# kspalaiologos/modern-rzip

Measured on AMD Instinct MI355X. Metric: rzip-stage GiB/s (mrzip -n), higher is better.
Workload: dtype u8; 1 GPU; tar-64G: rzip stage of mrzip -L7 on a 64 GiB synthetic tar (60 % text members, 25 % noise, 15 % exact duplicates, 512-byte aligned; BASELINE configs[2], the largest single-GPU configuration), one chunk per GPU, input resident in HBM; level=7, chunk_bytes_per_gpu=68719476736, streams=1, mode=streams

## Files before the change

### modern-rzip_amd/csrc/mrz_capi.hip

```cpp
#include <stdio.h>
#include <stdlib.h>
#include <string.h>

#include "../../include/mrzgpu.h"
#include "mrz_ctx.h"



static const unsigned k_levels[10][3] = { { 1, 4, 1 },  { 2, 4, 2 },  { 4, 4, 2 },   { 8, 4, 2 },   { 16, 4, 3 },
                                          { 32, 4, 4 }, { 32, 2, 6 }, { 64, 1, 16 }, { 64, 1, 32 }, { 64, 1, 128 } };

static void mrz_make_hash_index(int64_t H[256]) {
    int32_t r[31];
    int32_t word = 1;
    r[0] = 1;
    for (int i = 1; i < 31; i++) {
        const long hi = word / 127773, lo = word % 127773;
        long w = 16807 * lo - 2836 * hi;
        if (w < 0) w += 2147483647;
        r[i] = word = (int32_t)w;
    }
    int f = 3, b = 0;
    uint32_t draw[512];
    for (int k = -310; k < 512; k++) {
        const uint32_t s = (uint32_t)r[f] + (uint32_t)r[b];
        r[f] = (int32_t)s;
        if (++f == 31) f = 0;
        if (++b == 31) b = 0;
        if (k >= 0) draw[k] = s >> 1;
    }
    for (int i = 0; i < 256; i++) H[i] = ((int64_t)draw[2 * i] << 16) ^ (int64_t)draw[2 * i + 1];
}

extern "C" int mrz_abi_version(void) { return MRZ_ABI_VERSION; }

#define MRZ_EVENT_CAP (1ll << 28)
#define MRZ_EVENT_MIN 1024ll
#define MRZ_EVENT_MAX (1ll << 31)
static int64_t mrz_event_room(const mrz_ctx *ctx, int64_t n) {
    if (ctx->event_cap_set > 0) return ctx->event_cap_set;
    const int64_t worst = n / MRZ_MIN_MATCH + 2;
    return worst < MRZ_EVENT_CAP ? worst : MRZ_EVENT_CAP;
}

extern "C" const char *mrz_strerror(int code) {
    switch (code) {
        case MRZ_OK: return "ok";
        case MRZ_E_ARG: return "bad argument";
        case MRZ_E_NODEVICE: return "no usable HIP device (libmrzgpu has no CPU fallback)";
        case MRZ_E_NOMEM: return "out of memory";
        case MRZ_E_HIP: return "HIP runtime error";
        case MRZ_E_OVERFLOW: return "internal capacity exceeded";
        case MRZ_E_STATE: return "call order violated";
        case MRZ_E_CORRUPT: return "corrupt record stream or archive";
        case MRZ_E_UNSUPPORTED: return "block type not handled on this path (back-end codecs are host code)";
        default: return "unknown error";
    }
}

extern "C" int mrz_last_hip_error(const mrz_ctx *ctx, const char **text) {
    if (!ctx) return 0;
    if (text) *text = hipGetErrorString(ctx->last_err);
    return (int)ctx->last_err;
}

extern "C" int mrz_chunk_bytes(int64_t chunk_size) {
    int bits = 8;
    while (chunk_size >> bits > 0) bits++;
    return bits / 8 + (bits % 8 ? 1 : 0);
}

extern "C" void mrz_close(mrz_ctx *ctx) {
    if (!ctx) return;
    hipSetDevice(ctx->device);
    if (ctx->stream) hipStreamSynchronize(ctx->stream);
    hipFree(ctx->d_index);
    hipFree(ctx->d_tab);
    hipFree(ctx->d_state);
    if (ctx->h_ring) hipHostFree(ctx->h_ring);
    hipFree(ctx->d_fe_hdr);
    hipFree(ctx->d_bitmap);
    hipFree(ctx->d_tile_cnt);
    hipFree(ctx->d_tile_off);
    hipFree(ctx->d_grp_cnt);
    hipFree(ctx->d_cand);
    hipFree(ctx->d_events);
    hipFree(ctx->d_block_s0);
    hipFree(ctx->d_block_s1);
    hipFree(ctx->d_lit_off);
    hipFree(ctx->d_totals);
    hipFree(ctx->d_s0);
    hipFree(ctx->d_s1);
    hipFree(ctx->d_in);
    hipFree(ctx->d_crc_tables);
    hipFree(ctx->d_crc_parts);
    hipFree(ctx->d_crc_out);
    if (ctx->d_gmailbox) hipFree(ctx->d_gmailbox);
    if (ctx->d_seq_shared) hipFree(ctx->d_seq_shared);
    if (ctx->d_deep_shared) hipFree(ctx->d_deep_shared);
    if (ctx->d_wlog) hipFree(ctx->d_wlog);
    if (ctx->rz_scratch) hipFree(ctx->rz_scratch);
    if (ctx->d_rz_out) hipFree(ctx->d_rz_out);
    if (ctx->d_rz_done) hipFree(ctx->d_rz_done);
    if (ctx->d_rs_tables) hipFree(ctx->d_rs_tables);
    if (ctx->d_rs_out) hipFree(ctx->d_rs_out);
    if (ctx->lz4_scratch) hipFree(ctx->lz4_scratch);
    if (ctx->b2_scratch) hipFree(ctx->b2_scratch);
    if (ctx->side_stream) hipStreamDestroy(ctx->side_stream);
    if (ctx->copy_stream) hipStreamDestroy(ctx->copy_stream);
    if (ctx->stream) hipStreamDestroy(ctx->stream);
    free(ctx);
}

extern "C" int mrz_open(mrz_ctx **out, int device, int level, int64_t max_chunk) {
    if (!out || level < 1 || level > 9 || max_chunk < 0) return MRZ_E_ARG;
    *out = nullptr;
    int ndev = 0;
    hipError_t e0 = hipGetDeviceCount(&ndev);
    if (e0 != hipSuccess || ndev <= 0 || device < 0 || device >= ndev) {
        fprintf(stderr, "libmrzgpu: hipGetDeviceCount -> %d (%s), %d device(s), asked for %d\n", (int)e0,
                hipGetErrorString(e0), ndev, device);
        return MRZ_E_NODEVICE;
    }
    e0 = hipSetDevice(device);
    if (e0 != hipSuccess) {
        fprintf(stderr, "libmrzgpu: hipSetDevice(%d) -> %d (%s)\n", device, (int)e0, hipGetErrorString(e0));
        return MRZ_E_NODEVICE;
    }
    mrz_ctx *ctx = (mrz_ctx *)calloc(1, sizeof(mrz_ctx));
    if (!ctx) return MRZ_E_NOMEM;
    ctx->farm_helpers = -1;
    ctx->seg_positions = MRZ_SEG_POSITIONS;
    ctx->cand_cap = MRZ_CAND_CAP;
    {
        const char *e = getenv("MRZ_SEQ_ENGINE");
        if (e && !strcmp(e, "wide")) ctx->engine_pin = 1;
        if (e && !strcmp(e, "narrow")) ctx->engine_pin = 2;
        if (e && !strcmp(e, "deep")) ctx->engine_pin = 3;
        ctx->deep_min_bits = 6;
        if (const char *d = getenv("MRZ_DEEP_MIN_BITS")) ctx->deep_min_bits = atoi(d);
        ctx->narrow_max_bits = ctx->deep_min_bits;
        if (const char *d = getenv("MRZ_NARROW_MAX_BITS")) ctx->narrow_max_bits = atoi(d);
        e = getenv("MRZ_PRINT_PROF");
        if (e) ctx->print_prof = !strcmp(e, "narrow") ? 2 : 1;
        if (const char *c = getenv("MRZ_EVENT_CAPACITY")) {
            const long long v = atoll(c);
            if (v >= MRZ_EVENT_MIN && v <= MRZ_EVENT_MAX)
                ctx->event_cap_set = v;
            else if (v > 0)
                fprintf(stderr, "libmrzgpu: MRZ_EVENT_CAPACITY=%s ignored (%lld .. %lld entries)\n", c, MRZ_EVENT_MIN,
                        MRZ_EVENT_MAX);
        }
    }
    ctx->farm_default = mrz_sequencer_default_helpers(device);
    ctx->device = device;
    ctx->level = level;
    ctx->mb_used = k_levels[level][0];
    ctx->initial_freq = k_levels[level][1];
    ctx->max_chain = k_levels[level][2];
    const int64_t want = (int64_t)ctx->mb_used * (1048576 / 16);
    for (ctx->hash_bits = 0; (1ll << ctx->hash_bits) < want; ctx->hash_bits++) {
    }
    ctx->nslots = 1ll << ctx->hash_bits;
    mrz_make_hash_index(ctx->h_index);

    int rc = MRZ_OK;
    e0 = hipStreamCreate(&ctx->stream);
    if (e0 != hipSuccess) {
        fprintf(stderr, "libmrzgpu: hipStreamCreate -> %d (%s)\n", (int)e0, hipGetErrorString(e0));
        rc = MRZ_E_NODEVICE;
    }
    int64_t cap;
    if (!rc) { cap = 0; rc = mrz_grow(ctx, &ctx->d_index, &cap, 256); }
    if (!rc) { cap = 0; rc = mrz_grow(ctx, &ctx->d_tab, &cap, ctx->nslots); }
    if (!rc) { cap = 0; rc = mrz_grow(ctx, &ctx->d_state, &cap, 1); }
    if (!rc && hipHostMalloc((void **)&ctx->h_ring, MRZ_SEG_AHEAD * sizeof(mrz_seq_state)) != hipSuccess) rc = MRZ_E_NOMEM;
    if (!rc) { cap = 0; rc = mrz_grow(ctx, &ctx->d_fe_hdr, &cap, 1); }
    if (!rc) { cap = 0; rc = mrz_grow(ctx, &ctx->d_totals, &cap, 1); }
    if (!rc) { cap = 0; rc = mrz_grow(ctx, &ctx->d_crc_out, &cap, 4); }
    if (!rc) {
        void *p = nullptr;
        if (hipMalloc(&p, mrz_crc_tables_size()) != hipSuccess)
            rc = MRZ_E_NOMEM;
        else
            ctx->d_crc_tables = (mrz_crc_tables *)p;
    }
    if (!rc) {
        mrz_crc_tables *tb = (mrz_crc_tables *)malloc(mrz_crc_tables_size());
        if (!tb)
            rc = MRZ_E_NOMEM;
        else {
            mrz_crc_build_tables(tb);
            if (hipMemcpy(ctx->d_crc_tables, tb, mrz_crc_tables_size(), hipMemcpyHostToDevice) != hipSuccess)
                rc = MRZ_E_HIP;
            free(tb);
        }
    }
    if (!rc && hipMemcpy(ctx->d_index, ctx->h_index, sizeof(ctx->h_index), hipMemcpyHostToDevice) != hipSuccess)
        rc = MRZ_E_HIP;
    const size_t mbox = mrz_sequencer_mailbox_size() > mrz_seq_narrow_mailbox_size() ? mrz_sequencer_mailbox_size()
                                                                                     : mrz_seq_narrow_mailbox_size();
    if (!rc && mbox && !getenv("MRZ_NO_HELPER_WGS")) {
        void *p = nullptr;
        if (hipMalloc(&p, mbox) != hipSuccess)
            rc = MRZ_E_NOMEM;
        else
            ctx->d_gmailbox = p;
    }
    if (!rc) {
        if (hipMalloc(&ctx->d_seq_shared, mrz_sequencer_shared_size()) != hipSuccess ||
            hipMalloc((void **)&ctx->d_wlog, mrz_sequencer_wlog_size(ctx->nslots)) != hipSuccess)
            rc = MRZ_E_NOMEM;
        ctx->seq_wgs = 3;
        if (const char *e = getenv("MRZ_SEQ_WGS")) ctx->seq_wgs = atoi(e);
        if (hipMalloc(&ctx->d_deep_shared, mrz_seq_deep_shared_size()) != hipSuccess) rc = MRZ_E_NOMEM;
        ctx->deep_scanners = 63;
        if (const char *e = getenv("MRZ_DEEP_SCANNERS")) ctx->deep_scanners = atoi(e);
    }
    if (!rc && max_chunk > 0) {
        rc = mrz_grow(ctx, &ctx->d_events, &ctx->event_cap, mrz_event_room(ctx, max_chunk));
        if (!rc) rc = mrz_grow(ctx, &ctx->d_crc_parts, &ctx->crc_parts_cap, mrz_crc32_parts_needed(max_chunk));
        if (!rc) rc = mrz_fe_reserve(ctx, max_chunk / MRZ_TILE + 2, max_chunk);
    }
    if (rc) {
        mrz_close(ctx);
        return rc;
    }
    *out = ctx;
    return MRZ_OK;
}

extern "C" void *mrz_stream(const mrz_ctx *ctx) { return ctx ? (void *)ctx->stream : nullptr; }

extern "C" int mrz_synchronize(mrz_ctx *ctx) {
    if (!ctx) return MRZ_E_ARG;
    HIPCHK(ctx, hipSetDevice(ctx->device));
    HIPCHK(ctx, hipStreamSynchronize(ctx->stream));
    return MRZ_OK;
}

extern "C" int mrz_set_profiling(mrz_ctx *ctx, int enable) {
    if (!ctx) return MRZ_E_ARG;
    ctx->profiling = enable ? 1 : 0;
    return MRZ_OK;
}

extern "C" int mrz_set_progress(mrz_ctx *ctx, mrz_progress_fn fn, void *user) {
    if (!ctx) return MRZ_E_ARG;
    ctx->progress_fn = fn;
    ctx->progress_user = user;
    return MRZ_OK;
}

extern "C" int mrz_fetch_events(mrz_ctx *ctx, int64_t first, int64_t count, mrz_match *host_dst) {
    if (!ctx || first < 0 || count < 0 || (count > 0 && !host_dst)) return MRZ_E_ARG;
    if (first + count > ctx->events_final) return MRZ_E_STATE;
    if (first < ctx->ev_base) return MRZ_E_STATE;
    if (!count) return MRZ_OK;
    HIPCHK(ctx, hipSetDevice(ctx->device));
    if (!ctx->copy_stream) HIPCHK(ctx, hipStreamCreateWithFlags(&ctx->copy_stream, hipStreamNonBlocking));
    static_assert(sizeof(mrz_match) == sizeof(mrz_event), "mrz_match mirrors mrz_event");
    HIPCHK(ctx, hipMemcpyAsync(host_dst, ctx->d_events + (first - ctx->ev_base), (size_t)count * sizeof(mrz_event), hipMemcpyDeviceToHost,
                               ctx->copy_stream));
    HIPCHK(ctx, hipStreamSynchronize(ctx->copy_stream));
    return MRZ_OK;
}

extern "C" int mrz_set_cand_provider(mrz_ctx *ctx, mrz_cand_provider_fn fn, void *user) {
    if (!ctx) return MRZ_E_ARG;
    ctx->cand_fn = fn;
    ctx->cand_user = user;
    return MRZ_OK;
}

extern "C" int mrz_copy_to_device(mrz_ctx *ctx, void *dst_device, const void *src_host, int64_t n) {
    if (!ctx || n < 0 || (n > 0 && (!dst_device || !src_host))) return MRZ_E_ARG;
    if (!n) return MRZ_OK;
    HIPCHK(ctx, hipSetDevice(ctx->device));
    HIPCHK(ctx, hipMemcpyAsync(dst_device, src_host, (size_t)n, hipMemcpyHostToDevice, ctx->stream));
    HIPCHK(ctx, hipStreamSynchronize(ctx->stream));
    return MRZ_OK;
}

extern "C" int mrz_copy_device(mrz_ctx *ctx, void *dst_device, const void *src_device, int64_t n) {
    if (!ctx || n < 0 || (n > 0 && (!dst_device || !src_device))) return MRZ_E_ARG;
    if (!n) return MRZ_OK;
    HIPCHK(ctx, hipSetDevice(ctx->device));
    HIPCHK(ctx, hipMemcpyAsync(dst_device, src_device, (size_t)n, hipMemcpyDeviceToDevice, ctx->stream));
    HIPCHK(ctx, hipStreamSynchronize(ctx->stream));
    return MRZ_OK;
}

extern "C" int mrz_set_segment_positions(mrz_ctx *ctx, int64_t positions) {
    if (!ctx || positions < MRZ_TILE || positions > MRZ_SEG_POSITIONS || positions % MRZ_TILE) return MRZ_E_ARG;
    ctx->seg_positions = positions;
    return MRZ_OK;
}

extern "C" int mrz_set_candidate_capacity(mrz_ctx *ctx, int64_t entries) {
    if (!ctx || entries < MRZ_TILE || entries > (1ll << 30)) return MRZ_E_ARG;
    ctx->cand_cap = entries;
    return MRZ_OK;
}

extern "C" int mrz_set_event_capacity(mrz_ctx *ctx, int64_t entries) {
    if (!ctx || (entries > 0 && entries < MRZ_EVENT_MIN) || entries > MRZ_EVENT_MAX) return MRZ_E_ARG;
    ctx->event_cap_set = entries > 0 ? entries : 0;
    return MRZ_OK;
}

extern "C" int mrz_set_xcd(mrz_ctx *ctx, int xcd) {
    if (!ctx || xcd < 0 || xcd > 7) return MRZ_E_ARG;
    ctx->xcd = xcd;
    return MRZ_OK;
}

int mrz_fe_reserve(mrz_ctx *ctx, int64_t tiles, int64_t entries) {
    const int64_t max_tiles = ctx->seg_positions / MRZ_TILE;
    if (tiles > max_tiles) tiles = max_tiles;
    if (tiles < 1) tiles = 1;
    if (entries > ctx->cand_cap) entries = ctx->cand_cap;
    if (entries < MRZ_TILE) entries = MRZ_TILE;
    if (tiles > ctx->fe_tiles_cap) {
        int64_t c0 = 0, c1 = 0, c2 = 0, c3 = 0;
        if (ctx->d_bitmap) hipFree(ctx->d_bitmap), ctx->d_bitmap = nullptr;
        if (ctx->d_tile_cnt) hipFree(ctx->d_tile_cnt), ctx->d_tile_cnt = nullptr;
        if (ctx->d_tile_off) hipFree(ctx->d_tile_off), ctx->d_tile_off = nullptr;
        if (ctx->d_grp_cnt) hipFree(ctx->d_grp_cnt), ctx->d_grp_cnt = nullptr;
        ctx->fe_tiles_cap = 0;
        int rc = mrz_grow(ctx, &ctx->d_bitmap, &c0, tiles * (MRZ_TILE / 16) + 64);
        if (!rc) rc = mrz_grow(ctx, &ctx->d_tile_cnt, &c1, tiles + 1);
        if (!rc) rc = mrz_grow(ctx, &ctx->d_tile_off, &c2, tiles + 2);
        if (!rc) rc = mrz_grow(ctx, &ctx->d_grp_cnt, &c3, tiles / MRZ_FE_GROUP + 2);
        if (rc) return rc;
        ctx->fe_tiles_cap = tiles;
    }
    return mrz_grow(ctx, &ctx->d_cand, &ctx->cand_alloc, entries);
}

extern "C" int mrz_window_scan(mrz_ctx *ctx, const void *range_bytes, int64_t range_len, int where, int64_t range_start,
                               int64_t chunk_n, int64_t seg_start, int64_t max_span, int64_t min_mask, int64_t p_done,
                               int64_t cap, mrz_candidate *cand_out, int32_t *tile_off_out, void *bitmap_out, int out_where,
                               int64_t *scan_next, int64_t *n_cand) {
    if (!ctx || !range_bytes || !cand_out || !tile_off_out || !bitmap_out || !scan_next || !n_cand) return MRZ_E_ARG;
    if (range_len <= 0 || range_start < 0 || chunk_n <= 0 || cap < MRZ_TILE) return MRZ_E_ARG;
    if (max_span <= 0 || max_span > ctx->seg_positions || max_span % MRZ_TILE || seg_start % MRZ_TILE || seg_start < range_start)
        return MRZ_E_ARG;
    if (out_where != MRZ_MEM_HOST && out_where != MRZ_MEM_DEVICE) return MRZ_E_ARG;
    const int64_t end = chunk_n - MRZ_MIN_MATCH;
    int64_t last_pos = seg_start + max_span - 1;
    if (last_pos > end) last_pos = end;
    const int64_t need_end = last_pos + 48 < chunk_n ? last_pos + 48 : chunk_n;
    if (last_pos >= seg_start && need_end > range_start + range_len) return MRZ_E_ARG;
    HIPCHK(ctx, hipSetDevice(ctx->device));
    const uint8_t *d_range = nullptr;
    int rc = mrz_stage_input(ctx, range_bytes, range_len, where, &d_range);
    if (rc) return rc;
    const int64_t tiles = max_span / MRZ_TILE;
    const int64_t save_cap = ctx->cand_cap;
    if (cap > ctx->cand_cap) ctx->cand_cap = cap;
    rc = mrz_fe_reserve(ctx, tiles, cap);
    ctx->cand_cap = save_cap;
    if (rc) return rc;
    mrz_seq_state hs;
    memset(&hs, 0, sizeof(hs));
    hs.n = chunk_n;
    hs.end = end;
    hs.p = p_done + 1 < seg_start + MRZ_TILE ? p_done : seg_start - 1;
    hs.min_mask = min_mask;
    hs.scan_next = seg_start;
    hipStream_t s = ctx->stream;
    HIPCHK(ctx, hipMemcpyAsync(ctx->d_state, &hs, sizeof(hs), hipMemcpyHostToDevice, s));
    HIPCHK(ctx, mrz_launch_frontend(s, d_range - range_start, chunk_n, ctx->d_index, ctx->d_state, (int)tiles, cap,
                                    ctx->d_fe_hdr, ctx->d_bitmap, ctx->d_tile_cnt, ctx->d_tile_off, ctx->d_grp_cnt, ctx->d_cand));
    HIPCHK(ctx, hipMemcpyAsync(&hs, ctx->d_state, sizeof(hs), hipMemcpyDeviceToHost, s));
    HIPCHK(ctx, hipStreamSynchronize(s));
    int64_t T = (hs.scan_next - seg_start) / MRZ_TILE;
    if (hs.seg_start != seg_start || T < 0 || T > tiles) {
        T = 0;
        hs.n_cand = 0;
        hs.scan_next = hs.scan_next > seg_start ? hs.scan_next : seg_start;
    }
    const hipMemcpyKind k = out_where == MRZ_MEM_HOST ? hipMemcpyDeviceToHost : hipMemcpyDeviceToDevice;
    if (hs.n_cand > 0) HIPCHK(ctx, hipMemcpyAsync(cand_out, ctx->d_cand, (size_t)hs.n_cand * sizeof(mrz_cand), k, s));
    if (T > 0) {
        HIPCHK(ctx, hipMemcpyAsync(tile_off_out, ctx->d_tile_off, (size_t)(T + 1) * sizeof(int), k, s));
        HIPCHK(ctx, hipMemcpyAsync(bitmap_out, ctx->d_bitmap, (size_t)T * (MRZ_TILE / 8), k, s));
    }
    HIPCHK(ctx, hipStreamSynchronize(s));
    *scan_next = hs.scan_next;
    *n_cand = hs.n_cand;
    return MRZ_OK;
}

extern "C" int mrz_set_farm_helpers(mrz_ctx *ctx, int n) {
    if (!ctx) return MRZ_E_ARG;
    ctx->farm_helpers = n < 0 ? -1 : n;
    return MRZ_OK;
}

extern "C" int mrz_get_timings(const mrz_ctx *ctx, mrz_timings *out) {
    if (!ctx || !out) return MRZ_E_ARG;
    *out = ctx->timings;
    return MRZ_OK;
}

extern "C" int64_t mrz_table_slots(const mrz_ctx *ctx) { return ctx ? ctx->nslots : 0; }

extern "C" int mrz_fetch_table(mrz_ctx *ctx, void *host_dst) {
    if (!ctx || !host_dst) return MRZ_E_ARG;
    if (!ctx->have_chunk) return MRZ_E_STATE;
    HIPCHK(ctx, hipSetDevice(ctx->device));
    HIPCHK(ctx, hipMemcpy(host_dst, ctx->d_tab, (size_t)ctx->nslots * sizeof(mrz_slot), hipMemcpyDeviceToHost));
    return MRZ_OK;
}

int mrz_stage_input(mrz_ctx *ctx, const void *buf, int64_t n, int where, const uint8_t **dev) {
    if (where == MRZ_MEM_DEVICE) {
        *dev = (const uint8_t *)buf;
        return MRZ_OK;
    }
    if (where != MRZ_MEM_HOST) return MRZ_E_ARG;
    int rc = mrz_grow(ctx, &ctx->d_in, &ctx->in_cap, n + 64);
    if (rc) return rc;
    if (n > 0) HIPCHK(ctx, hipMemcpyAsync(ctx->d_in, buf, (size_t)n, hipMemcpyHostToDevice, ctx->stream));
    *dev = ctx->d_in;
    return MRZ_OK;
}

extern "C" int mrz_crc32(mrz_ctx *ctx, const void *buf, int64_t n, int where, uint32_t *crc_out) {
    if (!ctx || !crc_out || n < 0 || (n > 0 && !buf)) return MRZ_E_ARG;
    HIPCHK(ctx, hipSetDevice(ctx->device));
    const uint8_t *d = nullptr;
    int rc = mrz_stage_input(ctx, buf, n, where, &d);
    if (rc) return rc;
    rc = mrz_grow(ctx, &ctx->d_crc_parts, &ctx->crc_parts_cap, mrz_crc32_parts_needed(n));
    if (rc) return rc;
    HIPCHK(ctx, mrz_launch_crc32(ctx->stream, d, n, ctx->d_crc_tables, ctx->d_crc_parts, ctx->d_crc_out));
    HIPCHK(ctx, hipMemcpyAsync(crc_out, ctx->d_crc_out, 4, hipMemcpyDeviceToHost, ctx->stream));
    HIPCHK(ctx, hipStreamSynchronize(ctx->stream));
    return MRZ_OK;
}

struct mrz_evpair {
    hipEvent_t a, b;
    int kind;
};

static int64_t mrz_span_for_mask(const mrz_ctx *ctx, int64_t mask) {
    const int k = __builtin_popcountll((unsigned long long)mask);
    int64_t span = (ctx->cand_cap - ctx->cand_cap / 4) << (k < 24 ? k : 24);
    if (span > ctx->seg_positions) span = ctx->seg_positions;
    span = span / MRZ_TILE * MRZ_TILE;
    return span < MRZ_TILE ? MRZ_TILE : span;
}

extern "C" int mrz_rzip_chunk(mrz_ctx *ctx, const void *chunk, int64_t n, int where, int chunk_bytes,
                              int64_t *victim_round, mrz_chunk_result *res) {
    if (!ctx || !res || !victim_round || n < 0 || (n > 0 && !chunk) || chunk_bytes < 1 || chunk_bytes > 8)
        return MRZ_E_ARG;
    if (*victim_round < 0 || *victim_round >= (int64_t)ctx->max_chain) return MRZ_E_ARG;
    HIPCHK(ctx, hipSetDevice(ctx->device));
    memset(res, 0, sizeof(*res));
    memset(&ctx->timings, 0, sizeof(ctx->timings));
    ctx->have_chunk = 0;
    hipStream_t s = ctx->stream;

    const uint8_t *d_buf = nullptr;
    int rc = mrz_stage_input(ctx, chunk, n, where, &d_buf);
    if (rc) return rc;
    rc = mrz_grow(ctx, &ctx->d_events, &ctx->event_cap, mrz_event_room(ctx, n));
    if (rc) return rc;
    const int64_t ev_cap = ctx->event_cap_set > 0 ? ctx->event_cap_set : ctx->event_cap;
    const bool bounded = ev_cap < n / MRZ_MIN_MATCH + 2;
    rc = mrz_grow(ctx, &ctx->d_crc_parts, &ctx->crc_parts_cap, mrz_crc32_parts_needed(n));
    if (rc) return rc;
    const int64_t end = n - MRZ_MIN_MATCH;
    if (end > 0) {
        rc = mrz_fe_reserve(ctx, end / MRZ_TILE + 2, end + 1);
        if (rc) return rc;
    }

    mrz_evpair *evs = nullptr;
    int nev = 0, evcap = 0;
    hipEvent_t ev_begin = nullptr, ev_end = nullptr;
    if (ctx->profiling) {
        hipEventCreate(&ev_begin);
        hipEventCreate(&ev_end);
        hipEventRecord(ev_begin, s);
    }
#define PROF_BEGIN(k)                                                                       \
    do {                                                                                    \
        if (ctx->profiling) {                                                               \
            if (nev == evcap) {                                                             \
                const int ncap__ = evcap ? evcap * 2 : 64;                                  \
                mrz_evpair *ne__ = (mrz_evpair *)realloc(evs, (size_t)ncap__ * sizeof(mrz_evpair)); \
                if (ne__) evs = ne__, evcap = ncap__;                                       \
            }                                                                               \
            if (nev < evcap) {                                                              \
                evs[nev].kind = (k);                                                        \
                hipEventCreate(&evs[nev].a);                                                \
                hipEventCreate(&evs[nev].b);                                                \
                hipEventRecord(evs[nev].a, s);                                              \
            }                                                                               \
        }                                                                                   \
    } while (0)
#define PROF_END()                                     \
    do {                                               \
        if (ctx->profiling && nev < evcap) {           \
            hipEventRecord(evs[nev].b, s);             \
            nev++;                                     \
        }                                              \
    } while (0)

    mrz_seq_state hs;
    memset(&hs, 0, sizeof(hs));
    hs.n = n;
    hs.end = end;
    hs.min_mask = hs.tag_mask = (1ll << ctx->initial_freq) - 1;
    hs.limit = ctx->nslots / 3 * 2;
    hs.victim_round = *victim_round;
    hs.max_chain = ctx->max_chain;
    hs.slot_mask = ctx->nslots - 1;
    hs.event_cap = ev_cap;
    hs.finished = end > 0 ? 0 : 1;
    hipError_t herr = hipSuccess;
    int64_t E = 0;
    uint32_t crc = 0;
    mrz_enc_totals tot;
    memset(&tot, 0, sizeof(tot));

#define STEP(expr)                       \
    do {                                 \
        if (herr == hipSuccess) herr = (expr); \
    } while (0)

    STEP(hipMemsetAsync(ctx->d_tab, 0, (size_t)ctx->nslots * sizeof(mrz_slot), s));
    STEP(hipMemcpyAsync(ctx->d_state, &hs, sizeof(hs), hipMemcpyHostToDevice, s));
    STEP(hipMemsetAsync(ctx->d_totals, 0, sizeof(mrz_enc_totals), s));

    PROF_BEGIN(3);
    STEP(mrz_launch_crc32(s, d_buf, n, ctx->d_crc_tables, ctx->d_crc_parts, ctx->d_crc_out));
    PROF_END();

    ctx->events_final = 0;
    ctx->ev_base = 0;
    const size_t snap_bytes = offsetof(mrz_seq_state, prof);
    hipEvent_t seg_ev[MRZ_SEG_AHEAD];
    int n_seg_ev = 0;
    for (int k = 0; k < MRZ_SEG_AHEAD && herr == hipSuccess; k++) {
        STEP(hipEventCreateWithFlags(&seg_ev[k], hipEventDisableTiming));
        if (herr == hipSuccess) n_seg_ev++;
    }
    int64_t launched = 0, retired = 0, n_narrow = 0, n_deep = 0;
    int64_t span_of[MRZ_SEG_AHEAD];
    int64_t known_next = 0;
    int64_t known_mask = hs.min_mask, known_p = 0;
    int64_t hint_pos = 0, hint_matched = 0;
    int64_t known_events = 0, known_last = 0;
    bool finished = end <= 0;
    auto retire = [&]() {
        const mrz_seq_state *sn = &ctx->h_ring[retired % MRZ_SEG_AHEAD];
        retired++;
        known_p = sn->p;
        known_mask = sn->min_mask;
        known_events = sn->n_events;
        known_last = sn->last_match;
        if (!ctx->cand_fn)
            known_next = sn->scan_next;
        else if (sn->seg_end > sn->seg_start && sn->scan_next < sn->seg_end)
            known_next = sn->scan_next;
        hint_pos = sn->hint_positions;
        hint_matched = sn->hint_matched;
        if (ctx->progress_fn) {
            ctx->events_final = sn->n_events;
            if (ctx->progress_fn(ctx->progress_user, sn->n_events, sn->last_match, 0)) rc = MRZ_E_STATE;
        }
        if (sn->finished || sn->error) finished = true;
    };
    int64_t base0 = 0, base1 = 0, lit_from = 0, n_flushes = 0;
    auto encode_piece = [&](int64_t upto, int final_piece) {
        const int64_t Ep = upto - ctx->ev_base;
        const int64_t nblocks = (Ep + 1 + 255) / 256;
        int r = mrz_grow(ctx, &ctx->d_block_s0, &ctx->block_cap, nblocks);
        if (!r) r = mrz_grow(ctx, &ctx->d_block_s1, &ctx->block1_cap, nblocks);
        if (!r) r = mrz_grow(ctx, &ctx->d_lit_off, &ctx->lit_off_cap, Ep + 2);
        if (r) return r;
        PROF_BEGIN(2);
        STEP(mrz_launch_enc_size(s, ctx->d_events, Ep, final_piece, lit_from, n, chunk_bytes, ctx->d_block_s0,
                                 ctx->d_block_s1, base0, base1, ctx->d_totals));
        STEP(hipMemcpyAsync(&tot, ctx->d_totals, sizeof(tot), hipMemcpyDeviceToHost, s));
        STEP(hipStreamSynchronize(s));
        if (herr == hipSuccess) {
            if (!base0) r = mrz_grow(ctx, &ctx->d_s0, &ctx->s0_cap, tot.s0_len + 7 + 16);
            else r = mrz_grow_keep(ctx, &ctx->d_s0, &ctx->s0_cap, base0 + tot.s0_len + 7 + 16, base0);
            if (!r && !base1) r = mrz_grow(ctx, &ctx->d_s1, &ctx->s1_cap, tot.s1_len + 16);
            else if (!r) r = mrz_grow_keep(ctx, &ctx->d_s1, &ctx->s1_cap, base1 + tot.s1_len + 16, base1);
        }
        if (herr == hipSuccess && !r) {
            STEP(mrz_launch_enc_write(s, d_buf, ctx->d_events, Ep, final_piece, lit_from, n, chunk_bytes, ctx->d_block_s0,
                                      ctx->d_block_s1, ctx->d_s0, ctx->d_s1, base1, tot.s1_len, ctx->d_lit_off,
                                      ctx->d_totals, crc));
            STEP(hipMemcpyAsync(&tot, ctx->d_totals, sizeof(tot), hipMemcpyDeviceToHost, s));
        }
        PROF_END();
        return r;
    };
    auto drain = [&]() {
        const int r = encode_piece(known_events, 0);
        if (r || herr != hipSuccess) return r;
        ctx->ev_base = known_events;
        STEP(hipMemcpyAsync(&ctx->d_state->ev_base, &ctx->ev_base, sizeof(int64_t), hipMemcpyHostToDevice, s));
        STEP(hipStreamSynchronize(s));
        base0 += tot.s0_len;
        base1 += tot.s1_len;
        lit_from = known_last;
        n_flushes++;
        return 0;
    };
    int64_t pass_cap = MRZ_MIN_MATCH * (ev_cap / 2) / MRZ_TILE * MRZ_TILE;
    if (pass_cap < MRZ_TILE) pass_cap = MRZ_TILE;
    while (!finished && herr == hipSuccess && !rc) {
        while (retired < launched && !finished && !rc && hipEventQuery(seg_ev[retired % MRZ_SEG_AHEAD]) == hipSuccess) retire();
        if (finished || rc) break;
        int64_t est_next = known_next;
        for (int64_t k = retired; k < launched; k++) est_next += span_of[k % MRZ_SEG_AHEAD];
        const bool queue_full = launched - retired >= MRZ_SEG_AHEAD;
        const bool all_queued = est_next > end;
        if (queue_full || (all_queued && launched > retired)) {
            STEP(hipEventSynchronize(seg_ev[retired % MRZ_SEG_AHEAD]));
            if (herr != hipSuccess) break;
            retire();
            continue;
        }
        if (all_queued) {
            rc = MRZ_E_OVERFLOW;
            break;
        }
        int64_t span = mrz_span_for_mask(ctx, known_mask);
        if (bounded && span > pass_cap) span = pass_cap;
        int64_t max_tiles = span / MRZ_TILE;
        if (max_tiles > ctx->fe_tiles_cap) max_tiles = ctx->fe_tiles_cap;
        span = max_tiles * MRZ_TILE;
        if (bounded) {
            const int64_t pt = (known_p + 1) / MRZ_TILE * MRZ_TILE;
            int64_t from = known_next > pt ? known_next : pt;
            for (int64_t k = retired; k < launched; k++) from += span_of[k % MRZ_SEG_AHEAD];
            const int64_t fixed = known_events - ctx->ev_base + 2 + 1 + (launched - retired + 1);
            int64_t F = from + span - 1;
            if (F > end) F = end;
            if (fixed + (F - known_p) / MRZ_MIN_MATCH > ev_cap) {
                if (launched > retired) {
                    STEP(hipEventSynchronize(seg_ev[retired % MRZ_SEG_AHEAD]));
                    if (herr != hipSuccess) break;
                    retire();
                    continue;
                }
                if (known_events > ctx->ev_base) {
                    rc = drain();
                    continue;
                }
                const int64_t fit = (ev_cap - fixed) * MRZ_MIN_MATCH + MRZ_MIN_MATCH - 1 - (from - 1 - known_p);
                if (fit < MRZ_TILE) {
                    rc = MRZ_E_OVERFLOW;
                    break;
                }
                if (span > fit) span = fit / MRZ_TILE * MRZ_TILE;
                max_tiles = span / MRZ_TILE;
            }
        }
        PROF_BEGIN(0);
        if (ctx->cand_fn) {
            int64_t seg_start = known_next;
            const int64_t pt = (known_p + 1) / MRZ_TILE * MRZ_TILE;
            if (pt > seg_start) seg_start = pt;
            if (seg_start > end) {
                known_next = seg_start;
                span_of[launched % MRZ_SEG_AHEAD] = 0;
            } else {
                if (seg_start + span > end + 1) span = (end + 1 - seg_start + MRZ_TILE - 1) / MRZ_TILE * MRZ_TILE;
                int64_t geo[5] = { seg_start, 0, 0, 0, known_mask };
                int64_t nx = seg_start, nc = 0;
                if (herr == hipSuccess && ctx->cand_fn(ctx->cand_user, seg_start, span, known_mask, known_p, ctx->cand_cap,
                                                       (mrz_candidate *)ctx->d_cand, ctx->d_tile_off, ctx->d_bitmap, &nx, &nc,
                                                       (void *)s)) {
                    hipStreamSynchronize(s);
                    rc = MRZ_E_STATE;
                    break;
                }
                if (nx <= seg_start || nx > seg_start + span || nx % MRZ_TILE || nc < 0 || nc > ctx->cand_cap) {
                    hipStreamSynchronize(s);
                    rc = MRZ_E_STATE;
                    break;
                }
                geo[1] = nx < end + 1 ? nx : end + 1;
                geo[2] = nc;
                geo[3] = nx;
                STEP(hipMemcpyAsync(&ctx->d_state->seg_start, geo, sizeof(geo), hipMemcpyHostToDevice, s));
                STEP(hipStreamSynchronize(s));
                known_next = nx;
                span_of[launched % MRZ_SEG_AHEAD] = 0;
            }
        } else {
            STEP(mrz_launch_frontend(s, d_buf, n, ctx->d_index, ctx->d_state, (int)max_tiles, ctx->cand_cap, ctx->d_fe_hdr,
                                     ctx->d_bitmap, ctx->d_tile_cnt, ctx->d_tile_off, ctx->d_grp_cnt, ctx->d_cand));
            span_of[launched % MRZ_SEG_AHEAD] = span;
        }
        PROF_END();
        const int mask_bits = __builtin_popcountll((unsigned long long)known_mask);
        bool narrow = hint_pos > 0 && hint_matched * 10 >= hint_pos * 8 && mask_bits < ctx->narrow_max_bits;
        bool deep = !narrow && mask_bits >= ctx->deep_min_bits;
        if (ctx->engine_pin) narrow = ctx->engine_pin == 2, deep = ctx->engine_pin == 3;
        const int helpers = ctx->farm_helpers >= 0 && ctx->farm_helpers < ctx->farm_default ? ctx->farm_helpers : ctx->farm_default;
        PROF_BEGIN(1);
        if (narrow)
            STEP(mrz_launch_sequencer_narrow(s, d_buf, ctx->d_tab, ctx->d_cand, ctx->d_tile_off, (const mrz_u64 *)ctx->d_bitmap,
                                             ctx->d_events, ctx->d_state, ctx->d_gmailbox, helpers, ctx->xcd));
        else if (deep)
            STEP(mrz_launch_sequencer_deep(s, d_buf, ctx->d_tab, ctx->d_cand, ctx->d_tile_off, (const mrz_u64 *)ctx->d_bitmap,
                                           ctx->d_events, ctx->d_state, ctx->d_gmailbox, helpers, ctx->xcd, ctx->d_deep_shared,
                                           ctx->deep_scanners));
        else
            STEP(mrz_launch_sequencer(s, d_buf, ctx->d_tab, ctx->d_cand, ctx->d_tile_off, (const mrz_u64 *)ctx->d_bitmap,
                                      ctx->d_events, ctx->d_state, ctx->d_gmailbox, helpers, ctx->d_seq_shared, ctx->d_wlog,
                                      ctx->nslots, ctx->seq_wgs, ctx->xcd, ctx->engine_pin ? 0 : ctx->deep_min_bits));
        PROF_END();
        if (narrow) n_narrow++;
        if (deep) n_deep++;
        STEP(hipMemcpyAsync(&ctx->h_ring[launched % MRZ_SEG_AHEAD], ctx->d_state, snap_bytes, hipMemcpyDeviceToHost, s));
        STEP(hipEventRecord(seg_ev[launched % MRZ_SEG_AHEAD], s));
        launched++;
        if (launched <= 2 && !ctx->engine_pin && !ctx->cand_fn) STEP(hipStreamSynchronize(s));
    }
    hipStreamSynchronize(s);
    for (int k = 0; k < n_seg_ev; k++) hipEventDestroy(seg_ev[k]);
    STEP(hipMemcpyAsync(&hs, ctx->d_state, sizeof(hs), hipMemcpyDeviceToHost, s));
    STEP(hipMemcpyAsync(&crc, ctx->d_crc_out, 4, hipMemcpyDeviceToHost, s));
    STEP(hipStreamSynchronize(s));
    if (herr == hipSuccess) {
        if (!rc && (hs.error || !hs.finished)) {
            fprintf(stderr,
                    "libmrzgpu: sequencer stopped abnormally: error=%d finished=%d p=%lld end=%lld events=%lld/%lld "
                    "count=%lld min_mask=%lld scan_next=%lld launches=%lld\n",
                    hs.error, hs.finished, (long long)hs.p, (long long)hs.end, (long long)hs.n_events,
                    (long long)hs.event_cap, (long long)hs.count, (long long)hs.min_mask, (long long)hs.scan_next,
                    (long long)launched);
            rc = MRZ_E_OVERFLOW;
        }
        E = hs.n_events;
        if (!rc && ctx->progress_fn) {
            ctx->events_final = E;
            if (ctx->progress_fn(ctx->progress_user, E, hs.last_match, 1)) rc = MRZ_E_STATE;
        }
    }

    if (herr == hipSuccess && !rc) {
        rc = encode_piece(E, 1);
        if (ctx->profiling) hipEventRecord(ev_end, s);
        STEP(hipStreamSynchronize(s));
    }

    ctx->timings.n_segments = (int32_t)launched;
    ctx->timings.n_narrow = (int32_t)n_narrow;
    ctx->timings.n_deep = (int32_t)n_deep;
    ctx->timings.n_event_flushes = (int32_t)n_flushes;
    if (ctx->profiling) {
        hipStreamSynchronize(s);
        for (int i = 0; i < nev; i++) {
            float ms = 0;
            if (hipEventElapsedTime(&ms, evs[i].a, evs[i].b) == hipSuccess) {
                if (evs[i].kind == 0) ctx->timings.tagscan_ms += ms;
                if (evs[i].kind == 1) ctx->timings.sequencer_ms += ms;
                if (evs[i].kind == 2) ctx->timings.encode_ms += ms;
                if (evs[i].kind == 3) ctx->timings.crc_ms += ms;
            }
            hipEventDestroy(evs[i].a);
            hipEventDestroy(evs[i].b);
        }
        float ms = 0;
        if (hipEventElapsedTime(&ms, ev_begin, ev_end) == hipSuccess) ctx->timings.total_ms = ms;
        hipEventDestroy(ev_begin);
        hipEventDestroy(ev_end);
        free(evs);
    }
#undef PROF_BEGIN
#undef PROF_END
#undef STEP
    if (herr != hipSuccess) {
        ctx->last_err = herr;
        return MRZ_E_HIP;
    }
    if (rc) return rc;

    *victim_round = hs.victim_round;
    ctx->s0_len = base0 + tot.s0_len + 7;
    ctx->s1_len = base1 + tot.s1_len;
    ctx->have_chunk = 1;
    res->s0_len = ctx->s0_len;
    res->s1_len = ctx->s1_len;
    res->crc32 = crc;
    res->d_s0 = ctx->d_s0;
    res->d_s1 = ctx->d_s1;
    res->stats.inserts = hs.inserts;
    res->stats.tag_hits = hs.tag_hits;
    res->stats.tag_misses = hs.tag_misses;
    res->stats.literals = tot.literals + 1;
    res->stats.literal_bytes = tot.literal_bytes;
    res->stats.matches = tot.matches;
    res->stats.match_bytes = tot.match_bytes;
    res->min_mask = hs.min_mask;
    res->hash_count = hs.count;
    res->n_events = E;
    if (ctx->print_prof) {
        static const char *names[128] = { "batches", "formed", "committed", "segments", "emits", "backjump", "rewalk",
                                          "longres", "seq_cands", "cut_cplx", "cut_overflow", "skipout", "conf0", "pairs",
                                          "t_form", "t_walk", "t_conf", "t_pairs", "t_loop", "t_rewalk", "t_long", "t_seq",
                                          "farmed", "l_post", "l_stripe", "l_bwd", "l_wait", "l_rounds", "f_post", "f_wait",
                                          "f_fold", "s_tab", "s_pair", "s_ins", "ovl", "ovl_ok", "x_walk", "x_casc", "x_pool",
                                          "x_win", "x_same", "c_win", "c_evict", "c_deep", "c_many", "c_fail", "c_tie", "c_nw", "t_ovl",
                                          "h_pre", "h_cand", "h_post", "t_scan", "t_fold", "t_commit", "reprep", "w_stale", "w_drop", "reset",
                                          "t_turn", "t_prep", "t_precommit", "e_mask", "e_cull", "e_xw", "e_inwin", "e_window", "e_bulk",
                                          "e_more", "t_pc_cw", "t_pc_log", "t_pc_best", "t_pc_bulk", "t_turnwork", "t_snap", "rebulk",
                                          "batch_lanes", "cut_long", "cut_walk", "cut_conflict", "cut_cull", "batch_emits",
                                          "cut_cascade", "batch_formed", "t_walk2", "t_scans", "t_conflict", "t_window",
                                          "d_batches", "d_lanes", "d_rounds", "d_rescanned", "d_coop", "d_t_form", "d_t_scan",
                                          "d_t_commit", "d_t_rescan", "d_t_total", "d_launches", "d_t_coop", "d_coop_rec",
                                          "d_resolved", "d_s_coop", "d_s_conflict", "d_s_culled", "d_s_nocull", "d_s_stale", "d_c_over_alt", "d_c_over_noalt", "d_c_empty",
                                          "d_c_displace", "d_c_other" };
        for (int k = 0; k < 128; k++)
            if (names[k] && hs.prof[k]) fprintf(stderr, "seqstat %-12s %lld\n", names[k], (long long)hs.prof[k]);
    }
    return MRZ_OK;
}

extern "C" int mrz_fetch_streams(mrz_ctx *ctx, uint8_t *s0_host, uint8_t *s1_host) {
    if (!ctx) return MRZ_E_ARG;
    if (!ctx->have_chunk) return MRZ_E_STATE;
    HIPCHK(ctx, hipSetDevice(ctx->device));
    if (s0_host && ctx->s0_len > 0)
        HIPCHK(ctx, hipMemcpyAsync(s0_host, ctx->d_s0, (size_t)ctx->s0_len, hipMemcpyDeviceToHost, ctx->stream));
    if (s1_host && ctx->s1_len > 0)
        HIPCHK(ctx, hipMemcpyAsync(s1_host, ctx->d_s1, (size_t)ctx->s1_len, hipMemcpyDeviceToHost, ctx->stream));
    HIPCHK(ctx, hipStreamSynchronize(ctx->stream));
    return MRZ_OK;
}
```

### modern-rzip_amd/csrc/mrz_common.h

```cpp
#pragma once
#include <stdint.h>

#define MRZ_MIN_MATCH 31
#define MRZ_GREAT_MATCH 1024
#define MRZ_WAVE 64

struct __attribute__((aligned(16))) mrz_slot {
    int64_t off;
    int64_t t;
};

struct mrz_event {
    int64_t p;
    int64_t ofs;
    int64_t len;
};

struct mrz_seq_state {
    int64_t n;
    int64_t end;
    int64_t p;
    int64_t cur_p, cur_ofs, cur_len;
    int64_t last_match;
    int64_t min_mask;
    int64_t tag_mask;
    int64_t count;
    int64_t limit;
    int64_t clean_ptr;
    int64_t victim_round;
    int64_t max_chain;
    int64_t slot_mask;
    int64_t n_events;
    int64_t event_cap;
    int64_t ev_base;
    int64_t inserts, tag_hits, tag_misses;
    int32_t finished;
    int32_t error;
    int64_t hint_positions;
    int64_t hint_events;
    int64_t hint_matched;
    int64_t seg_start;
    int64_t seg_end;
    int64_t n_cand;
    int64_t scan_next;
    int64_t list_mask;
    int64_t prof[128];
};

typedef mrz_slot mrz_cand;

struct mrz_fe_hdr {
    int64_t base;
    int64_t mask;
    int64_t p_done;
    int32_t ntiles;
    int32_t T;
};

#define MRZ_TILE 4096
#define MRZ_TILE_SHIFT 12
#define MRZ_FE_GROUP 256

struct mrz_enc_totals {
    int64_t s0_len;
    int64_t s1_len;
    int64_t literals, literal_bytes, matches, match_bytes;
};
```

### modern-rzip_amd/csrc/mrz_ctx.h

```cpp
#pragma once
#include <stdint.h>
#include <stdlib.h>

#include "../../include/mrzgpu.h"
#include "mrz_kernels.h"

#define MRZ_SEG_POSITIONS (1ll << 30)
#define MRZ_CAND_CAP (8ll << 20)
#define MRZ_SEG_AHEAD 4

struct mrz_ctx {
    int device;
    int level;
    unsigned mb_used, initial_freq, max_chain;
    int hash_bits;
    int64_t nslots;
    hipStream_t stream;
    hipError_t last_err;
    int profiling;
    mrz_timings timings;

    int64_t h_index[256];
    int64_t *d_index;
    mrz_slot *d_tab;
    mrz_seq_state *d_state;
    mrz_seq_state *h_ring;
    mrz_fe_hdr *d_fe_hdr;
    uint16_t *d_bitmap;
    int *d_tile_cnt, *d_tile_off, *d_grp_cnt;
    int64_t fe_tiles_cap;
    mrz_cand *d_cand;
    int64_t cand_alloc;
    int64_t cand_cap;
    int engine_pin;
    int deep_min_bits;
    int narrow_max_bits;
    int print_prof;
    int xcd;
    mrz_event *d_events;
    int64_t event_cap;
    int64_t event_cap_set;
    int64_t ev_base;
    int64_t *d_block_s0, *d_block_s1;
    int64_t block_cap, block1_cap;
    int64_t *d_lit_off;
    int64_t lit_off_cap;
    mrz_enc_totals *d_totals;
    uint8_t *d_s0, *d_s1;
    int64_t s0_cap, s1_cap;
    int64_t s0_len, s1_len;
    uint8_t *d_in;
    int64_t in_cap;
    mrz_crc_tables *d_crc_tables;
    uint32_t *d_crc_parts;
    int64_t crc_parts_cap;
    uint32_t *d_crc_out;
    void *d_gmailbox;
    void *d_seq_shared;
    unsigned *d_wlog;
    int seq_wgs;
    void *d_deep_shared;
    int deep_scanners;
    int farm_helpers;
    int farm_default;
    void *d_rs_tables;
    uint8_t *d_rs_out;
    int64_t rs_out_cap;
    void *rz_scratch;
    int64_t rz_scratch_cap;
    uint8_t *d_rz_out;
    int64_t rz_out_cap;
    unsigned *d_rz_done;
    int64_t rz_done_cap;
    int have_chunk;

    void *lz4_scratch;
    int64_t lz4_scratch_cap;
    void *b2_scratch;
    int64_t b2_scratch_cap;
    hipStream_t side_stream;
    hipStream_t copy_stream;
    mrz_progress_fn progress_fn;
    void *progress_user;
    int64_t events_final;
    int64_t seg_positions;
    mrz_cand_provider_fn cand_fn;
    void *cand_user;
};

#define HIPCHK(ctx, expr)                     \
    do {                                      \
        hipError_t e__ = (expr);              \
        if (e__ != hipSuccess) {              \
            (ctx)->last_err = e__;            \
            return MRZ_E_HIP;                 \
        }                                     \
    } while (0)

template <typename T>
static inline int mrz_grow(mrz_ctx *ctx, T **ptr, int64_t *cap, int64_t want) {
    if (want <= *cap && *ptr) return MRZ_OK;
    if (*ptr) {
        hipFree(*ptr);
        *ptr = nullptr;
        *cap = 0;
    }
    int64_t ask = want < 16 ? 16 : want;
    void *p = nullptr;
    hipError_t e = hipMalloc(&p, (size_t)ask * sizeof(T));
    if (e != hipSuccess) {
        ctx->last_err = e;
        return MRZ_E_NOMEM;
    }
    *ptr = (T *)p;
    *cap = ask;
    return MRZ_OK;
}

template <typename T>
static inline int mrz_grow_keep(mrz_ctx *ctx, T **ptr, int64_t *cap, int64_t want, int64_t keep) {
    if (want <= *cap && *ptr) return MRZ_OK;
    int64_t ask = *cap + *cap / 2 > want ? *cap + *cap / 2 : want;
    if (ask < 16) ask = 16;
    void *p = nullptr;
    hipError_t e = hipMalloc(&p, (size_t)ask * sizeof(T));
    if (e != hipSuccess && ask > want) {
        ask = want;
        e = hipMalloc(&p, (size_t)ask * sizeof(T));
    }
    if (e != hipSuccess) {
        ctx->last_err = e;
        return MRZ_E_NOMEM;
    }
    if (*ptr) {
        if (keep > 0) e = hipMemcpyAsync(p, *ptr, (size_t)keep * sizeof(T), hipMemcpyDeviceToDevice, ctx->stream);
        if (e == hipSuccess) e = hipStreamSynchronize(ctx->stream);
        if (e != hipSuccess) {
            hipFree(p);
            ctx->last_err = e;
            return MRZ_E_HIP;
        }
        hipFree(*ptr);
    }
    *ptr = (T *)p;
    *cap = ask;
    return MRZ_OK;
}

int mrz_fe_reserve(mrz_ctx *ctx, int64_t tiles, int64_t entries);

int mrz_stage_input(mrz_ctx *ctx, const void *buf, int64_t n, int where, const uint8_t **dev);
```

### modern-rzip_amd/csrc/mrz_kernels.h

```cpp
#pragma once
#include <hip/hip_runtime.h>
#include <stdint.h>

#include "mrz_common.h"

typedef unsigned long long mrz_u64;
struct mrz_crc_tables;

extern "C" {
struct mrz_fe_bufs {
    mrz_fe_hdr *hdr;
    uint16_t *bitmap16;
    int *tile_cnt;
    int *tile_off;
    int *grp_cnt;
    mrz_cand *cand;
};
hipError_t mrz_launch_frontend(hipStream_t stream, const uint8_t *buf, int64_t n, const int64_t *hash_index,
                               mrz_seq_state *st, int max_tiles, int64_t cap, mrz_fe_hdr *hdr, uint16_t *bitmap16,
                               int *tile_cnt, int *tile_off, int *grp_cnt, mrz_cand *cand);
hipError_t mrz_launch_sequencer(hipStream_t stream, const uint8_t *buf, mrz_slot *tab, const mrz_cand *cand,
                                const int *tile_off, const mrz_u64 *bitmap, mrz_event *events, mrz_seq_state *st,
                                void *gmailbox, int n_helpers, void *wide_shared, unsigned *wlog,
                                int64_t nslots, int seq_wgs, int xcd, int deep_bits);
size_t mrz_sequencer_shared_size(void);
size_t mrz_sequencer_wlog_size(int64_t nslots);
hipError_t mrz_launch_sequencer_narrow(hipStream_t stream, const uint8_t *buf, mrz_slot *tab, const mrz_cand *cand,
                                       const int *tile_off, const mrz_u64 *bitmap, mrz_event *events, mrz_seq_state *st,
                                       void *gmailbox, int n_helpers, int xcd);
hipError_t mrz_launch_sequencer_deep(hipStream_t stream, const uint8_t *buf, mrz_slot *tab, const mrz_cand *cand,
                                     const int *tile_off, const mrz_u64 *bitmap, mrz_event *events, mrz_seq_state *st,
                                     void *gmailbox, int n_helpers, int xcd, void *deep_shared, int scanners);
size_t mrz_seq_deep_shared_size(void);
size_t mrz_sequencer_mailbox_size(void);
size_t mrz_seq_narrow_mailbox_size(void);
int mrz_sequencer_default_helpers(int device);
hipError_t mrz_launch_enc_size(hipStream_t stream, const mrz_event *ev, int64_t E, int final_piece, int64_t lit0,
                               int64_t n, int cb, int64_t *block_s0, int64_t *block_s1, int64_t base0, int64_t base1,
                               mrz_enc_totals *totals);
hipError_t mrz_launch_enc_write(hipStream_t stream, const uint8_t *buf, const mrz_event *ev, int64_t E, int final_piece,
                                int64_t lit0, int64_t n, int cb, const int64_t *block_s0, const int64_t *block_s1,
                                uint8_t *s0, uint8_t *s1, int64_t base1, int64_t s1_len, int64_t *lit_off,
                                mrz_enc_totals *totals, uint32_t crc);
void mrz_crc_build_tables(mrz_crc_tables *tb);
size_t mrz_crc_tables_size(void);
int64_t mrz_crc32_parts_needed(int64_t n);
hipError_t mrz_launch_crc32(hipStream_t stream, const uint8_t *buf, int64_t n, const mrz_crc_tables *tb, uint32_t *parts,
                            uint32_t *crc_out);
}
```

### modern-rzip_amd/csrc/mrz_seq_common.h

```cpp
#pragma once
#include "mrz_device.h"
#include <stdlib.h>

#ifdef __HIP_DEVICE_COMPILE__
#define MRZ_WAVE_SYNC() __builtin_amdgcn_wave_barrier()
#else
#define MRZ_WAVE_SYNC() (void)__ballot(1)
#endif

#ifndef MRZ_WIDE_WAVES
#define MRZ_WIDE_WAVES 8
#endif
#ifndef MRZ_SEQ_WAVES
#define MRZ_SEQ_WAVES MRZ_WIDE_WAVES
#endif
#define MRZ_SEQ_THREADS (64 * MRZ_SEQ_WAVES)
#ifdef MRZ_NARROW_ENGINE
#define MRZ_STRIPE_WAVES (MRZ_SEQ_WAVES > 2 ? MRZ_SEQ_WAVES - 1 : MRZ_SEQ_WAVES)
#else
#define MRZ_STRIPE_WAVES 1
#endif
#ifndef MRZ_HELPER_WAVES
#define MRZ_HELPER_WAVES 3
#endif
#define MRZ_CASCADE_MAX 64
#ifndef MRZ_SEQ_CREDIT
#define MRZ_SEQ_CREDIT 8
#endif
#ifndef MRZ_LOW_YIELD_RUNS
#define MRZ_LOW_YIELD_RUNS 2
#endif

#ifdef MRZ_SEQ_PROFILE
#define PROF_T0() int64_t prof_t0 = (int64_t)__builtin_amdgcn_s_memtime()
#define PROF_T0R() prof_t0 = (int64_t)__builtin_amdgcn_s_memtime()
#define PROF_ADD(k)                                                      \
    do {                                                                 \
        const int64_t now__ = (int64_t)__builtin_amdgcn_s_memtime();     \
        stat[k] += now__ - prof_t0;                                      \
        prof_t0 = now__;                                                 \
    } while (0)
#else
#define PROF_T0()
#define PROF_T0R()
#define PROF_ADD(k)
#endif

#if defined(MRZ_SEQ_PROFILE) && !defined(MRZ_SEQ_STATS)
#define MRZ_SEQ_STATS 1
#endif
#ifdef MRZ_SEQ_STATS
#define ST_ADD(k, v) (stat[k] += (v))
#else
#define ST_ADD(k, v) ((void)0)
#endif
#ifndef MRZ_WLOG_SHIFT
#define MRZ_WLOG_SHIFT 2
#endif
enum { MRZ_ST_BATCHES, MRZ_ST_FORMED, MRZ_ST_COMMITTED, MRZ_ST_SEGMENTS, MRZ_ST_EMITS, MRZ_ST_BACKJUMP, MRZ_ST_REWALK,
       MRZ_ST_LONGRES, MRZ_ST_SEQ, MRZ_ST_CUT_CPLX, MRZ_ST_CUT_OVERFLOW, MRZ_ST_SKIPOUT, MRZ_ST_CONF0, MRZ_ST_PAIRS,
       MRZ_ST_T_FORM, MRZ_ST_T_WALK, MRZ_ST_T_CONF, MRZ_ST_T_PAIRS, MRZ_ST_T_LOOP, MRZ_ST_T_REWALK, MRZ_ST_T_LONG,
       MRZ_ST_T_SEQ, MRZ_ST_FARMED, MRZ_ST_L_POST, MRZ_ST_L_STRIPE, MRZ_ST_L_BWD, MRZ_ST_L_WAIT, MRZ_ST_L_ROUNDS,
       MRZ_ST_F_POST, MRZ_ST_F_WAIT, MRZ_ST_F_FOLD, MRZ_ST_S_TAB, MRZ_ST_S_PAIR, MRZ_ST_S_INS, MRZ_ST_OVL, MRZ_ST_OVL_OK,
       MRZ_ST_X_WALK, MRZ_ST_X_CASC, MRZ_ST_X_POOL, MRZ_ST_X_WIN, MRZ_ST_X_SAME, MRZ_ST_C_WIN, MRZ_ST_C_EVICT, MRZ_ST_C_DEEP,
       MRZ_ST_C_MANY, MRZ_ST_C_FAIL, MRZ_ST_C_TIE, MRZ_ST_C_NW, MRZ_ST_T_OVL, MRZ_ST_H_PRE, MRZ_ST_H_CAND, MRZ_ST_H_POST,
       MRZ_ST_T_SCAN, MRZ_ST_T_FOLD, MRZ_ST_T_COMMIT, MRZ_ST_REPREP, MRZ_ST_W_STALE, MRZ_ST_W_DROP, MRZ_ST_RESET,
       MRZ_ST_T_TURN, MRZ_ST_T_PREP, MRZ_ST_T_PRECOMMIT, MRZ_ST_E_MASK, MRZ_ST_E_CULL, MRZ_ST_E_XW, MRZ_ST_E_INWIN,
       MRZ_ST_E_WINDOW, MRZ_ST_E_BULK, MRZ_ST_E_MORE, MRZ_ST_T_PC_CW, MRZ_ST_T_PC_LOG, MRZ_ST_T_PC_BEST, MRZ_ST_T_PC_BULK, MRZ_ST_T_TURNWORK, MRZ_ST_T_SNAP, MRZ_ST_REBULK,
       MRZ_ST_BATCH_LANES, MRZ_ST_CUT_LONG, MRZ_ST_CUT_WALK, MRZ_ST_CUT_CONFLICT, MRZ_ST_CUT_CULL, MRZ_ST_BATCH_EMITS,
       MRZ_ST_CUT_CASCADE, MRZ_ST_BATCH_FORMED, MRZ_ST_T_WALK2, MRZ_ST_T_SCANS, MRZ_ST_T_CONFLICT, MRZ_ST_T_WINDOW,
       MRZ_ST_D_BATCHES, MRZ_ST_D_LANES, MRZ_ST_D_ROUNDS, MRZ_ST_D_RESCANNED, MRZ_ST_D_COOP, MRZ_ST_D_T_FORM, MRZ_ST_D_T_SCAN,
       MRZ_ST_D_T_COMMIT, MRZ_ST_D_T_RESCAN, MRZ_ST_D_T_TOTAL, MRZ_ST_D_LAUNCHES, MRZ_ST_D_T_COOP, MRZ_ST_D_COOP_REC,
       MRZ_ST_D_RESOLVED, MRZ_ST_D_S_COOP, MRZ_ST_D_S_CONFLICT, MRZ_ST_D_S_CULLED, MRZ_ST_D_S_NOCULL, MRZ_ST_D_S_STALE, MRZ_ST_D_C_OVER_ALT, MRZ_ST_D_C_OVER_NOALT, MRZ_ST_D_C_EMPTY, MRZ_ST_D_C_DISPLACE, MRZ_ST_D_C_OTHER,
       MRZ_ST_N };
static_assert(MRZ_ST_N <= (int)(sizeof(((mrz_seq_state *)0)->prof) / sizeof(int64_t)), "mrz_seq_state.prof holds the counters");

struct mrz_seq_args {
    const uint8_t *buf;
    mrz_slot *tab;
    const mrz_cand *cand;
    const int *tile_off;
    const mrz_u64 *bitmap;
    mrz_event *events;
    mrz_seq_state *st;
    void *gmailbox;
    int n_helpers;
    int xcd;
    int deep_bits;
};

struct mrz_cands {
    const mrz_cand *cand;
    const int *tile_off;
    const mrz_u64 *bitmap;
    int64_t seg_start, seg_end, n;
};

__device__ static int64_t mrz_cand_lower_bound(const mrz_cands &K, int64_t pos, int lane) {
    if (pos <= K.seg_start) return 0;
    if (pos >= K.seg_end) return K.n;
    const int64_t rel = pos - K.seg_start;
    const int64_t tile = rel >> MRZ_TILE_SHIFT;
    const int r = (int)(rel & (MRZ_TILE - 1));
    const mrz_u64 w = K.bitmap[tile * (MRZ_TILE / 64) + lane];
    const int base = K.tile_off[tile];
    int c = 0;
    if (lane < (r >> 6))
        c = __popcll(w);
    else if (lane == (r >> 6))
        c = __popcll(w & mrz_low_mask(r & 63));
    const int sum = mrz_lane_read(mrz_wave_incl_sum(c, lane), 63);
    return (int64_t)mrz_uni(base) + sum;
}

__device__ __forceinline__ int mrz_mb_load(int *p) {
    return __hip_atomic_load(p, __ATOMIC_ACQUIRE, __HIP_MEMORY_SCOPE_WORKGROUP);
}
__device__ __forceinline__ void mrz_mb_store(int *p, int v) {
    __hip_atomic_store(p, v, __ATOMIC_RELEASE, __HIP_MEMORY_SCOPE_WORKGROUP);
}

__device__ __forceinline__ void mrz_mb_add(int *p, int v) {
    __hip_atomic_fetch_add(p, v, __ATOMIC_RELEASE, __HIP_MEMORY_SCOPE_WORKGROUP);
}

struct mrz_mailbox {
    int64_t p0, op, maxf, base;
    int64_t res[MRZ_SEQ_WAVES];
    int seq;
    int done;
    int quit;
    int scout_seq;
    int64_t scout_pos;
    int64_t scout_clean;
};

#ifndef MRZ_STRIPE_PIECES
#define MRZ_STRIPE_PIECES 4
#endif
#define MRZ_STRIPE (MRZ_STRIPE_PIECES * 1024)

template <int PIECES>
__device__ static int64_t mrz_wave_fwd_stripe_n(const uint8_t *__restrict__ buf, int64_t p0, int64_t op, int64_t maxf,
                                                int64_t base, int lane) {
    uint4 a[PIECES], b[PIECES];
#pragma unroll
    for (int j = 0; j < PIECES; j++) {
        const int64_t off = base + j * 1024 + lane * 16;
        if (off < maxf) {
            a[j] = mrz_ld16(buf + p0 + off);
            b[j] = mrz_ld16(buf + op + off);
        }
    }
    int64_t found = -1;
#pragma unroll
    for (int j = 0; j < PIECES; j++) {
        if (found >= 0) continue;
        const int64_t off = base + j * 1024 + lane * 16;
        int lane_len = 0;
        bool full = false;
        if (off < maxf) {
            const int64_t rem = maxf - off;
            const int lim = rem < 16 ? (int)rem : 16;
            const int d = mrz_first_diff16(a[j], b[j]);
            lane_len = d < lim ? d : lim;
            full = lane_len == 16;
        }
        const mrz_u64 stop = __ballot(!full);
        if (stop) {
            const int fl = __ffsll((long long)stop) - 1;
            found = base + j * 1024 + (int64_t)fl * 16 + mrz_lane_read(lane_len, fl);
        }
    }
    return found;
}

__device__ __forceinline__ int64_t mrz_wave_fwd_stripe(const uint8_t *__restrict__ buf, int64_t p0, int64_t op,
                                                       int64_t maxf, int64_t base, int lane) {
    return mrz_wave_fwd_stripe_n<MRZ_STRIPE_PIECES>(buf, p0, op, maxf, base, lane);
}

__device__ static int64_t mrz_wave_bwd(const uint8_t *__restrict__ buf, int64_t p0, int64_t op, int64_t maxb,
                                       int lane) {
    if (maxb <= 0) return 0;
    for (int64_t base = 0;; base += 1024) {
        const int64_t off = base + lane * 16;
        int lane_len = 0;
        bool full = false;
        if (off < maxb) {
            const int64_t rem = maxb - off;
            const int lim = rem < 16 ? (int)rem : 16;
            int cnt;
            if (op - off - 16 >= 0) {
                cnt = mrz_top_equal16(mrz_ld16(buf + p0 - off - 16), mrz_ld16(buf + op - off - 16));
            } else {
                cnt = 0;
                while (cnt < lim && buf[p0 - off - 1 - cnt] == buf[op - off - 1 - cnt]) cnt++;
            }
            lane_len = cnt < lim ? cnt : lim;
            full = lane_len == 16;
        }
        const mrz_u64 stop = __ballot(!full);
        if (stop) {
            const int fl = __ffsll((long long)stop) - 1;
            return base + (int64_t)fl * 16 + mrz_lane_read(lane_len, fl);
        }
    }
}

__device__ static int64_t mrz_long_match_len(const uint8_t *__restrict__ buf, mrz_mailbox *mb, int *mb_seq, int64_t p0,
                                             int64_t op, int64_t end, int64_t last_match, int64_t *rev_out, int lane,
                                             int64_t *stat = nullptr, int64_t *cont_base = nullptr) {
    *rev_out = 0;
#ifdef MRZ_SEQ_PROFILE
    int64_t lt0 = (int64_t)__builtin_amdgcn_s_memtime();
#define LPROF(k)                                                         \
    do {                                                                 \
        if (stat) {                                                      \
            const int64_t now__ = (int64_t)__builtin_amdgcn_s_memtime(); \
            stat[k] += now__ - lt0;                                      \
            lt0 = now__;                                                 \
        }                                                                \
    } while (0)
#else
#define LPROF(k)
#endif
    if (op >= p0) return 0;
    const int64_t maxf = end - p0;
    const int64_t floor_p = last_match > 0 ? last_match : 0;
    int64_t maxb = p0 - floor_p;
    if (op < maxb) maxb = op;
    int64_t fwd = 0, rev = 0;
    bool have_rev = false;
    const bool striped = MRZ_STRIPE_WAVES > 1 && mb != nullptr;
    const int64_t round_bytes = (int64_t)(striped ? MRZ_STRIPE_WAVES : 1) * MRZ_STRIPE;
    if (maxf > 0) {
        for (int64_t base = 0;; base += round_bytes) {
            if (striped) {
                if (lane == 0) {
                    mb->p0 = p0;
                    mb->op = op;
                    mb->maxf = maxf;
                    mb->base = base;
                    mb->done = 0;
                }
                *mb_seq += 1;
                if (lane == 0) mrz_mb_store(&mb->seq, *mb_seq);
            }
            LPROF(MRZ_ST_L_POST);
            int64_t best = mrz_wave_fwd_stripe(buf, p0, op, maxf, base, lane);
            LPROF(MRZ_ST_L_STRIPE);
            if (!have_rev) {
                rev = mrz_wave_bwd(buf, p0, op, maxb, lane);
                have_rev = true;
            }
            LPROF(MRZ_ST_L_BWD);
            if (striped) {
                while (mrz_uni(mrz_mb_load(&mb->done)) < MRZ_STRIPE_WAVES - 1) __builtin_amdgcn_s_sleep(1);
                for (int w = 1; w < MRZ_STRIPE_WAVES && best < 0; w++) best = mrz_uni64(mb->res[w]);
            }
            LPROF(MRZ_ST_L_WAIT);
#ifdef MRZ_SEQ_STATS
            if (stat) stat[MRZ_ST_L_ROUNDS] += 1;
#endif
            if (best >= 0) {
                fwd = best;
                break;
            }
            if (cont_base) {
                *cont_base = base + round_bytes;
                *rev_out = rev;
                return -1;
            }
        }
    }
    if (!have_rev) rev = mrz_wave_bwd(buf, p0, op, maxb, lane);
    *rev_out = rev;
    const int64_t len = fwd + rev;
    return len < MRZ_MIN_MATCH ? 0 : len;
}

__device__ __forceinline__ bool mrz_insert_step(const mrz_slot e, bool empty, int64_t t, int my_rank, int64_t slot0,
                                                int64_t slot_mask, int64_t better, int64_t max_chain,
                                                int64_t *round, int64_t *victim_h, int64_t *count,
                                                int64_t *victim_round, int64_t *stop_slot, int *kind, int64_t *occ_t,
                                                int64_t *occ_off) {
    const bool minbit = !empty && ((e.t & better) != better);
    const bool lesser = !empty && (mrz_ones_rank(e.t) < my_rank);
    const bool same = !empty && (e.t == t);
    const mrz_u64 m_stop = __ballot(empty || minbit || lesser);
    const int first_stop = m_stop ? __ffsll((long long)m_stop) - 1 : MRZ_WAVE;
    const mrz_u64 m_same = __ballot(same) & mrz_low_mask(first_stop);
    const int cnt = __popcll(m_same);
    const int64_t kv = *victim_round - *round;
    if (kv >= 0 && kv < cnt) *victim_h = (slot0 + mrz_nth_set(m_same, (int)kv)) & slot_mask;
    const int64_t k = max_chain - *round;
    if (k <= cnt) {
        *count -= 1;
        int64_t vr = *victim_round + 1;
        if (vr == max_chain) vr = 0;
        *victim_round = vr;
        *stop_slot = *victim_h;
        *kind = 1;
        return true;
    }
    if (first_stop < MRZ_WAVE) {
        *stop_slot = (slot0 + first_stop) & slot_mask;
        const int64_t et = mrz_bcast64(e.t, first_stop);
        const int64_t eo = mrz_bcast64(e.off, first_stop);
        if ((eo | et) == 0)
            *kind = 0;
        else if ((et & better) != better) {
            *count -= 1;
            *kind = 1;
        } else {
            *kind = 2;
            *occ_t = et;
            *occ_off = eo;
        }
        return true;
    }
    *round += cnt;
    return false;
}

#ifndef MRZ_HELPER_WGS
#define MRZ_HELPER_WGS 240
#endif
#ifndef MRZ_HELPERS_PER_CU
#define MRZ_HELPERS_PER_CU 1
#endif
#define MRZ_FARM_ENTRIES 16
#define MRZ_FARM_WATCH ((MRZ_HELPER_WGS + 63) / 64)
#ifndef MRZ_FARM_WAVE_BYTES
#define MRZ_FARM_WAVE_BYTES 2048
#endif
#ifndef MRZ_FARM_HELPER_SLEEP
#define MRZ_FARM_HELPER_SLEEP 2
#endif
#ifndef MRZ_FARM_LEADER_SLEEP
#define MRZ_FARM_LEADER_SLEEP 1
#endif
#ifndef MRZ_FARM_HINT_MIN
#define MRZ_FARM_HINT_MIN 8192
#endif
#define MRZ_FARM_SPW (MRZ_HELPER_WAVES * MRZ_FARM_WAVE_BYTES)
#define MRZ_FARM_GMAX 255
#ifndef MRZ_FARM_ROWS0
#define MRZ_FARM_ROWS0 14
#endif
#ifndef MRZ_FARM_BULK_MULT
#define MRZ_FARM_BULK_MULT 16
#endif
#define MRZ_FARM_SHIFT 40
#define MRZ_FARM_PAYLOAD ((1ull << MRZ_FARM_SHIFT) - 1)
#define MRZ_FARM_NONE MRZ_FARM_PAYLOAD
#define MRZ_SPIN_LIMIT (1 << 20)
#define MRZ_HELPER_SPIN_LIMIT (1ll << 34)

struct mrz_gmailbox {
    unsigned long long quit;
    unsigned long long ready;
    unsigned long long pad0[14];
    unsigned long long words[8 + MRZ_FARM_ENTRIES];
    unsigned long long pad1[8];
    unsigned long long rev[MRZ_FARM_ENTRIES];
    unsigned long long res[MRZ_HELPER_WGS > 0 ? MRZ_HELPER_WGS : 1];
    long long dbg[5][MRZ_FARM_ENTRIES];
};

__device__ __forceinline__ unsigned long long mrz_g_loadu(const unsigned long long *p) {
    return __hip_atomic_load(p, __ATOMIC_RELAXED, __HIP_MEMORY_SCOPE_AGENT);
}
__device__ __forceinline__ void mrz_g_storeu(unsigned long long *p, unsigned long long v) {
    __hip_atomic_store(p, v, __ATOMIC_RELAXED, __HIP_MEMORY_SCOPE_AGENT);
}

#if MRZ_HELPER_WGS > 0
__device__ static void mrz_helper_wg(const uint8_t *__restrict__ buf, mrz_gmailbox *g) {
    __shared__ unsigned long long s_job[2][26];
    __shared__ unsigned long long s_min;
    __shared__ unsigned s_cnt;
    const int lane = threadIdx.x & 63;
    const int wave = mrz_uni((int)(threadIdx.x >> 6));
    if (wave >= MRZ_HELPER_WAVES) return;
    if (threadIdx.x == 0) {
        s_job[0][25] = __hip_atomic_fetch_add(&g->ready, 1ull, __ATOMIC_RELAXED, __HIP_MEMORY_SCOPE_AGENT);
        s_min = MRZ_FARM_NONE;
        s_cnt = 0;
    }
    __syncthreads();
    const int me = (int)s_job[0][25];
    if (me >= MRZ_HELPER_WGS) return;
    unsigned long long seen = 0;
    int par = 0;
    while (true) {
        par ^= 1;
        if (wave == 0) {
            long long spins = 0;
            while (true) {
                unsigned long long w = 0;
                if (lane < 8 + MRZ_FARM_ENTRIES)
                    w = mrz_g_loadu(&g->words[lane]);
                else if (lane == 8 + MRZ_FARM_ENTRIES)
                    w = mrz_g_loadu(&g->quit);
                const unsigned long long tag = w >> MRZ_FARM_SHIFT;
                const unsigned long long tag0 = (unsigned long long)mrz_bcast64((int64_t)tag, 0);
                const bool quit = mrz_bcast64((int64_t)w, 8 + MRZ_FARM_ENTRIES) != 0;
                const bool fresh = tag0 != seen && __ballot(lane < 8 + MRZ_FARM_ENTRIES && tag != tag0) == 0;
                const bool giveup = quit || spins++ >= MRZ_HELPER_SPIN_LIMIT;
                if (fresh || giveup) {
                    if (lane < 8 + MRZ_FARM_ENTRIES) s_job[par][lane] = w & MRZ_FARM_PAYLOAD;
                    if (lane == 8 + MRZ_FARM_ENTRIES) s_job[par][lane] = giveup ? ~0ull : tag0;
                    break;
                }
                __builtin_amdgcn_s_sleep(MRZ_FARM_HELPER_SLEEP);
            }
        }
        __syncthreads();
        const unsigned long long tag = s_job[par][8 + MRZ_FARM_ENTRIES];
        if (tag == ~0ull) return;
        seen = tag;
        const int cfg = (int)s_job[par][4];
        const int lgc = cfg & 0xff, G = (cfg >> 8) & 0xff, mult = (cfg >> 24) & 0xff;
        const bool want_rev = (cfg >> 16) & 1;
        const int e = me & ((1 << lgc) - 1), s = me >> lgc;
        const bool bwd_job = want_rev && s == G;
        if (s >= G && !bwd_job) continue;
        const int64_t p0 = (int64_t)s_job[par][0], op = (int64_t)s_job[par][8 + e];
        if (op >= p0) continue;
        if (bwd_job) {
            if (wave == 0) {
                const int64_t floor_p = (int64_t)s_job[par][2];
                int64_t maxb = p0 - floor_p;
                if (op < maxb) maxb = op;
                const int64_t rev = mrz_wave_bwd(buf, p0, op, maxb, lane);
                if (lane == 0) mrz_g_storeu(&g->rev[e], (tag << MRZ_FARM_SHIFT) | (unsigned long long)rev);
            }
            continue;
        }
        const int64_t maxf = (int64_t)s_job[par][1], base = (int64_t)s_job[par][3];
        int64_t r = -1;
        {
            const int64_t off0 = base + (int64_t)s * mult * MRZ_FARM_SPW + (int64_t)wave * mult * MRZ_FARM_WAVE_BYTES;
            if (mult >= 4) {
                for (int k = 0; k < mult * MRZ_FARM_WAVE_BYTES && r < 0; k += 8192)
                    r = mrz_wave_fwd_stripe_n<8>(buf, p0, op, maxf, off0 + k, lane);
            } else
                for (int k = 0; k < mult && r < 0; k++)
                    r = mrz_wave_fwd_stripe_n<MRZ_FARM_WAVE_BYTES / 1024>(buf, p0, op, maxf,
                                                                          off0 + (int64_t)k * MRZ_FARM_WAVE_BYTES, lane);
        }
        if (lane == 0) {
            if (r >= 0) atomicMin(&s_min, (unsigned long long)r);
            if (atomicAdd(&s_cnt, 1u) == MRZ_HELPER_WAVES - 1) {
                const unsigned long long best = atomicExch(&s_min, MRZ_FARM_NONE);
                s_cnt = 0;
                mrz_g_storeu(&g->res[me], (tag << MRZ_FARM_SHIFT) | best);
            }
        }
    }
}
#endif

#define MRZ_SMAX 16
#ifndef MRZ_WALK_SLOTS
#define MRZ_WALK_SLOTS 8
#endif
#ifndef MRZ_WALK_STEPS
#define MRZ_WALK_STEPS 12
#endif
#ifndef MRZ_WALK_LANE_STEPS
#define MRZ_WALK_LANE_STEPS 2
#endif
#ifndef MRZ_WALK_COOP_MAX
#define MRZ_WALK_COOP_MAX 6
#endif
#define MRZ_WALK_COOP_STEPS 2

struct mrz_coop_lds {
    int64_t same_off[MRZ_SMAX];
    int pair_res[MRZ_SMAX];
    unsigned long long farm_min[16];
    int64_t pend_h[MRZ_CASCADE_MAX], pend_t[MRZ_CASCADE_MAX], pend_o[MRZ_CASCADE_MAX];
    int n_written;
    int64_t cull_slot;
};

__device__ __forceinline__ int mrz_first_diff16_bf(uint4 a, uint4 b) {
    const uint32_t d0 = a.x ^ b.x, d1 = a.y ^ b.y, d2 = a.z ^ b.z, d3 = a.w ^ b.w;
    int r = 16;
    r = d3 ? 12 + ((__ffs((int)d3) - 1) >> 3) : r;
    r = d2 ? 8 + ((__ffs((int)d2) - 1) >> 3) : r;
    r = d1 ? 4 + ((__ffs((int)d1) - 1) >> 3) : r;
    r = d0 ? ((__ffs((int)d0) - 1) >> 3) : r;
    return r;
}
__device__ __forceinline__ int mrz_top_equal16_bf(uint4 a, uint4 b) {
    const uint32_t d0 = a.x ^ b.x, d1 = a.y ^ b.y, d2 = a.z ^ b.z, d3 = a.w ^ b.w;
    int r = 16;
    r = d0 ? 12 + (__clz((int)d0) >> 3) : r;
    r = d1 ? 8 + (__clz((int)d1) >> 3) : r;
    r = d2 ? 4 + (__clz((int)d2) >> 3) : r;
    r = d3 ? (__clz((int)d3) >> 3) : r;
    return r;
}

__device__ static void mrz_lane_match_len(const uint8_t *__restrict__ buf, int64_t q, int64_t op, int64_t end,
                                          int64_t last_match, int64_t *len, int64_t *rev, bool *is_long) {
    *len = 0;
    *rev = 0;
    *is_long = false;
    if (op >= q) return;
    int64_t maxf = end - q;
    if (maxf < 0) maxf = 0;
    const int64_t floor_p = last_match > 0 ? last_match : 0;
    int64_t maxb = q - floor_p;
    if (op < maxb) maxb = op;
    if (maxb < 0) maxb = 0;
    const int64_t last_ok = end + (MRZ_MIN_MATCH - 16);
    uint4 fa[4], fb[4], ba[4], bb[4];
#pragma unroll
    for (int j = 0; j < 4; j++) {
        int64_t pa = q + j * 16, pb = op + j * 16;
        pa = pa < last_ok ? pa : last_ok;
        pb = pb < last_ok ? pb : last_ok;
        fa[j] = mrz_ld16(buf + pa);
        fb[j] = mrz_ld16(buf + pb);
        int64_t ra = q - (j + 1) * 16, rb = op - (j + 1) * 16;
        ra = ra > 0 ? ra : 0;
        rb = rb > 0 ? rb : 0;
        ba[j] = mrz_ld16(buf + ra);
        bb[j] = mrz_ld16(buf + rb);
    }
    int rawf;
    {
        const int d0 = mrz_first_diff16_bf(fa[0], fb[0]), d1 = mrz_first_diff16_bf(fa[1], fb[1]);
        const int d2 = mrz_first_diff16_bf(fa[2], fb[2]), d3 = mrz_first_diff16_bf(fa[3], fb[3]);
        rawf = d0 < 16 ? d0 : 16 + (d1 < 16 ? d1 : 16 + (d2 < 16 ? d2 : 16 + d3));
    }
    const int64_t fwd = rawf < maxf ? rawf : maxf;
    bool lng = rawf == 64 && maxf > 64;
    const int edge = op < 64 ? (int)(op >> 4) : 4;
    int rawb;
    {
        const int e0 = edge > 0 ? mrz_top_equal16_bf(ba[0], bb[0]) : 16, e1 = edge > 1 ? mrz_top_equal16_bf(ba[1], bb[1]) : 16;
        const int e2 = edge > 2 ? mrz_top_equal16_bf(ba[2], bb[2]) : 16, e3 = edge > 3 ? mrz_top_equal16_bf(ba[3], bb[3]) : 16;
        rawb = e0 < 16 ? e0 : 16 + (e1 < 16 ? e1 : 16 + (e2 < 16 ? e2 : 16 + e3));
    }
    const int64_t rv = rawb < maxb ? rawb : maxb;
    lng = lng || (rawb == 64 && maxb > 64) || (edge < 4 && rawb >= 16 * edge && maxb > 16 * edge);
    *is_long = lng;
    if (lng) return;
    *rev = rv;
    const int64_t l = fwd + rv;
    *len = l >= MRZ_MIN_MATCH ? l : 0;
}

struct mrz_lead {
    int64_t p, cur_p, cur_ofs, cur_len, last_match;
    int64_t min_mask, tag_mask, count, clean_ptr, victim_round;
    int64_t n_events, inserts, tag_hits, tag_misses;
    int64_t last_len;
    int64_t mbytes;
};

struct mrz_cfg {
    const uint8_t *buf;
    mrz_slot *tab;
    mrz_event *events;
    mrz_seq_state *st;
    int64_t end, limit, max_chain, slot_mask, nslots, event_cap;
    int64_t ev_base;
    mrz_gmailbox *gmb;
    unsigned long long *gseq;
    int *gnw;
    int n_helpers;
    int64_t *farm_hint;
    int *long_seen;
    mrz_mailbox *mb;
    int *mb_seq;
};

__device__ __forceinline__ bool mrz_select_emit(const mrz_cfg &C, mrz_lead &L, int64_t mlen, int64_t m_off,
                                                int64_t m_rev, int lane) {
    if (mlen > L.cur_len) {
        L.cur_p = L.p - m_rev;
        L.cur_len = mlen;
        L.cur_ofs = m_off;
    }
    if ((L.cur_len >= MRZ_GREAT_MATCH || L.p >= L.cur_p + MRZ_MIN_MATCH) && L.cur_len >= MRZ_MIN_MATCH) {
        if (L.n_events - C.ev_base >= C.event_cap) {
            if (lane == 0) C.st->error = 1;
            return false;
        }
        if (lane == 0) {
            mrz_event ev;
            ev.p = L.cur_p;
            ev.ofs = L.cur_ofs;
            ev.len = L.cur_len;
            C.events[L.n_events - C.ev_base] = ev;
        }
        L.n_events++;
        L.last_len = L.cur_len;
        L.mbytes += L.cur_len;
        L.last_match = L.cur_p + L.cur_len;
        L.cur_p = L.p = L.last_match;
        L.cur_len = 0;
    }
    return true;
}

__device__ static void mrz_cull_one(const mrz_cfg &C, mrz_lead &L, int lane) {
    mrz_slot *tab = C.tab;
    while (true) {
        const int64_t better2 = (L.min_mask << 1) | 1;
        bool culled = false;
        while (L.clean_ptr < C.nslots) {
            const int64_t s = L.clean_ptr + lane;
            mrz_slot e;
            e.off = 0;
            e.t = 0;
            if (s < C.nslots) e = tab[s];
            const bool hit = ((e.off | e.t) != 0) && ((e.t & better2) != better2);
            const mrz_u64 m = __ballot(hit);
            if (m) {
                const int fl = __ffsll((long long)m) - 1;
                L.clean_ptr += fl;
                if (lane == fl) {
                    mrz_slot z;
                    z.off = 0;
                    z.t = 0;
                    tab[s] = z;
                }
                L.count--;
                culled = true;
                break;
            }
            L.clean_ptr += MRZ_WAVE;
        }
        if (culled) {
            L.tag_mask = better2;
            return;
        }
        L.min_mask = better2;
        L.clean_ptr = 0;
    }
}

#if MRZ_HELPER_WGS > 0
__device__ static bool mrz_farm(const mrz_cfg &C, mrz_coop_lds *B, int64_t p0, int64_t maxf, int64_t floor_p,
                                int64_t base, int nsx, int64_t my_op, bool my_pending, bool want_rev, int lane,
                                int64_t *stat, int64_t *my_fwd, int64_t *my_rev) {
    mrz_gmailbox *g = C.gmb;
#ifdef MRZ_SEQ_PROFILE
    int64_t prof_t0 = (int64_t)__builtin_amdgcn_s_memtime();
#endif
    mrz_u64 pending = __ballot(my_pending && lane < nsx);
    int64_t fwd = 0, rev = 0;
    int rounds = 0;
    while (pending) {
        const int np = __popcll(pending);
        int lgc = 0;
        while ((1 << lgc) < np) lgc++;
        const int ncols = 1 << lgc;
        int G = (*C.gnw >> lgc) - (want_rev ? 1 : 0);
        if (G > MRZ_FARM_GMAX) G = MRZ_FARM_GMAX;
        if (rounds == 0 && G > MRZ_FARM_ROWS0) G = MRZ_FARM_ROWS0;
        const int mult = rounds == 0 ? 1 : (rounds == 1 ? 4 : MRZ_FARM_BULK_MULT);
        const int nass = G << lgc;
        const int my_col = __popcll(pending & mrz_low_mask(lane));
        const bool mine = lane < nsx && ((pending >> lane) & 1);
        *C.gseq += 1;
        const unsigned long long seq = *C.gseq;
        {
            const int col = lane - 8;
            if (mine) B->farm_min[my_col] = (unsigned long long)my_op;
            MRZ_WAVE_SYNC();
            const int64_t op_of = (col >= 0 && col < np) ? (int64_t)B->farm_min[col] : 0;
            MRZ_WAVE_SYNC();
            unsigned long long v = 0;
            if (lane == 0) v = (unsigned long long)p0;
            if (lane == 1) v = (unsigned long long)(maxf > 0 ? maxf : 0);
            if (lane == 2) v = (unsigned long long)floor_p;
            if (lane == 3) v = (unsigned long long)base;
            if (lane == 4) v = (unsigned long long)(lgc | (G << 8) | ((want_rev ? 1 : 0) << 16) | (mult << 24));
            if (lane >= 8) v = (unsigned long long)((col < np) ? op_of : p0);
            if (lane < 8 + MRZ_FARM_ENTRIES) mrz_g_storeu(&g->words[lane], (seq << MRZ_FARM_SHIFT) | v);
        }
        PROF_ADD(MRZ_ST_F_POST);
        int colw[MRZ_FARM_WATCH];
        bool watch[MRZ_FARM_WATCH];
#pragma unroll
        for (int j = 0; j < MRZ_FARM_WATCH; j++) {
            const int w = lane + 64 * j;
            colw[j] = w & (ncols - 1);
            watch[j] = w < nass && colw[j] < np;
        }
        const bool watch_rev = want_rev && mine;
        unsigned long long val[MRZ_FARM_WATCH], rv = 0, ready = 0;
#pragma unroll
        for (int j = 0; j < MRZ_FARM_WATCH; j++) val[j] = 0;
        int spins = 0;
        while (true) {
            bool ok = true;
#pragma unroll
            for (int j = 0; j < MRZ_FARM_WATCH; j++)
                if (watch[j]) val[j] = mrz_g_loadu(&g->res[lane + 64 * j]);
            if (watch_rev) rv = mrz_g_loadu(&g->rev[my_col]);
            if (lane == 63) ready = mrz_g_loadu(&g->ready);
#pragma unroll
            for (int j = 0; j < MRZ_FARM_WATCH; j++)
                if (watch[j]) ok = ok && (val[j] >> MRZ_FARM_SHIFT) == seq;
            if (watch_rev) ok = ok && (rv >> MRZ_FARM_SHIFT) == seq;
            if (__ballot(!ok) == 0) break;
            if (spins++ >= MRZ_SPIN_LIMIT) {
                *C.gnw = -1;
                return false;
            }
            __builtin_amdgcn_s_sleep(MRZ_FARM_LEADER_SLEEP);
        }
        {
            int seen = (int)mrz_bcast64((int64_t)ready, 63);
            if (seen > C.n_helpers) seen = C.n_helpers;
            if (seen > *C.gnw) *C.gnw = seen;
        }
        PROF_ADD(MRZ_ST_F_WAIT);
        ST_ADD(MRZ_ST_FARMED, 1);
        if (lane < MRZ_FARM_ENTRIES) B->farm_min[lane] = MRZ_FARM_NONE;
        MRZ_WAVE_SYNC();
#pragma unroll
        for (int j = 0; j < MRZ_FARM_WATCH; j++) {
            const unsigned long long off = val[j] & MRZ_FARM_PAYLOAD;
            if (watch[j] && off != MRZ_FARM_NONE) atomicMin(&B->farm_min[colw[j]], off);
        }
        MRZ_WAVE_SYNC();
        const unsigned long long m = mine ? B->farm_min[my_col] : MRZ_FARM_NONE;
        const bool resolved = mine && m != MRZ_FARM_NONE;
        if (resolved) fwd = (int64_t)m;
        if (watch_rev) rev = (int64_t)(rv & MRZ_FARM_PAYLOAD);
        pending &= ~__ballot(resolved);
        base += (int64_t)G * mult * MRZ_FARM_SPW;
        want_rev = false;
        rounds++;
        PROF_ADD(MRZ_ST_F_FOLD);
    }
    *my_fwd = fwd;
    *my_rev = rev;
    return true;
}

__device__ __forceinline__ void mrz_farm_census(const mrz_cfg &C) {
    if (C.gmb && *C.gnw >= 0 && *C.gnw < C.n_helpers) {
        int seen = (int)mrz_uni64((int64_t)mrz_g_loadu(&C.gmb->ready));
        if (seen > C.n_helpers) seen = C.n_helpers;
        *C.gnw = seen;
    }
}
#endif

__device__ static bool mrz_resolve_entries(const mrz_cfg &C, mrz_lead &L, mrz_coop_lds *B,
                                           int64_t qx, int nsx, int lane, int64_t *stat,
                                           int64_t *xb, int64_t *xoff, int64_t *xrev, int *xh, int *xm) {
    const uint8_t *__restrict__ buf = C.buf;
    int my_r = 0;
    int64_t my_op = 0, my_ml = 0, my_rv = 0;
    if (lane < nsx) {
        my_r = B->pair_res[lane];
        my_op = B->same_off[lane];
    }
    const mrz_u64 longmask = __ballot(lane < nsx && my_r < 0);
    const int nlong = __popcll(longmask);
    if (nlong) *C.long_seen = 1;
    const int64_t floor_p = L.last_match > 0 ? L.last_match : 0;
    bool farmed = false;
#if MRZ_HELPER_WGS > 0
    if (nlong && C.gmb && nsx <= MRZ_FARM_ENTRIES) {
        mrz_farm_census(C);
        if (*C.gnw >= 2 * MRZ_FARM_ENTRIES && (nlong >= 2 || *C.farm_hint >= MRZ_FARM_HINT_MIN)) {
            int64_t fw, rv;
            if (mrz_farm(C, B, qx, C.end - qx, floor_p, 0, nsx, my_op, my_r < 0 && my_op < qx, true, lane, stat, &fw,
                         &rv)) {
                if (my_r < 0) {
                    my_ml = my_op < qx ? fw + rv : 0;
                    my_rv = rv;
                    if (my_ml < MRZ_MIN_MATCH) my_ml = 0;
                }
                farmed = true;
            }
        }
    }
#endif
    if (!farmed) {
        for (int k = 0; k < nsx; k++) {
            if (!((longmask >> k) & 1)) continue;
            const int64_t op = mrz_bcast64(my_op, k);
            int64_t rv = 0, cont = 0;
            int64_t ml = mrz_long_match_len(buf, C.mb, C.mb_seq, qx, op, C.end, L.last_match, &rv, lane, stat,
#if MRZ_HELPER_WGS > 0
                                            (C.gmb && *C.gnw >= MRZ_FARM_ENTRIES) ? &cont : nullptr
#else
                                            nullptr
#endif
            );
#if MRZ_HELPER_WGS > 0
            if (ml < 0) {
                int64_t fw, dummy;
                if (mrz_farm(C, B, qx, C.end - qx, floor_p, cont, 1, op, true, false, lane, stat, &fw, &dummy)) {
                    fw = mrz_bcast64(fw, 0);
                    ml = fw + rv;
                    if (ml < MRZ_MIN_MATCH) ml = 0;
                } else
                    ml = mrz_long_match_len(buf, C.mb, C.mb_seq, qx, op, C.end, L.last_match, &rv, lane, stat, nullptr);
            }
#endif
            if (lane == k) {
                my_ml = ml;
                my_rv = rv;
            }
        }
    }
    if (lane < nsx && my_r >= 0) {
        my_ml = my_r >> 8;
        my_rv = my_r & 0xff;
    }
#if MRZ_HELPER_WGS > 0
    if (nlong) {
        int64_t far = 0;
        for (int k = 0; k < nsx; k++)
            if ((longmask >> k) & 1) {
                const int64_t v = mrz_bcast64(my_ml, k);
                if (v > far) far = v;
            }
        *C.farm_hint = far;
    }
#endif
    for (int k = 0; k < nsx; k++) {
        const int64_t ml = mrz_bcast64(my_ml, k);
        if (ml) {
            if (ml > *xb) {
                const int64_t rv = mrz_bcast64(my_rv, k);
                *xb = ml;
                *xoff = mrz_bcast64(my_op, k) - rv;
                *xrev = rv;
            }
            *xh += 1;
        } else
            *xm += 1;
    }
    return true;
}

__device__ static bool mrz_seq_candidate(const mrz_cfg &C, mrz_lead &L, mrz_coop_lds *B, int64_t t, int lane,
                                         int64_t *stat) {
    const uint8_t *__restrict__ buf = C.buf;
    mrz_slot *tab = C.tab;
    const int64_t p = L.p, end = C.end, slot_mask = C.slot_mask, max_chain = C.max_chain;
    PROF_T0();
    const bool do_insert = (t & L.tag_mask) == L.tag_mask;
    const int64_t better = (L.min_mask << 1) | 1;
    const int my_rank = mrz_ones_rank(t);
    if (lane == 0) {
        B->n_written = 0;
        B->cull_slot = -1;
    }
    int64_t mlen = 0, m_off = 0, m_rev = 0;
    bool ins_found = !do_insert;
    int64_t ins_slot = 0, occ_t = 0, occ_off = 0;
    int ins_kind = 0;
    if (do_insert) {
        L.inserts++;
        L.count++;
    }
    {
        const int64_t h0 = t & slot_mask;
        int64_t round = 0, victim_h = 0;
        for (int64_t b = 0;; b += MRZ_WAVE) {
            const int64_t s = (h0 + b + lane) & slot_mask;
            const mrz_slot e = tab[s];
            const bool empty = (e.off | e.t) == 0;
            const mrz_u64 m_empty = __ballot(empty);
            const int first_empty = m_empty ? __ffsll((long long)m_empty) - 1 : MRZ_WAVE;
            PROF_ADD(MRZ_ST_S_TAB);
            if (!ins_found)
                ins_found = mrz_insert_step(e, empty, t, my_rank, h0 + b, slot_mask, better, max_chain, &round,
                                            &victim_h, &L.count, &L.victim_round, &ins_slot, &ins_kind, &occ_t,
                                            &occ_off);
            const mrz_u64 m_same = __ballot(!empty && e.t == t) & mrz_low_mask(first_empty);
            mrz_u64 todo = m_same;
            while (todo) {
                const int my_idx = __popcll(todo & mrz_low_mask(lane));
                const bool is_mine = ((todo >> lane) & 1) && my_idx < MRZ_SMAX;
                if (is_mine) B->same_off[my_idx] = e.off;
                const int total = __popcll(todo);
                const int npass = total < MRZ_SMAX ? total : MRZ_SMAX;
                mrz_u64 rest = todo;
                for (int k = 0; k < npass; k++) rest &= rest - 1;
                MRZ_WAVE_SYNC();
                if (lane < npass) {
                    int64_t ml, rv;
                    bool lng;
                    mrz_lane_match_len(buf, p, B->same_off[lane], end, L.last_match, &ml, &rv, &lng);
                    B->pair_res[lane] = lng ? -1 : (int)((ml << 8) | rv);
                }
                MRZ_WAVE_SYNC();
                PROF_ADD(MRZ_ST_S_PAIR);
                int xh = 0, xm = 0;
                if (!mrz_resolve_entries(C, L, B, p, npass, lane, stat, &mlen, &m_off, &m_rev, &xh, &xm))
                    return false;
                L.tag_hits += xh;
                L.tag_misses += xm;
#ifdef MRZ_DBG_HITS_COOP
                if (lane == 0) MRZ_DBG_HITS_COOP(p, xh, xm);
#endif
                todo = rest;
                PROF_T0R();
            }
            if (first_empty < MRZ_WAVE) break;
        }
    }

    PROF_T0R();
    if (do_insert) {
        int np = 0;
        int64_t it = t, io = p;
        while (true) {
            if (np >= MRZ_CASCADE_MAX) {
                if (lane == 0) C.st->error = 2;
                return false;
            }
            if (lane == 0) {
                B->pend_h[np] = ins_slot;
                B->pend_t[np] = it;
                B->pend_o[np] = io;
            }
            np++;
            if (ins_kind != 2) break;
            it = occ_t;
            io = occ_off;
            const int64_t h0 = it & slot_mask;
            const int rank2 = mrz_ones_rank(it);
            int64_t round = 0, victim_h = 0;
            for (int64_t b = 0;; b += MRZ_WAVE) {
                const int64_t s = (h0 + b + lane) & slot_mask;
                const mrz_slot e = tab[s];
                const bool empty = (e.off | e.t) == 0;
                if (mrz_insert_step(e, empty, it, rank2, h0 + b, slot_mask, better, max_chain, &round, &victim_h,
                                    &L.count, &L.victim_round, &ins_slot, &ins_kind, &occ_t, &occ_off))
                    break;
            }
        }
        if (lane == 0) B->n_written = np;
        while (np-- > 0) {
            const int64_t hs = mrz_uni64(B->pend_h[np]);
            if (lane == 0) {
                mrz_slot w;
                w.off = B->pend_o[np];
                w.t = B->pend_t[np];
                tab[hs] = w;
            }
        }
        if (L.count > C.limit) {
            mrz_cull_one(C, L, lane);
            if (lane == 0) B->cull_slot = L.clean_ptr;
        }
    }
    const bool okk = mrz_select_emit(C, L, mlen, m_off, m_rev, lane);
    PROF_ADD(MRZ_ST_S_INS);
    return okk;
}
```

### modern-rzip_amd/csrc/mrz_seq_deep.hip

```cpp
#ifndef MRZ_DEEP_WAVES
#define MRZ_DEEP_WAVES 8
#endif
#define MRZ_SEQ_WAVES MRZ_DEEP_WAVES
#include "mrz_seq_common.h"
#include <cstddef>

#ifndef MRZ_DEEP_LANES
#define MRZ_DEEP_LANES 256
#endif
#ifndef MRZ_DEEP_GROUP
#define MRZ_DEEP_GROUP 8
#endif
#define MRZ_DEEP_THREADS (64 * MRZ_DEEP_WAVES)
#ifdef __HIP_DEVICE_COMPILE__
#define MRZ_DEEP_WAIT() asm volatile("s_waitcnt vmcnt(0)" ::: "memory")
#else
#define MRZ_DEEP_WAIT() ((void)0)
#endif
#define MRZ_DEEP_MAP 2048
#define MRZ_DEEP_CW_WORDS 32
#define MRZ_DEEP_XW 192

enum { MRZ_DK_NONE = 255, MRZ_DK_EMPTY = 0, MRZ_DK_OVER = 1, MRZ_DK_DISPLACE = 2, MRZ_DK_EVICT = 3 };
#define MRZ_DF_INS 1
#define MRZ_DF_CPLX 2
#define MRZ_DF_STALE 4
#define MRZ_DF_FE2 8
#define MRZ_DS_COOP 1
#define MRZ_DS_CONFLICT 2
#define MRZ_DS_CULLED 4
#define MRZ_DS_NOCULL 8

struct mrz_deep_recs {
    int64_t q[MRZ_DEEP_LANES], t[MRZ_DEEP_LANES];
    int64_t occ_t[MRZ_DEEP_LANES], occ_off[MRZ_DEEP_LANES];
    int64_t old_t[MRZ_DEEP_LANES], old_t2[MRZ_DEEP_LANES];
    int64_t cp_scan[MRZ_DEEP_LANES];
    int64_t alt_old_t[MRZ_DEEP_LANES];
    int alt_w[MRZ_DEEP_LANES];
    int h[MRZ_DEEP_LANES], fe[MRZ_DEEP_LANES], w[MRZ_DEEP_LANES], h2[MRZ_DEEP_LANES], w2[MRZ_DEEP_LANES];
    unsigned short xw_seen[MRZ_DEEP_LANES];
    unsigned char kind[MRZ_DEEP_LANES], kind2[MRZ_DEEP_LANES], nsame[MRZ_DEEP_LANES], flags[MRZ_DEEP_LANES];
    unsigned char alt_kind[MRZ_DEEP_LANES];
    int same_slot[MRZ_DEEP_LANES][MRZ_SMAX];
    int64_t same_off[MRZ_DEEP_LANES][MRZ_SMAX];
    unsigned short raw[MRZ_DEEP_LANES][MRZ_SMAX];
};

struct mrz_deep_lds {
    mrz_lead lead;
    int ctl[16];
    int wsum[MRZ_DEEP_WAVES], wsum2[MRZ_DEEP_WAVES], wmin[MRZ_DEEP_WAVES], wmin2[MRZ_DEEP_WAVES], wmin3[MRZ_DEEP_WAVES];
    int n_rescan;
    mrz_deep_recs R;
    int idx[MRZ_DEEP_LANES];
    int cmin[MRZ_DEEP_LANES];
    int cpos[MRZ_DEEP_LANES];
    int xw_n;
    int xw_slot[MRZ_DEEP_XW];
    unsigned short rescan_list[MRZ_DEEP_LANES];
    unsigned smap_key[MRZ_DEEP_MAP];
    int smap_lane[MRZ_DEEP_MAP];
    unsigned long long tmap_key[MRZ_DEEP_MAP];
    int tmap_lane[MRZ_DEEP_MAP];
    mrz_u64 cw[MRZ_DEEP_CW_WORDS];
    int cwcum[MRZ_DEEP_CW_WORDS + 1];
#ifdef MRZ_SEQ_STATS
    int64_t stat[MRZ_ST_N], stat_unused[MRZ_ST_N];
#endif
    mrz_coop_lds coop;
};

__device__ __forceinline__ bool mrz_deep_ranges_meet(int a, int la, int b, int lb, int smask) {
    return la > 0 && lb > 0 && ((((b - a) & smask) < la) || (((a - b) & smask) < lb));
}

__device__ static unsigned mrz_deep_probe_raw(const uint8_t *__restrict__ buf, int64_t q, int64_t op, int64_t end) {
    if (op >= q) return 0;
    int64_t maxf = end - q;
    if (maxf < 0) maxf = 0;
    const int64_t last_ok = end + (MRZ_MIN_MATCH - 16);
    uint4 fa[4], fb[4], ba[4], bb[4];
#pragma unroll
    for (int j = 0; j < 4; j++) {
        int64_t pa = q + j * 16, pb = op + j * 16;
        pa = pa < last_ok ? pa : last_ok;
        pb = pb < last_ok ? pb : last_ok;
        fa[j] = mrz_ld16(buf + pa);
        fb[j] = mrz_ld16(buf + pb);
        int64_t ra = q - (j + 1) * 16, rb = op - (j + 1) * 16;
        ra = ra > 0 ? ra : 0;
        rb = rb > 0 ? rb : 0;
        ba[j] = mrz_ld16(buf + ra);
        bb[j] = mrz_ld16(buf + rb);
    }
    int rawf;
    {
        const int d0 = mrz_first_diff16_bf(fa[0], fb[0]), d1 = mrz_first_diff16_bf(fa[1], fb[1]);
        const int d2 = mrz_first_diff16_bf(fa[2], fb[2]), d3 = mrz_first_diff16_bf(fa[3], fb[3]);
        rawf = d0 < 16 ? d0 : 16 + (d1 < 16 ? d1 : 16 + (d2 < 16 ? d2 : 16 + d3));
    }
    const int fwd = rawf < maxf ? rawf : (int)maxf;
    const unsigned lngf = (rawf == 64 && maxf > 64) ? 1u : 0u;
    const int edge = op < 64 ? (int)(op >> 4) : 4;
    int rawb;
    {
        const int e0 = edge > 0 ? mrz_top_equal16_bf(ba[0], bb[0]) : 16, e1 = edge > 1 ? mrz_top_equal16_bf(ba[1], bb[1]) : 16;
        const int e2 = edge > 2 ? mrz_top_equal16_bf(ba[2], bb[2]) : 16, e3 = edge > 3 ? mrz_top_equal16_bf(ba[3], bb[3]) : 16;
        rawb = e0 < 16 ? e0 : 16 + (e1 < 16 ? e1 : 16 + (e2 < 16 ? e2 : 16 + e3));
    }
    return (unsigned)fwd | (lngf << 7) | ((unsigned)rawb << 8);
}

__device__ __forceinline__ int mrz_deep_pair_eval(unsigned raw, int64_t q, int64_t op, int64_t floor_p) {
    if (op >= q) return 0;
    const int fwd = (int)(raw & 127u), rawb = (int)((raw >> 8) & 127u);
    int64_t maxb = q - floor_p;
    if (op < maxb) maxb = op;
    if (maxb < 0) maxb = 0;
    const int edge = op < 64 ? (int)(op >> 4) : 4;
    if (((raw >> 7) & 1u) || (rawb == 64 && maxb > 64) || (edge < 4 && rawb >= 16 * edge && maxb > 16 * edge)) return 1;
    const int rv = rawb < maxb ? rawb : (int)maxb;
    return fwd + rv >= MRZ_MIN_MATCH ? 1 : 0;
}

__device__ __forceinline__ unsigned mrz_deep_hs(unsigned x) { return (x * 2654435761u) >> (32 - 11); }
static_assert(MRZ_DEEP_MAP == 2048, "mrz_deep_hs gives 11 bits");
static_assert(MRZ_DEEP_LANES * 4 <= MRZ_DEEP_MAP * 3 / 4 || MRZ_DEEP_LANES <= 256, "the maps hold a batch's writes");

__device__ static void mrz_deep_smap_put(mrz_deep_lds *S, int slot, int lane_no) {
    const unsigned key = (unsigned)slot + 1u;
    unsigned i = mrz_deep_hs(key);
    for (int n = 0; n < MRZ_DEEP_MAP; n++) {
        const unsigned k = atomicCAS(&S->smap_key[i], 0u, key);
        if (k == 0u || k == key) {
            atomicMin(&S->smap_lane[i], lane_no);
            return;
        }
        i = (i + 1) & (MRZ_DEEP_MAP - 1);
    }
}
__device__ static int mrz_deep_smap_get(const mrz_deep_lds *S, int slot) {
    if (slot < 0) return 0x7fffffff;
    const unsigned key = (unsigned)slot + 1u;
    unsigned i = mrz_deep_hs(key);
    for (int n = 0; n < MRZ_DEEP_MAP; n++) {
        const unsigned k = S->smap_key[i];
        if (k == 0u) return 0x7fffffff;
        if (k == key) return S->smap_lane[i];
        i = (i + 1) & (MRZ_DEEP_MAP - 1);
    }
    return 0;
}
__device__ static void mrz_deep_tmap_put(mrz_deep_lds *S, int64_t tag, int lane_no) {
    if (tag == 0) return;
    const unsigned long long key = (unsigned long long)tag;
    unsigned i = mrz_deep_hs((unsigned)(key ^ (key >> 23)));
    for (int n = 0; n < MRZ_DEEP_MAP; n++) {
        const unsigned long long k = atomicCAS(&S->tmap_key[i], 0ull, key);
        if (k == 0ull || k == key) {
            atomicMin(&S->tmap_lane[i], lane_no);
            return;
        }
        i = (i + 1) & (MRZ_DEEP_MAP - 1);
    }
}
__device__ static int mrz_deep_tmap_get(const mrz_deep_lds *S, int64_t tag) {
    if (tag == 0) return 0x7fffffff;
    const unsigned long long key = (unsigned long long)tag;
    unsigned i = mrz_deep_hs((unsigned)(key ^ (key >> 23)));
    for (int n = 0; n < MRZ_DEEP_MAP; n++) {
        const unsigned long long k = S->tmap_key[i];
        if (k == 0ull) return 0x7fffffff;
        if (k == key) return S->tmap_lane[i];
        i = (i + 1) & (MRZ_DEEP_MAP - 1);
    }
    return 0;
}

__device__ __forceinline__ int mrz_deep_cw_slot(const mrz_deep_lds *S, int64_t cw_base, int r) {
    int lo = 0, hi = MRZ_DEEP_CW_WORDS - 1;
#pragma unroll
    for (int it = 0; it < 5; it++) {
        const int mid = (lo + hi + 1) >> 1;
        if (S->cwcum[mid] <= r)
            lo = mid;
        else
            hi = mid - 1;
    }
    return (int)(cw_base + lo * 64 + mrz_select64(S->cw[lo], r - S->cwcum[lo]));
}
static_assert(MRZ_DEEP_CW_WORDS == 32, "mrz_deep_cw_slot searches 32 words in 5 steps");

__device__ static void mrz_deep_scan(const mrz_cfg &C, mrz_deep_lds *S, int i, int64_t better, int64_t tag_mask,
                                     int64_t clean_ptr, int xw_n, int lane, int from = 0) {
    const mrz_slot *tab = C.tab;
    const uint8_t *__restrict__ buf = C.buf;
    const int smask = (int)C.slot_mask;
    const int max_chain = (int)C.max_chain;
    const int64_t q = mrz_uni64(S->R.q[i]), t = mrz_uni64(S->R.t[i]);
    const bool ins = (t & tag_mask) == tag_mask;
    const int my_rank = mrz_ones_rank(t);
    const int h = (int)(t & C.slot_mask);
    int fe = -1, w = -1, kind = ins ? -1 : MRZ_DK_NONE;
    int nsame = 0, round = 0;
    bool cplx = false;
    int64_t occ_t = 0, occ_off = 0, old_t = 0;
    bool cont = false, insert_kept = false, fe2 = false;
    int nsame0 = 0;
    int alt_w = -1, alt_kind = MRZ_DK_NONE, alt_st = 0, alt_round = 0;
    int64_t alt_old_t = 0;
    if (from > 0) {
        const int f0 = mrz_uni((int)S->R.flags[i]), k0 = mrz_uni((int)S->R.kind[i]);
        const int ns0 = mrz_uni((int)S->R.nsame[i]);
        if (!(f0 & MRZ_DF_CPLX) && k0 != MRZ_DK_EVICT && k0 != MRZ_DK_DISPLACE && from <= ((mrz_uni(S->R.fe[i]) - h) & smask)) {
            cont = true;
            const bool before = lane < ns0 && ((S->R.same_slot[i][lane < MRZ_SMAX ? lane : 0] - h) & smask) < from;
            nsame0 = nsame = __popcll(__ballot(before));
            if (ins && (k0 == MRZ_DK_EMPTY || k0 == MRZ_DK_OVER) && ((mrz_uni(S->R.w[i]) - h) & smask) < from) {
                insert_kept = true;
                kind = k0;
                w = mrz_uni(S->R.w[i]);
                old_t = mrz_uni64(S->R.old_t[i]);
            } else
                round = nsame;
        }
    }
    const int start = cont ? from : 0;
    const int max_groups = (int)((C.nslots + 64 * MRZ_DEEP_GROUP - 1) / (64 * MRZ_DEEP_GROUP)) + 1;
    for (int grp = 0; fe < 0; grp++) {
        if (grp >= max_groups) {
            cplx = true;
            fe = h;
            break;
        }
        mrz_slot e[MRZ_DEEP_GROUP];
        const int s0 = h + start + grp * (64 * MRZ_DEEP_GROUP) + lane;
#pragma unroll
        for (int g = 0; g < MRZ_DEEP_GROUP; g++) e[g] = tab[(s0 + g * 64) & smask];
#pragma unroll
        for (int g = 0; g < MRZ_DEEP_GROUP; g++) {
            if (fe >= 0) continue;
            const int sb = s0 - lane + g * 64;
            const bool empty = (e[g].off | e[g].t) == 0;
            const mrz_u64 m_empty = __ballot(empty);
            const int fe_idx = m_empty ? __ffsll((long long)m_empty) - 1 : 64;
            const mrz_u64 valid = mrz_low_mask(fe_idx);
            const mrz_u64 m_same = __ballot(!empty && e[g].t == t) & valid;
            mrz_u64 m_due = 0, m_low = 0;
            if (kind == -1 || alt_st == 1) {
                m_due = __ballot(!empty && (e[g].t & better) != better) & valid;
                m_low = __ballot(!empty && mrz_ones_rank(e[g].t) < my_rank) & valid & ~m_due;
            }
            int alt_from = 0;
            if (kind == -1) {
                const mrz_u64 m_stop = m_due | m_low;
                const int ks = m_stop ? __ffsll((long long)m_stop) - 1 : 64;
                const int nq = __popcll(m_same & mrz_low_mask(ks));
                if (round + nq >= max_chain) {
                    kind = MRZ_DK_EVICT;
                } else {
                    round += nq;
                    if (ks < 64) {
                        w = (sb + ks) & smask;
                        if ((m_due >> ks) & 1) {
                            kind = MRZ_DK_OVER;
                            old_t = mrz_bcast64(e[g].t, ks);
                            alt_st = 1;
                            alt_from = ks + 1;
                            alt_round = round;
                        } else {
                            kind = MRZ_DK_DISPLACE;
                            occ_t = mrz_bcast64(e[g].t, ks);
                            occ_off = mrz_bcast64(e[g].off, ks);
                        }
                    } else if (fe_idx < 64) {
                        w = (sb + fe_idx) & smask;
                        kind = MRZ_DK_EMPTY;
                        if (fe_idx < 63 && ((m_empty >> (fe_idx + 1)) & 1)) {
                            alt_w = (sb + fe_idx + 1) & smask;
                            alt_kind = MRZ_DK_EMPTY;
                        }
                        alt_st = 2;
                    }
                }
            }
            if (alt_st == 1 && alt_from < 64) {
                const mrz_u64 beyond = ~mrz_low_mask(alt_from);
                const mrz_u64 m_stop2 = (m_due | m_low) & beyond;
                const int ks2 = m_stop2 ? __ffsll((long long)m_stop2) - 1 : 64;
                const int nq2 = __popcll(m_same & beyond & mrz_low_mask(ks2));
                if (alt_round + nq2 >= max_chain)
                    alt_st = 2;
                else {
                    alt_round += nq2;
                    if (ks2 < 64) {
                        if ((m_due >> ks2) & 1) {
                            alt_w = (sb + ks2) & smask;
                            alt_kind = MRZ_DK_OVER;
                            alt_old_t = mrz_bcast64(e[g].t, ks2);
                        }
                        alt_st = 2;
                    } else if (fe_idx < 64) {
                        alt_w = (sb + fe_idx) & smask;
                        alt_kind = MRZ_DK_EMPTY;
                        alt_st = 2;
                    }
                }
            }
            if (m_same) {
                if ((m_same >> lane) & 1) {
                    const int k = nsame + __popcll(m_same & mrz_low_mask(lane));
                    if (k < MRZ_SMAX) {
                        S->R.same_slot[i][k] = (sb + lane) & smask;
                        S->R.same_off[i][k] = e[g].off;
                    }
                }
                nsame += __popcll(m_same);
            }
            if (fe_idx < 64) {
                fe = (sb + fe_idx) & smask;
                fe2 = fe_idx < 63 && ((m_empty >> (fe_idx + 1)) & 1);
            }
        }
    }
    if (nsame > MRZ_SMAX) cplx = true;
    if (kind == MRZ_DK_EVICT && max_chain > MRZ_SMAX) cplx = true;
    int h2 = 0, w2 = -1, kind2 = MRZ_DK_NONE;
    int64_t old_t2 = 0;
    if (kind == MRZ_DK_DISPLACE && !cplx) {
        const int rank2 = mrz_ones_rank(occ_t);
        h2 = (int)(occ_t & C.slot_mask);
        int round2 = 0;
        bool done = false;
        for (int grp = 0; !done; grp++) {
            if (grp >= max_groups) {
                cplx = true;
                break;
            }
            mrz_slot e[MRZ_DEEP_GROUP];
            const int s0 = h2 + grp * (64 * MRZ_DEEP_GROUP) + lane;
#pragma unroll
            for (int g = 0; g < MRZ_DEEP_GROUP; g++) e[g] = tab[(s0 + g * 64) & smask];
#pragma unroll
            for (int g = 0; g < MRZ_DEEP_GROUP; g++) {
                if (done) continue;
                const int sb = s0 - lane + g * 64;
                const bool empty = (e[g].off | e[g].t) == 0;
                const bool due = !empty && (e[g].t & better) != better;
                const bool low = !empty && !due && mrz_ones_rank(e[g].t) < rank2;
                const mrz_u64 m_empty = __ballot(empty), m_due = __ballot(due), m_low = __ballot(low);
                const mrz_u64 m_stop = m_empty | m_due | m_low;
                const int ks = m_stop ? __ffsll((long long)m_stop) - 1 : 64;
                const int nq = __popcll(__ballot(!empty && !due && !low && e[g].t == occ_t) & mrz_low_mask(ks));
                if (round2 + nq >= max_chain) {
                    cplx = true;
                    done = true;
                } else if (ks < 64) {
                    if ((m_low >> ks) & 1)
                        cplx = true;
                    else {
                        w2 = (sb + ks) & smask;
                        kind2 = ((m_empty >> ks) & 1) ? MRZ_DK_EMPTY : MRZ_DK_OVER;
                        if (kind2 == MRZ_DK_OVER) old_t2 = mrz_bcast64(e[g].t, ks);
                    }
                    done = true;
                } else
                    round2 += nq;
            }
        }
    }
    const int ns = nsame < MRZ_SMAX ? nsame : MRZ_SMAX;
    if (ns > nsame0) {
        MRZ_WAVE_SYNC();
        if (lane >= nsame0 && lane < ns) S->R.raw[i][lane] = (unsigned short)mrz_deep_probe_raw(buf, q, S->R.same_off[i][lane], C.end);
    }
    if (lane == 0) {
        S->R.h[i] = h;
        S->R.fe[i] = fe;
        S->R.w[i] = w;
        S->R.kind[i] = (unsigned char)(kind < 0 ? MRZ_DK_NONE : kind);
        S->R.h2[i] = h2;
        S->R.w2[i] = w2;
        S->R.kind2[i] = (unsigned char)kind2;
        S->R.occ_t[i] = occ_t;
        S->R.occ_off[i] = occ_off;
        S->R.old_t[i] = old_t;
        S->R.old_t2[i] = old_t2;
        S->R.alt_w[i] = (cplx || kind == MRZ_DK_DISPLACE || kind == MRZ_DK_EVICT || insert_kept) ? -1 : alt_w;
        S->R.alt_kind[i] = (unsigned char)alt_kind;
        S->R.alt_old_t[i] = alt_old_t;
        S->R.nsame[i] = (unsigned char)ns;
        S->R.flags[i] = (unsigned char)((ins ? MRZ_DF_INS : 0) | (cplx ? MRZ_DF_CPLX : 0) | (fe2 ? MRZ_DF_FE2 : 0));
        if (!cont) {
            S->R.cp_scan[i] = clean_ptr;
            S->R.xw_seen[i] = (unsigned short)xw_n;
        }
    }
}

#ifndef MRZ_DEEP_SCANNERS
#define MRZ_DEEP_SCANNERS 63
#endif
#ifndef MRZ_DEEP_HELP_MIN
#define MRZ_DEEP_HELP_MIN 48
#endif

struct mrz_deep_shared {
    unsigned long long seq;
    unsigned long long quit;
    unsigned long long n_ok;
    unsigned long long xcc_plus1;
    unsigned long long pad0[12];
    long long nb, nscan, better, tag_mask, clean_ptr, xw_n;
    long long pad1[10];
    unsigned long long done;
    unsigned long long pad2[15];
    mrz_deep_recs R;
};

#ifdef __HIP_DEVICE_COMPILE__
#define MRZ_DEEP_ACQUIRE() __builtin_amdgcn_fence(__ATOMIC_ACQUIRE, "agent")
#define MRZ_DEEP_RELEASE() __builtin_amdgcn_fence(__ATOMIC_RELEASE, "agent")
#define MRZ_DEEP_XCC_ID() (__builtin_amdgcn_s_getreg(20 | (0 << 6) | (3 << 11)) & 15)
#else
#define MRZ_DEEP_ACQUIRE() ((void)0)
#define MRZ_DEEP_RELEASE() ((void)0)
#define MRZ_DEEP_XCC_ID() 0
#endif

__device__ __forceinline__ void mrz_deep_rec_copy(mrz_deep_recs *dst, const mrz_deep_recs *src, int i) {
    dst->occ_t[i] = src->occ_t[i];
    dst->occ_off[i] = src->occ_off[i];
    dst->old_t[i] = src->old_t[i];
    dst->old_t2[i] = src->old_t2[i];
    dst->cp_scan[i] = src->cp_scan[i];
    dst->alt_old_t[i] = src->alt_old_t[i];
    dst->alt_w[i] = src->alt_w[i];
    dst->alt_kind[i] = src->alt_kind[i];
    dst->h[i] = src->h[i];
    dst->fe[i] = src->fe[i];
    dst->w[i] = src->w[i];
    dst->h2[i] = src->h2[i];
    dst->w2[i] = src->w2[i];
    dst->xw_seen[i] = src->xw_seen[i];
    dst->kind[i] = src->kind[i];
    dst->kind2[i] = src->kind2[i];
    dst->flags[i] = src->flags[i];
    const int ns = src->nsame[i];
    dst->nsame[i] = (unsigned char)ns;
    for (int k = 0; k < ns; k++) {
        dst->same_slot[i][k] = src->same_slot[i][k];
        dst->same_off[i][k] = src->same_off[i][k];
        dst->raw[i][k] = src->raw[i][k];
    }
}


__device__ static void mrz_deep_scan_helper(const mrz_cfg &C, mrz_deep_lds *S, mrz_deep_shared *G, int tid, int lane, int wave) {
    if (tid == 0) {
        long long spins = 0;
        unsigned long long x = 0;
        while ((x = __hip_atomic_load(&G->xcc_plus1, __ATOMIC_RELAXED, __HIP_MEMORY_SCOPE_AGENT)) == 0 &&
               !__hip_atomic_load(&G->quit, __ATOMIC_RELAXED, __HIP_MEMORY_SCOPE_AGENT) && spins++ < (1ll << 24))
            __builtin_amdgcn_s_sleep(8);
        int ticket = -1;
        if (x != 0)
            ticket = (int)__hip_atomic_fetch_add(&G->n_ok, 1ull, __ATOMIC_RELAXED, __HIP_MEMORY_SCOPE_AGENT);
        S->ctl[0] = ticket;
    }
    __syncthreads();
    const int ticket = mrz_uni(S->ctl[0]);
    if (ticket < 0 || ticket >= MRZ_DEEP_SCANNERS) return;
    const int me = ticket + 1;
    unsigned long long seen = 0;
    while (true) {
        if (tid == 0) {
            long long spins = 0;
            unsigned long long sq = 0;
            int v = 1;
            while (true) {
                sq = __hip_atomic_load(&G->seq, __ATOMIC_RELAXED, __HIP_MEMORY_SCOPE_AGENT);
                if (sq != seen) break;
                if (__hip_atomic_load(&G->quit, __ATOMIC_RELAXED, __HIP_MEMORY_SCOPE_AGENT) || spins++ > MRZ_HELPER_SPIN_LIMIT) {
                    v = 0;
                    break;
                }
                __builtin_amdgcn_s_sleep(2);
            }
            MRZ_DEEP_ACQUIRE();
            S->ctl[1] = v;
            S->lead.p = (int64_t)sq;
        }
        __syncthreads();
        if (!mrz_uni(S->ctl[1])) return;
        seen = (unsigned long long)mrz_uni64(S->lead.p);
        const int nb = (int)G->nb, nscan = (int)G->nscan, xw_n = (int)G->xw_n;
        const int64_t better = G->better, tag_mask = G->tag_mask, clean_ptr = G->clean_ptr;
        int mine_n = 0;
        if (me < nscan) {
            for (int i = me + tid * nscan; i < nb; i += nscan * MRZ_DEEP_THREADS) {
                S->R.q[i] = G->R.q[i];
                S->R.t[i] = G->R.t[i];
            }
            __syncthreads();
            int k = 0;
            for (int i = me; i < nb; i += nscan, k++)
                if (k % MRZ_DEEP_WAVES == wave) mrz_deep_scan(C, S, i, better, tag_mask, clean_ptr, xw_n, lane);
            mine_n = k;
            __syncthreads();
            for (int i = me + tid * nscan; i < nb; i += nscan * MRZ_DEEP_THREADS) mrz_deep_rec_copy(&G->R, &S->R, i);
            MRZ_DEEP_WAIT();
        }
        __syncthreads();
        if (tid == 0 && mine_n) {
            MRZ_DEEP_RELEASE();
            __hip_atomic_fetch_add(&G->done, (unsigned long long)mine_n, __ATOMIC_RELEASE, __HIP_MEMORY_SCOPE_AGENT);
        }
    }
}

__device__ static __attribute__((noinline)) bool mrz_deep_coop(const mrz_cfg &C, mrz_lead &L, mrz_coop_lds *B, int64_t t,
                                                               int lane, int64_t *stat) {
    return mrz_seq_candidate(C, L, B, t, lane, stat);
}

__device__ static __attribute__((noinline)) bool mrz_deep_candidate_rec(const mrz_cfg &C, mrz_lead &L, mrz_deep_lds *S, int i, int *xw_n, int lane,
                                              int64_t *stat) {
    mrz_coop_lds *B = &S->coop;
    const int64_t q = mrz_uni64(S->R.q[i]), t = mrz_uni64(S->R.t[i]);
    const int ns = mrz_uni((int)S->R.nsame[i]);
    const int f = mrz_uni((int)S->R.flags[i]);
    int64_t mlen = 0, m_off = 0, m_rev = 0;
    L.p = q;
    if (ns) {
        if (lane < ns) {
            const int64_t op = S->R.same_off[i][lane];
            B->same_off[lane] = op;
            int64_t ml, rv;
            bool lng;
            mrz_lane_match_len(C.buf, q, op, C.end, L.last_match, &ml, &rv, &lng);
            B->pair_res[lane] = lng ? -1 : (int)((ml << 8) | rv);
        }
        MRZ_WAVE_SYNC();
        int xh = 0, xm = 0;
        if (!mrz_resolve_entries(C, L, B, q, ns, lane, stat, &mlen, &m_off, &m_rev, &xh, &xm)) return false;
        L.tag_hits += xh;
        L.tag_misses += xm;
    }
    int nx = *xw_n;
    if (f & MRZ_DF_INS) {
        const int kind = mrz_uni((int)S->R.kind[i]);
        L.inserts++;
        L.count++;
        int ws = mrz_uni(S->R.w[i]);
        if (kind == MRZ_DK_OVER)
            L.count--;
        else if (kind == MRZ_DK_EVICT) {
            L.count--;
            ws = mrz_uni(S->R.same_slot[i][(int)L.victim_round]);
            L.victim_round = L.victim_round + 1 == C.max_chain ? 0 : L.victim_round + 1;
        } else if (kind == MRZ_DK_DISPLACE) {
            const int w2 = mrz_uni(S->R.w2[i]);
            if (mrz_uni((int)S->R.kind2[i]) == MRZ_DK_OVER) L.count--;
            if (lane == 0) {
                mrz_slot oc;
                oc.off = S->R.occ_off[i];
                oc.t = S->R.occ_t[i];
                C.tab[w2] = oc;
                S->xw_slot[nx] = w2;
            }
            nx++;
        }
        if (lane == 0) {
            mrz_slot nw;
            nw.off = q;
            nw.t = t;
            C.tab[ws] = nw;
            S->xw_slot[nx] = ws;
        }
        nx++;
        if (L.count > C.limit) {
            MRZ_DEEP_WAIT();
            mrz_cull_one(C, L, lane);
            if (lane == 0) S->xw_slot[nx] = (int)L.clean_ptr;
            nx++;
        }
    }
    *xw_n = nx;
    return mrz_select_emit(C, L, mlen, m_off, m_rev, lane);
}

__device__ __forceinline__ int mrz_deep_incl(int v, int *ws, int lane, int wave, int *total) {
    const int incl = mrz_wave_incl_sum(v, lane);
    if (lane == 63) ws[wave] = incl;
    __syncthreads();
    int add = 0, tot = 0;
#pragma unroll
    for (int w = 0; w < MRZ_DEEP_WAVES; w++) {
        const int x = ws[w];
        tot += x;
        if (w < wave) add += x;
    }
    *total = tot;
    return incl + add;
}

__device__ __forceinline__ int mrz_deep_first(bool flag, int *wm, int lane, int wave, int tid, int none) {
    const mrz_u64 m = __ballot(flag);
    if (lane == 0) wm[wave] = m ? wave * 64 + (__ffsll((long long)m) - 1) : none;
    __syncthreads();
    int r = none;
#pragma unroll
    for (int w = 0; w < MRZ_DEEP_WAVES; w++) r = wm[w] < r ? wm[w] : r;
    return r;
}

__global__ __launch_bounds__(MRZ_DEEP_THREADS) void mrz_seq_deep_kernel(mrz_seq_args a, mrz_deep_shared *G, int scanners) {
#ifdef MRZ_EMU_LDS_PER_BLOCK
    static mrz_deep_lds deep_all[1 + 15];
    mrz_deep_lds *S = &deep_all[(blockIdx.x / 8) % (1 + 15)];
#else
    __shared__ mrz_deep_lds deep;
    mrz_deep_lds *S = &deep;
#endif
    const int tid = (int)threadIdx.x;
    const int lane = tid & 63;
    const int wave = mrz_uni(tid >> 6);
    mrz_seq_state *st = a.st;
    if (st->finished || st->error) return;
    const int xcd = a.xcd & 7;
    const int bx = (int)blockIdx.x;
    const bool is_seq = bx == xcd;
#ifdef MRZ_EMU_LDS_PER_BLOCK
    const bool is_scanner = G != nullptr && !is_seq && bx % 8 == xcd && bx / 8 >= 1 && bx / 8 <= scanners && bx / 8 <= MRZ_DEEP_SCANNERS;
#else
    const bool is_scanner = G != nullptr && !is_seq && (bx < xcd ? bx : bx - 1) < scanners && scanners <= MRZ_DEEP_SCANNERS;
#endif
#if MRZ_HELPER_WGS > 0
    if (!is_seq && !is_scanner) {
        if (a.gmailbox) mrz_helper_wg(a.buf, (mrz_gmailbox *)a.gmailbox);
        return;
    }
#else
    if (!is_seq && !is_scanner) return;
#endif
    mrz_cfg C;
    C.buf = a.buf;
    C.tab = a.tab;
    C.events = a.events;
    C.st = st;
    C.end = st->end;
    C.limit = st->limit;
    C.max_chain = st->max_chain;
    C.slot_mask = st->slot_mask;
    C.nslots = st->slot_mask + 1;
    C.event_cap = st->event_cap;
    C.ev_base = st->ev_base;
    C.gmb = (mrz_gmailbox *)a.gmailbox;
    unsigned long long gseq = 0;
    C.gseq = &gseq;
    int gnw = 0;
    C.gnw = &gnw;
    C.n_helpers = a.n_helpers;
    int64_t farm_hint = 0;
    C.farm_hint = &farm_hint;
    int long_seen = 0;
    C.long_seen = &long_seen;
    C.mb = nullptr;
    C.mb_seq = nullptr;
    mrz_cands K;
    K.cand = a.cand;
    K.tile_off = a.tile_off;
    K.bitmap = a.bitmap;
    K.seg_start = st->seg_start;
    K.seg_end = st->seg_end;
    K.n = st->n_cand;
    if (is_scanner) {
        mrz_deep_scan_helper(C, S, G, tid, lane, wave);
        return;
    }
    if (K.seg_end <= K.seg_start) {
        if (tid == 0 && G) __hip_atomic_store(&G->quit, 1ull, __ATOMIC_RELAXED, __HIP_MEMORY_SCOPE_AGENT);
#if MRZ_HELPER_WGS > 0
        if (tid == 0 && C.gmb) mrz_g_storeu(&C.gmb->quit, 1ull);
#endif
        return;
    }
    if (tid == 0 && G) __hip_atomic_store(&G->xcc_plus1, (unsigned long long)MRZ_DEEP_XCC_ID() + 1ull, __ATOMIC_RELAXED, __HIP_MEMORY_SCOPE_AGENT);
    unsigned long long batch_seq = 0;
    const int64_t lim = (C.end < K.seg_end - 1) ? C.end : K.seg_end - 1;
    const int smask = (int)C.slot_mask;
    const int max_chain = (int)C.max_chain;
#ifdef MRZ_SEQ_STATS
    for (int k = tid; k < MRZ_ST_N; k += MRZ_DEEP_THREADS) S->stat[k] = 0;
    __syncthreads();
    int64_t *stat = tid == 0 ? S->stat : S->stat_unused;
#else
    int64_t *stat = nullptr;
#endif

    mrz_lead L;
    L.p = st->p;
    L.cur_p = st->cur_p;
    L.cur_ofs = st->cur_ofs;
    L.cur_len = st->cur_len;
    L.last_match = st->last_match;
    L.min_mask = st->min_mask;
    L.tag_mask = st->tag_mask;
    L.count = st->count;
    L.clean_ptr = st->clean_ptr;
    L.victim_round = st->victim_round;
    L.n_events = st->n_events;
    L.inserts = st->inserts;
    L.tag_hits = st->tag_hits;
    L.tag_misses = st->tag_misses;
    L.last_len = 0;
    L.mbytes = 0;
    const int64_t hint_p0 = L.p, hint_ev0 = L.n_events;

    int64_t ci;
    {
        int64_t pos = L.p + 1;
        if (pos < K.seg_start) pos = K.seg_start;
        ci = mrz_cand_lower_bound(K, pos, lane);
    }
    bool ok = true;
    PROF_T0();
#ifdef MRZ_SEQ_PROFILE
    const int64_t launch_t0 = (int64_t)__builtin_amdgcn_s_memtime();
#endif
    ST_ADD(MRZ_ST_D_LAUNCHES, 1);
    while (ok && ci < K.n && L.p < lim) {
        PROF_T0R();
        const int64_t better = (L.min_mask << 1) | 1;
        const bool loose = L.tag_mask != better;
        int64_t my_q = 0, my_t = 0;
        bool live = false;
        if (ci + tid < K.n) {
            const mrz_cand c = K.cand[ci + tid];
            my_q = c.off;
            my_t = c.t;
            live = c.off > L.p && c.off <= lim && (c.t & L.min_mask) == L.min_mask;
        }
        int total;
        const int incl = mrz_deep_incl(live ? 1 : 0, S->wsum, lane, wave, &total);
        const int at = incl - 1;
        if (live && at < MRZ_DEEP_LANES) {
            S->R.q[at] = my_q;
            S->R.t[at] = my_t;
            S->idx[at] = (int)(ci + tid);
        }
        const int nb = total < MRZ_DEEP_LANES ? total : MRZ_DEEP_LANES;
        int64_t n_examined = K.n - ci < MRZ_DEEP_THREADS ? K.n - ci : MRZ_DEEP_THREADS;
        __syncthreads();
        if (total > MRZ_DEEP_LANES) n_examined = (int64_t)S->idx[MRZ_DEEP_LANES - 1] + 1 - ci;
        if (nb == 0) {
            ci += n_examined;
            __syncthreads();
            continue;
        }
        ST_ADD(MRZ_ST_D_BATCHES, 1);
        ST_ADD(MRZ_ST_D_LANES, nb);
        PROF_ADD(MRZ_ST_D_T_FORM);
        if (!loose) {
            int nscan = 1;
            if (G && nb >= MRZ_DEEP_HELP_MIN) {
                int nh = (int)mrz_uni64((int64_t)__hip_atomic_load(&G->n_ok, __ATOMIC_RELAXED, __HIP_MEMORY_SCOPE_AGENT));
                if (nh > MRZ_DEEP_SCANNERS) nh = MRZ_DEEP_SCANNERS;
                if (nh > scanners) nh = scanners;
                nscan = 1 + nh;
            }
            int helper_lanes = 0;
            if (nscan > 1) {
                if (tid < nb) {
                    G->R.q[tid] = S->R.q[tid];
                    G->R.t[tid] = S->R.t[tid];
                }
                if (tid == 0) {
                    G->nb = nb;
                    G->nscan = nscan;
                    G->better = better;
                    G->tag_mask = L.tag_mask;
                    G->clean_ptr = L.clean_ptr;
                    G->xw_n = 0;
                    __hip_atomic_store(&G->done, 0ull, __ATOMIC_RELAXED, __HIP_MEMORY_SCOPE_AGENT);
                }
                MRZ_DEEP_WAIT();
                __syncthreads();
                batch_seq++;
                if (tid == 0) {
                    MRZ_DEEP_RELEASE();
                    __hip_atomic_store(&G->seq, batch_seq, __ATOMIC_RELEASE, __HIP_MEMORY_SCOPE_AGENT);
                }
                helper_lanes = nb - (nb + nscan - 1) / nscan;
            }
            {
                int k = 0;
                for (int i = 0; i < nb; i += nscan, k++)
                    if (k % MRZ_DEEP_WAVES == wave) mrz_deep_scan(C, S, i, better, L.tag_mask, L.clean_ptr, 0, lane);
            }
            if (nscan > 1) {
                if (tid == 0) {
                    long long spins = 0;
                    while (__hip_atomic_load(&G->done, __ATOMIC_ACQUIRE, __HIP_MEMORY_SCOPE_AGENT) < (unsigned long long)helper_lanes &&
                           spins++ < (1ll << 26))
                        __builtin_amdgcn_s_sleep(1);
                    S->ctl[6] = spins < (1ll << 26) ? 1 : 0;
                    MRZ_DEEP_ACQUIRE();
                }
                __syncthreads();
                if (!mrz_uni(S->ctl[6])) {
                    if (tid == 0) C.st->error = 7;
                    ok = false;
                } else if (tid < nb && tid % nscan != 0)
                    mrz_deep_rec_copy(&S->R, &G->R, tid);
            }
        }
        __syncthreads();
        PROF_ADD(MRZ_ST_D_T_SCAN);
        for (int k = tid; k < MRZ_DEEP_MAP; k += MRZ_DEEP_THREADS) {
            S->smap_key[k] = 0u;
            S->smap_lane[k] = 0x7fffffff;
            S->tmap_key[k] = 0ull;
            S->tmap_lane[k] = 0x7fffffff;
        }
        __syncthreads();
        int next = 0;
        bool cut = false;
        int xw_n = 0;
        while (next < nb && !cut && ok) {
            const int i = tid;
            const bool mine = i >= next && i < nb;
            const int round_start = next;
            int coop_lane = -1;
            bool use_record = false;
            if (loose || L.cur_len > 0) {
                coop_lane = next;
            } else {
                const int64_t cw_base = L.clean_ptr;
                const bool load_cw = L.count + (nb - next) > C.limit;
                constexpr int CW_PER_WAVE = (MRZ_DEEP_CW_WORDS + MRZ_DEEP_WAVES - 1) / MRZ_DEEP_WAVES;
                mrz_slot cwe[CW_PER_WAVE];
#pragma unroll
                for (int b = 0; b < CW_PER_WAVE; b++) {
                    cwe[b].off = 0;
                    cwe[b].t = 0;
                    const int wi = b * MRZ_DEEP_WAVES + wave;
                    const int64_t slot = cw_base + (int64_t)wi * 64 + lane;
                    if (load_cw && wi < MRZ_DEEP_CW_WORDS && slot < C.nslots) cwe[b] = C.tab[slot];
                }
                const int f = mine ? S->R.flags[i] : 0;
                const bool ins = mine && (f & MRZ_DF_INS), cplx = mine && (f & MRZ_DF_CPLX);
                const int kind = mine ? S->R.kind[i] : MRZ_DK_NONE, kind2 = mine ? S->R.kind2[i] : MRZ_DK_NONE;
                const int64_t q = mine ? S->R.q[i] : 0, t = mine ? S->R.t[i] : 0;
                const int w = mine ? S->R.w[i] : -1, w2 = mine ? S->R.w2[i] : -1, fe = mine ? S->R.fe[i] : -1;
                const int h = mine ? S->R.h[i] : 0, h2 = mine ? S->R.h2[i] : 0;
                const int64_t occ_t = mine ? S->R.occ_t[i] : 0;
                const bool wr_w = ins && !cplx && (kind == MRZ_DK_EMPTY || kind == MRZ_DK_OVER || kind == MRZ_DK_DISPLACE);
                const bool wr_w2 = ins && !cplx && kind == MRZ_DK_DISPLACE;
                if (ins && !cplx) {
                    if (wr_w) mrz_deep_smap_put(S, w, i);
                    if (wr_w2) mrz_deep_smap_put(S, w2, i);
                    mrz_deep_tmap_put(S, t, i);
                    if (kind == MRZ_DK_OVER) mrz_deep_tmap_put(S, S->R.old_t[i], i);
                    if (kind == MRZ_DK_DISPLACE) {
                        mrz_deep_tmap_put(S, occ_t, i);
                        if (kind2 == MRZ_DK_OVER) mrz_deep_tmap_put(S, S->R.old_t2[i], i);
                    }
                }
                __syncthreads();
                int res = 0, res_x = -1;
                int w_e = w, kind_e = kind, fe_e = fe;
                if (mine && !cplx && !(f & MRZ_DF_STALE) && kind != MRZ_DK_DISPLACE) {
                    const int m_t = mrz_deep_tmap_get(S, t);
                    const int m_fe = mrz_deep_smap_get(S, fe);
                    const int m_w = wr_w ? mrz_deep_smap_get(S, w) : 0x7fffffff;
                    const bool c_w = wr_w && m_w < i, c_fe = m_fe < i;
                    if (m_t >= i && (c_w || c_fe)) {
                        bool can = true;
                        const int aw = S->R.alt_w[i], ak = S->R.alt_kind[i];
                        if (c_w) {
                            const int x = m_w;
                            res_x = x;
                            const int kx = S->R.kind[x];
                            can = aw >= 0 && S->R.w[x] == w && (kx == MRZ_DK_EMPTY || kx == MRZ_DK_OVER) &&
                                  mrz_ones_rank(S->R.t[x]) >= mrz_ones_rank(t);
                            res |= 1;
                            if (kind == MRZ_DK_EMPTY) res |= 2;
                        }
                        if (c_fe && !(res & 2)) {
                            can = can && (f & MRZ_DF_FE2) && !((res & 1) && ak == MRZ_DK_EMPTY);
                            res |= 2;
                        }
                        if (!can) res = 0;
                    }
                    if (res & 1) {
                        w_e = S->R.alt_w[i];
                        kind_e = S->R.alt_kind[i];
                        mrz_deep_smap_put(S, w_e, i);
                        if (kind_e == MRZ_DK_OVER) mrz_deep_tmap_put(S, S->R.alt_old_t[i], i);
                    }
                    if (res & 2) fe_e = (fe + 1) & smask;
                }
                __syncthreads();
                int cmin = 0x7fffffff;
                int cfrom = 0x7fffffff;
                int stop = 0;
                const int cw_len = MRZ_DEEP_CW_WORDS * 64;
                if (mine) {
                    if (cplx)
                        stop |= MRZ_DS_COOP;
                    else {
                        int m;
                        bool hard = false;
                        m = mrz_deep_smap_get(S, fe);
                        cmin = m < cmin ? m : cmin;
                        if (m < i) {
                            cfrom = (fe - h) & smask;
                            if (!(res & 2)) hard = true;
                        }
                        m = mrz_deep_tmap_get(S, t);
                        if (m != i) cmin = m < cmin ? m : cmin;
                        if (m < i) {
                            cfrom = 0;
                            hard = true;
                        }
                        if (wr_w) {
                            m = mrz_deep_smap_get(S, w);
                            if (m != i) cmin = m < cmin ? m : cmin;
                            if (m < i) {
                                const int pw_ = (w - h) & smask;
                                cfrom = pw_ < cfrom ? pw_ : cfrom;
                                if (!(res & 1) || m != res_x) hard = true;
                            }
                        }
                        if (wr_w2) {
                            m = mrz_deep_smap_get(S, w2);
                            if (m != i) cmin = m < cmin ? m : cmin;
                            if (m < i) {
                                cfrom = 0;
                                hard = true;
                            }
                            m = mrz_deep_tmap_get(S, occ_t);
                            if (m != i) cmin = m < cmin ? m : cmin;
                            if (m < i) {
                                cfrom = 0;
                                hard = true;
                            }
                        }
                        if ((res & 1) && mrz_deep_smap_get(S, w_e) < i) hard = true;
                        if ((res & 2) && mrz_deep_smap_get(S, fe_e) < i) hard = true;
                        if (hard || (f & MRZ_DF_STALE)) stop |= MRZ_DS_CONFLICT;
                        const int ns = S->R.nsame[i];
                        const int64_t floor_p = L.last_match > 0 ? L.last_match : 0;
                        for (int k = 0; k < ns; k++)
                            if (mrz_deep_pair_eval(S->R.raw[i][k], q, S->R.same_off[i][k], floor_p)) stop |= MRZ_DS_COOP;
                        if (wr_w && kind_e == MRZ_DK_OVER && w_e >= cw_base && w_e < cw_base + cw_len) stop |= MRZ_DS_COOP;
                        if (wr_w2 && kind2 == MRZ_DK_OVER && w2 >= cw_base && w2 < cw_base + cw_len) stop |= MRZ_DS_COOP;
                        for (int k = S->R.xw_seen[i]; k < xw_n; k++) {
                            const int xs = S->xw_slot[k];
                            if ((((xs - h) & smask) <= ((fe_e - h) & smask)) || (wr_w2 && (((xs - h2) & smask) <= ((w2 - h2) & smask))))
                                stop |= MRZ_DS_CULLED;
                        }
                        const int64_t cp0 = S->R.cp_scan[i];
                        if (L.clean_ptr != cp0) {
                            const int lc = (int)(L.clean_ptr - cp0) + 1;
                            if (mrz_deep_ranges_meet(h, ((fe_e - h) & smask) + 1, (int)cp0, lc, smask)) stop |= MRZ_DS_CULLED;
                            if (wr_w2 && mrz_deep_ranges_meet(h2, ((w2 - h2) & smask) + 1, (int)cp0, lc, smask)) stop |= MRZ_DS_CULLED;
                        }
                    }
                    S->cmin[i] = cmin;
                }
                int e1 = mrz_deep_first(mine && stop != 0, S->wmin, lane, wave, tid, nb);
                for (int k = tid; k < MRZ_DEEP_MAP; k += MRZ_DEEP_THREADS) {
                    S->smap_key[k] = 0u;
                    S->smap_lane[k] = 0x7fffffff;
                    S->tmap_key[k] = 0ull;
                    S->tmap_lane[k] = 0x7fffffff;
                }
#pragma unroll
                for (int b = 0; b < CW_PER_WAVE; b++) {
                    const int wi = b * MRZ_DEEP_WAVES + wave;
                    const mrz_u64 m = __ballot(((cwe[b].off | cwe[b].t) != 0) && ((cwe[b].t & better) != better));
                    if (lane == 0 && wi < MRZ_DEEP_CW_WORDS) S->cw[wi] = m;
                }
                __syncthreads();
                if (wave == 0) {
                    const int c = lane < MRZ_DEEP_CW_WORDS ? __popcll(S->cw[lane]) : 0;
                    const int cinc = mrz_wave_incl_sum(c, lane);
                    if (lane < MRZ_DEEP_CW_WORDS) S->cwcum[lane + 1] = cinc;
                    if (lane == 0) S->cwcum[0] = 0;
                }
                __syncthreads();
                const int cw_total = S->cwcum[MRZ_DEEP_CW_WORDS];
                const bool inb = mine && i < e1;
                const bool a_ins = inb && ins;
                const bool a_ev = a_ins && kind == MRZ_DK_EVICT;
                const int d = a_ins ? (kind_e == MRZ_DK_EMPTY ? 1 : (kind == MRZ_DK_DISPLACE ? (kind2 == MRZ_DK_EMPTY ? 1 : 0) : 0)) : 0;
                int dummy;
                const int i1 = mrz_deep_incl(d | (a_ev ? 1 << 10 : 0) | (a_ins ? 1 << 20 : 0), S->wsum, lane, wave, &dummy);
                int64_t c_before = L.count + ((i1 & 1023) - d);
                if (c_before > C.limit) c_before = C.limit;
                const bool cull = a_ins && (c_before + d > C.limit);
                const int i2 = mrz_deep_incl((cull ? 1 : 0) | ((inb ? (int)S->R.nsame[i] : 0) << 10), S->wsum2, lane, wave, &dummy);
                int cslot = -1;
                const int r_before = (i2 & 1023) - (cull ? 1 : 0);
                if (cull) {
                    if (r_before >= cw_total)
                        stop |= MRZ_DS_NOCULL;
                    else
                        cslot = mrz_deep_cw_slot(S, cw_base, r_before);
                }
                if (inb && !cplx && r_before > 0) {
                    const int rr = r_before - 1 < cw_total ? r_before - 1 : cw_total - 1;
                    if (rr >= 0) {
                        const int lc = (int)(mrz_deep_cw_slot(S, cw_base, rr) - cw_base) + 1;
                        if (mrz_deep_ranges_meet(h, ((fe_e - h) & smask) + 1, (int)cw_base, lc, smask) ||
                            (wr_w2 && mrz_deep_ranges_meet(h2, ((w2 - h2) & smask) + 1, (int)cw_base, lc, smask)))
                            stop |= MRZ_DS_CULLED;
                    }
                }
                const int e2 = mrz_deep_first(inb && stop != 0, S->wmin2, lane, wave, tid, e1);
                if (mine && i == e2) S->ctl[4] = stop;
                if (mine && i >= e2 && cmin < e2) {
                    const int old = (f & MRZ_DF_STALE) ? S->cpos[i] : 0x7fffffff;
                    S->cpos[i] = cfrom < old ? cfrom : old;
                    S->R.flags[i] = (unsigned char)(f | MRZ_DF_STALE);
                }
                if (mine && i < e2) {
                    if (a_ins) {
                        int ws = w_e;
                        if (a_ev) {
                            const int er = ((i1 >> 10) & 1023) - 1;
                            const int vr = (int)(((unsigned)L.victim_round + (unsigned)er) % (unsigned)max_chain);
                            ws = S->R.same_slot[i][vr];
                        }
                        if (kind == MRZ_DK_DISPLACE) {
                            mrz_slot oc;
                            oc.off = S->R.occ_off[i];
                            oc.t = occ_t;
                            C.tab[w2] = oc;
                        }
                        mrz_slot nw;
                        nw.off = q;
                        nw.t = t;
                        C.tab[ws] = nw;
                        if (cslot >= 0) {
                            mrz_slot z;
                            z.off = 0;
                            z.t = 0;
                            C.tab[cslot] = z;
                        }
                    }
                }
                if (e2 > next && tid == e2 - 1) {
                    mrz_lead N = L;
                    int64_t c_after = c_before + d;
                    if (c_after > C.limit) c_after = C.limit;
                    N.count = c_after;
                    N.inserts = L.inserts + ((i1 >> 20) & 1023);
                    N.victim_round = (int64_t)(((unsigned)L.victim_round + (unsigned)((i1 >> 10) & 1023)) % (unsigned)max_chain);
                    N.tag_misses = L.tag_misses + (i2 >> 10);
                    N.p = q;
                    S->lead = N;
                }
                {
                    const bool is_c = mine && i < e2 && cslot >= 0;
                    const mrz_u64 mc = __ballot(is_c);
                    int wl = -1;
                    if (mc) wl = mrz_lane_read(cslot, 63 - __clzll((long long)mc));
                    if (lane == 0) S->wsum2[wave] = wl;
                }
                MRZ_DEEP_WAIT();
                __syncthreads();
                if (e2 > next) {
                    L = S->lead;
                    int lastc = -1;
#pragma unroll
                    for (int wv = 0; wv < MRZ_DEEP_WAVES; wv++) lastc = S->wsum2[wv] > lastc ? S->wsum2[wv] : lastc;
                    if (lastc >= 0) L.clean_ptr = lastc;
                }
                ST_ADD(MRZ_ST_COMMITTED, e2 - next);
                next = e2;
                PROF_ADD(MRZ_ST_D_T_COMMIT);
                if (next < nb) {
                    const int sf = mrz_uni(S->ctl[4]);
                    ST_ADD(MRZ_ST_D_S_COOP, (sf & MRZ_DS_COOP) ? 1 : 0);
                    ST_ADD(MRZ_ST_D_S_CONFLICT, (sf & MRZ_DS_CONFLICT) ? 1 : 0);
                    ST_ADD(MRZ_ST_D_S_CULLED, (sf & MRZ_DS_CULLED) ? 1 : 0);
                    ST_ADD(MRZ_ST_D_S_NOCULL, (sf & MRZ_DS_NOCULL) ? 1 : 0);
                    ST_ADD(MRZ_ST_D_S_STALE, (S->R.flags[next] & MRZ_DF_STALE) ? 1 : 0);
                    if ((sf & MRZ_DS_CONFLICT) && !(sf & MRZ_DS_COOP)) {
                        const int kk = S->R.kind[next];
                        (void)kk;
                        ST_ADD(MRZ_ST_D_C_OVER_ALT, (kk == MRZ_DK_OVER && S->R.alt_w[next] >= 0) ? 1 : 0);
                        ST_ADD(MRZ_ST_D_C_OVER_NOALT, (kk == MRZ_DK_OVER && S->R.alt_w[next] < 0) ? 1 : 0);
                        ST_ADD(MRZ_ST_D_C_EMPTY, kk == MRZ_DK_EMPTY ? 1 : 0);
                        ST_ADD(MRZ_ST_D_C_DISPLACE, kk == MRZ_DK_DISPLACE ? 1 : 0);
                        ST_ADD(MRZ_ST_D_C_OTHER, (kk == MRZ_DK_NONE || kk == MRZ_DK_EVICT) ? 1 : 0);
                    }
                    bool stop_stale = (sf & (MRZ_DS_CONFLICT | MRZ_DS_CULLED)) != 0 || (S->R.flags[next] & MRZ_DF_STALE);
                    if (!stop_stale && !(S->R.flags[next] & MRZ_DF_CPLX)) {
                        const int64_t cp0 = S->R.cp_scan[next];
                        if (L.clean_ptr != cp0) {
                            const int lc = (int)(L.clean_ptr - cp0) + 1;
                            const int hh = S->R.h[next], ff = S->R.fe[next];
                            stop_stale = mrz_deep_ranges_meet(hh, ((ff - hh) & smask) + 1, (int)cp0, lc, smask);
                            if (!stop_stale && (S->R.flags[next] & MRZ_DF_INS) && S->R.kind[next] == MRZ_DK_DISPLACE) {
                                const int hh2 = S->R.h2[next], ww2 = S->R.w2[next];
                                stop_stale = mrz_deep_ranges_meet(hh2, ((ww2 - hh2) & smask) + 1, (int)cp0, lc, smask);
                            }
                        }
                    }
                    if ((sf & MRZ_DS_COOP) && !stop_stale) {
                        coop_lane = next;
                        use_record = !(S->R.flags[next] & MRZ_DF_CPLX);
                    } else if ((sf & MRZ_DS_NOCULL) && next == round_start && !stop_stale) {
                        coop_lane = next;
                        use_record = !(S->R.flags[next] & MRZ_DF_CPLX);
                    } else {
                        bool again = false, by_flag = false;
                        if (i >= next && i < nb && !(S->R.flags[i] & MRZ_DF_CPLX)) {
                            again = (S->R.flags[i] & MRZ_DF_STALE) != 0;
                            by_flag = again;
                            {
                                const int hh = S->R.h[i], ff = S->R.fe[i], hh2 = S->R.h2[i], ww2 = S->R.w2[i];
                                const bool dsp = (S->R.flags[i] & MRZ_DF_INS) && S->R.kind[i] == MRZ_DK_DISPLACE;
                                for (int k = S->R.xw_seen[i]; k < xw_n && !again; k++) {
                                    const int xs = S->xw_slot[k];
                                    again = (((xs - hh) & smask) <= ((ff - hh) & smask)) || (dsp && (((xs - hh2) & smask) <= ((ww2 - hh2) & smask)));
                                }
                            }
                            if (!again) {
                                const int64_t cp0 = S->R.cp_scan[i];
                                if (L.clean_ptr != cp0) {
                                    const int lc = (int)(L.clean_ptr - cp0) + 1;
                                    const int hh = S->R.h[i], ff = S->R.fe[i];
                                    again = mrz_deep_ranges_meet(hh, ((ff - hh) & smask) + 1, (int)cp0, lc, smask);
                                    if (!again && (S->R.flags[i] & MRZ_DF_INS) && S->R.kind[i] == MRZ_DK_DISPLACE) {
                                        const int hh2 = S->R.h2[i], ww2 = S->R.w2[i];
                                        again = mrz_deep_ranges_meet(hh2, ((ww2 - hh2) & smask) + 1, (int)cp0, lc, smask);
                                    }
                                }
                            }
                        }
                        if (again && i >= next && i < nb) {
                            bool other = false;
                            {
                                const int hh = S->R.h[i], ff = S->R.fe[i], hh2 = S->R.h2[i], ww2 = S->R.w2[i];
                                const bool dsp = (S->R.flags[i] & MRZ_DF_INS) && S->R.kind[i] == MRZ_DK_DISPLACE;
                                for (int k = S->R.xw_seen[i]; k < xw_n && !other; k++) {
                                    const int xs = S->xw_slot[k];
                                    other = (((xs - hh) & smask) <= ((ff - hh) & smask)) || (dsp && (((xs - hh2) & smask) <= ((ww2 - hh2) & smask)));
                                }
                                const int64_t cp0 = S->R.cp_scan[i];
                                if (!other && L.clean_ptr != cp0) {
                                    const int lc = (int)(L.clean_ptr - cp0) + 1;
                                    other = mrz_deep_ranges_meet(hh, ((ff - hh) & smask) + 1, (int)cp0, lc, smask) ||
                                            (dsp && mrz_deep_ranges_meet(hh2, ((ww2 - hh2) & smask) + 1, (int)cp0, lc, smask));
                                }
                            }
                            if (!by_flag || other) S->cpos[i] = 0;
                        }
                        if (tid == 0) S->n_rescan = 0;
                        __syncthreads();
                        if (again) S->rescan_list[atomicAdd(&S->n_rescan, 1)] = (unsigned short)i;
                        __syncthreads();
                        const int nr = S->n_rescan;
                        ST_ADD(MRZ_ST_D_ROUNDS, 1);
                        ST_ADD(MRZ_ST_D_RESCANNED, nr);
                        for (int k = wave; k < nr; k += MRZ_DEEP_WAVES) {
                            const int li = (int)S->rescan_list[k];
                            const int cf = mrz_uni(S->cpos[li]);
                            mrz_deep_scan(C, S, li, better, L.tag_mask, L.clean_ptr, xw_n, lane, cf == 0x7fffffff ? 0 : cf);
                        }
                        __syncthreads();
                        PROF_ADD(MRZ_ST_D_T_RESCAN);
                    }
                }
            }
            if (coop_lane >= 0) {
                if (wave == 0) {
                    int cl = coop_lane;
                    int verdict = 1, nx = xw_n;
                    while (true) {
                        const int64_t q = mrz_uni64(S->R.q[cl]), t = mrz_uni64(S->R.t[cl]);
                        const int64_t mm0 = L.min_mask, tm0 = L.tag_mask;
                        L.p = q;
                        int nx_rec = nx;
                        const bool rec = use_record && nx + 4 <= MRZ_DEEP_XW;
                        const bool okc = rec ? mrz_deep_candidate_rec(C, L, S, cl, &nx_rec, lane, stat)
                                             : mrz_deep_coop(C, L, &S->coop, t, lane, stat);
                        ST_ADD(MRZ_ST_D_COOP, 1);
                        ST_ADD(MRZ_ST_D_COOP_REC, rec ? 1 : 0);
                        const bool same_masks = L.min_mask == mm0 && L.tag_mask == tm0;
                        const int nwr = rec ? 0 : mrz_uni(S->coop.n_written);
                        const int64_t cs = rec ? -1 : mrz_uni64(S->coop.cull_slot);
                        const bool room = nx + nwr + 1 <= MRZ_DEEP_XW;
                        if (rec)
                            nx = nx_rec;
                        else if (okc && same_masks && room && !loose) {
                            if (lane < nwr) S->xw_slot[nx + lane] = (int)S->coop.pend_h[lane];
                            nx += nwr;
                            if (cs >= 0) {
                                if (lane == 0) S->xw_slot[nx] = (int)cs;
                                nx++;
                            }
                        }
                        verdict = !okc ? 3 : ((same_masks && (room || loose) && L.p >= q) ? 1 : 2);
                        if (!(loose && verdict == 1)) break;
                        int j = cl + 1;
                        while (j < nb && mrz_uni64(S->R.q[j]) <= L.p) j++;
                        if (j >= nb) break;
                        cl = j;
                    }
                    if (lane == 0) {
                        S->lead = L;
                        S->ctl[0] = verdict;
                        S->ctl[5] = nx;
                    }
                    MRZ_DEEP_WAIT();
                }
                __syncthreads();
                L = S->lead;
                xw_n = mrz_uni(S->ctl[5]);
                const int v = mrz_uni(S->ctl[0]);
                if (v == 3) ok = false;
                if (v == 2) cut = true;
                {
                    const int i = tid;
                    const int nf = mrz_deep_first(i > coop_lane && i < nb && S->R.q[i] > L.p, S->wmin3, lane, wave, tid, nb);
                    next = nf;
                }
                PROF_ADD(MRZ_ST_D_T_COOP);
            }
        }
        if (ok) {
            if (cut || L.p > mrz_uni64(S->R.q[nb - 1])) {
                int64_t pos = L.p + 1;
                if (pos < K.seg_start) pos = K.seg_start;
                ci = mrz_cand_lower_bound(K, pos, lane);
            } else
                ci += n_examined;
        }
        __syncthreads();
    }
    if (ok && ci >= K.n && L.p < lim) L.p = lim;
#ifdef MRZ_SEQ_PROFILE
    stat[MRZ_ST_D_T_TOTAL] += (int64_t)__builtin_amdgcn_s_memtime() - launch_t0;
#endif
    if (tid == 0) {
        if (G) __hip_atomic_store(&G->quit, 1ull, __ATOMIC_RELAXED, __HIP_MEMORY_SCOPE_AGENT);
#if MRZ_HELPER_WGS > 0
        if (C.gmb) mrz_g_storeu(&C.gmb->quit, 1ull);
#endif
        st->p = L.p;
        st->cur_p = L.cur_p;
        st->cur_ofs = L.cur_ofs;
        st->cur_len = L.cur_len;
        st->last_match = L.last_match;
        st->min_mask = L.min_mask;
        st->tag_mask = L.tag_mask;
        st->count = L.count;
        st->clean_ptr = L.clean_ptr;
        st->victim_round = L.victim_round;
        st->n_events = L.n_events;
        st->inserts = L.inserts;
        st->tag_hits = L.tag_hits;
        st->tag_misses = L.tag_misses;
        st->finished = L.p >= C.end ? 1 : 0;
        st->hint_positions = L.p - hint_p0;
        st->hint_events = L.n_events - hint_ev0;
        st->hint_matched = L.mbytes;
#ifdef MRZ_SEQ_STATS
        for (int k = 0; k < MRZ_ST_N; k++) st->prof[k] += stat[k];
#endif
    }
}

extern "C" hipError_t mrz_launch_sequencer_deep(hipStream_t stream, const uint8_t *buf, mrz_slot *tab, const mrz_cand *cand,
                                                const int *tile_off, const mrz_u64 *bitmap, mrz_event *events,
                                                mrz_seq_state *st, void *gmailbox, int n_helpers, int xcd, void *deep_shared,
                                                int scanners) {
    mrz_seq_args a;
    a.buf = buf;
    a.tab = tab;
    a.cand = cand;
    a.tile_off = tile_off;
    a.bitmap = bitmap;
    a.events = events;
    a.st = st;
    a.gmailbox = gmailbox;
    a.xcd = xcd & 7;
    a.deep_bits = 0;
#if MRZ_HELPER_WGS == 0
    n_helpers = 0;
#endif
    if (n_helpers > MRZ_HELPER_WGS) n_helpers = MRZ_HELPER_WGS;
    if (n_helpers < 0 || !gmailbox) n_helpers = 0;
    a.n_helpers = n_helpers;
    if (gmailbox) {
        hipError_t e = hipMemsetAsync(gmailbox, 0, sizeof(mrz_gmailbox), stream);
        if (e != hipSuccess) return e;
    }
    if (scanners < 0 || !deep_shared) scanners = 0;
    if (scanners > MRZ_DEEP_SCANNERS) scanners = MRZ_DEEP_SCANNERS;
    unsigned grid = (unsigned)(1 + a.n_helpers);
    if (grid < (unsigned)(a.xcd + 1)) grid = (unsigned)(a.xcd + 1);
#ifdef MRZ_EMU_LDS_PER_BLOCK
    if (scanners > 0) {
        grid = (unsigned)(8 * scanners + a.xcd + 1);
        emu::request_coresident();
    }
#else
    if (scanners > a.n_helpers / 2) scanners = a.n_helpers / 2;
    while (scanners > 0 && grid < (unsigned)(scanners + 2)) scanners--;
#endif
    if (deep_shared) {
        hipError_t e = hipMemsetAsync(deep_shared, 0, offsetof(mrz_deep_shared, R), stream);
        if (e != hipSuccess) return e;
    }
    hipLaunchKernelGGL(mrz_seq_deep_kernel, dim3(grid), dim3(MRZ_DEEP_THREADS), 0, stream, a, (mrz_deep_shared *)deep_shared,
                       scanners);
    return hipGetLastError();
}

extern "C" size_t mrz_seq_deep_shared_size(void) { return sizeof(mrz_deep_shared); }
```

Before: 6.372 GiB/s.

## Double deep sequencer batch to 512 lanes with pooled same-slot storage

Raises the deep sequencer's batch from 256 to 512 lanes, with each thread forming two candidates, and caps the batch at half size when the min mask is wide. Per-lane fixed same-slot arrays in LDS are replaced by a shared pool with per-lane offsets and per-wave staging, so LDS stays bounded as the lane count grows. Helper handshakes now carry a sequence stamp in the done counter and job parameters are snapshotted into LDS. The aim is fewer batch rounds and less per-batch overhead. The cost is more conflict rescans, and lanes whose pool allocation overflows fall back to the complex path.

```diff
diff --git a/modern-rzip_amd/csrc/mrz_capi.hip b/modern-rzip_amd/csrc/mrz_capi.hip
--- a/modern-rzip_amd/csrc/mrz_capi.hip
+++ b/modern-rzip_amd/csrc/mrz_capi.hip
@@ -216,6 +216,8 @@
         if (hipMalloc(&ctx->d_deep_shared, mrz_seq_deep_shared_size()) != hipSuccess) rc = MRZ_E_NOMEM;
         ctx->deep_scanners = 63;
         if (const char *e = getenv("MRZ_DEEP_SCANNERS")) ctx->deep_scanners = atoi(e);
+        if (const char *e = getenv("MRZ_DEEP_BATCH")) ctx->deep_batch = atoi(e);
+        if (const char *e = getenv("MRZ_DEEP_NARROW_BITS")) ctx->deep_narrow_bits = atoi(e);
     }
     if (!rc && max_chunk > 0) {
         rc = mrz_grow(ctx, &ctx->d_events, &ctx->event_cap, mrz_event_room(ctx, max_chunk));
@@ -719,7 +721,7 @@
         else if (deep)
             STEP(mrz_launch_sequencer_deep(s, d_buf, ctx->d_tab, ctx->d_cand, ctx->d_tile_off, (const mrz_u64 *)ctx->d_bitmap,
                                            ctx->d_events, ctx->d_state, ctx->d_gmailbox, helpers, ctx->xcd, ctx->d_deep_shared,
-                                           ctx->deep_scanners));
+                                           ctx->deep_scanners, ctx->deep_batch, ctx->deep_narrow_bits));
         else
             STEP(mrz_launch_sequencer(s, d_buf, ctx->d_tab, ctx->d_cand, ctx->d_tile_off, (const mrz_u64 *)ctx->d_bitmap,
                                       ctx->d_events, ctx->d_state, ctx->d_gmailbox, helpers, ctx->d_seq_shared, ctx->d_wlog,
@@ -811,6 +813,7 @@
     res->min_mask = hs.min_mask;
     res->hash_count = hs.count;
     res->n_events = E;
+    res->reserved = (uint32_t)hs.deep_max_batch;
     if (ctx->print_prof) {
         static const char *names[128] = { "batches", "formed", "committed", "segments", "emits", "backjump", "rewalk",
                                           "longres", "seq_cands", "cut_cplx", "cut_overflow", "skipout", "conf0", "pairs",
diff --git a/modern-rzip_amd/csrc/mrz_common.h b/modern-rzip_amd/csrc/mrz_common.h
--- a/modern-rzip_amd/csrc/mrz_common.h
+++ b/modern-rzip_amd/csrc/mrz_common.h
@@ -44,6 +44,7 @@
     int64_t n_cand;
     int64_t scan_next;
     int64_t list_mask;
+    int64_t deep_max_batch;
     int64_t prof[128];
 };
 
diff --git a/modern-rzip_amd/csrc/mrz_ctx.h b/modern-rzip_amd/csrc/mrz_ctx.h
--- a/modern-rzip_amd/csrc/mrz_ctx.h
+++ b/modern-rzip_amd/csrc/mrz_ctx.h
@@ -61,6 +61,8 @@
     int seq_wgs;
     void *d_deep_shared;
     int deep_scanners;
+    int deep_batch;
+    int deep_narrow_bits;
     int farm_helpers;
     int farm_default;
     void *d_rs_tables;
diff --git a/modern-rzip_amd/csrc/mrz_kernels.h b/modern-rzip_amd/csrc/mrz_kernels.h
--- a/modern-rzip_amd/csrc/mrz_kernels.h
+++ b/modern-rzip_amd/csrc/mrz_kernels.h
@@ -30,7 +30,8 @@
                                        void *gmailbox, int n_helpers, int xcd);
 hipError_t mrz_launch_sequencer_deep(hipStream_t stream, const uint8_t *buf, mrz_slot *tab, const mrz_cand *cand,
                                      const int *tile_off, const mrz_u64 *bitmap, mrz_event *events, mrz_seq_state *st,
-                                     void *gmailbox, int n_helpers, int xcd, void *deep_shared, int scanners);
+                                     void *gmailbox, int n_helpers, int xcd, void *deep_shared, int scanners,
+                                     int batch, int narrow_bits);
 size_t mrz_seq_deep_shared_size(void);
 size_t mrz_sequencer_mailbox_size(void);
 size_t mrz_seq_narrow_mailbox_size(void);
diff --git a/modern-rzip_amd/csrc/mrz_seq_common.h b/modern-rzip_amd/csrc/mrz_seq_common.h
--- a/modern-rzip_amd/csrc/mrz_seq_common.h
+++ b/modern-rzip_amd/csrc/mrz_seq_common.h
@@ -87,6 +87,8 @@
     int n_helpers;
     int xcd;
     int deep_bits;
+    int deep_batch;
+    int deep_narrow_bits;
 };
 
 struct mrz_cands {
diff --git a/modern-rzip_amd/csrc/mrz_seq_deep.hip b/modern-rzip_amd/csrc/mrz_seq_deep.hip
--- a/modern-rzip_amd/csrc/mrz_seq_deep.hip
+++ b/modern-rzip_amd/csrc/mrz_seq_deep.hip
@@ -6,7 +6,13 @@
 #include <cstddef>
 
 #ifndef MRZ_DEEP_LANES
-#define MRZ_DEEP_LANES 256
+#define MRZ_DEEP_LANES 512
+#endif
+#ifndef MRZ_DEEP_POOL
+#define MRZ_DEEP_POOL 1024
+#endif
+#ifndef MRZ_DEEP_NARROW_BITS
+#define MRZ_DEEP_NARROW_BITS 14
 #endif
 #ifndef MRZ_DEEP_GROUP
 #define MRZ_DEEP_GROUP 8
@@ -17,7 +23,8 @@
 #else
 #define MRZ_DEEP_WAIT() ((void)0)
 #endif
-#define MRZ_DEEP_MAP 2048
+#define MRZ_DEEP_MAP_BITS (MRZ_DEEP_LANES > 256 ? 12 : 11)
+#define MRZ_DEEP_MAP (1 << MRZ_DEEP_MAP_BITS)
 #define MRZ_DEEP_CW_WORDS 32
 #define MRZ_DEEP_XW 192
 
@@ -31,7 +38,8 @@
 #define MRZ_DS_CULLED 4
 #define MRZ_DS_NOCULL 8
 
-struct mrz_deep_recs {
+template <int NPOOL>
+struct mrz_deep_recs_t {
     int64_t q[MRZ_DEEP_LANES], t[MRZ_DEEP_LANES];
     int64_t occ_t[MRZ_DEEP_LANES], occ_off[MRZ_DEEP_LANES];
     int64_t old_t[MRZ_DEEP_LANES], old_t2[MRZ_DEEP_LANES];
@@ -42,10 +50,15 @@
     unsigned short xw_seen[MRZ_DEEP_LANES];
     unsigned char kind[MRZ_DEEP_LANES], kind2[MRZ_DEEP_LANES], nsame[MRZ_DEEP_LANES], flags[MRZ_DEEP_LANES];
     unsigned char alt_kind[MRZ_DEEP_LANES];
-    int same_slot[MRZ_DEEP_LANES][MRZ_SMAX];
-    int64_t same_off[MRZ_DEEP_LANES][MRZ_SMAX];
-    unsigned short raw[MRZ_DEEP_LANES][MRZ_SMAX];
+    unsigned short first[MRZ_DEEP_LANES];
+    int pool_n;
+    int64_t pool_off[NPOOL];
+    int pool_slot[NPOOL];
+    unsigned short pool_raw[NPOOL];
 };
+typedef mrz_deep_recs_t<MRZ_DEEP_POOL> mrz_deep_recs;
+typedef mrz_deep_recs_t<MRZ_DEEP_LANES * MRZ_SMAX> mrz_deep_recs_dev;
+static_assert(MRZ_DEEP_LANES * MRZ_SMAX <= 65536 && MRZ_DEEP_POOL <= 65536, "mrz_deep_recs_t::first is 16 bits wide");
 
 struct mrz_deep_lds {
     mrz_lead lead;
@@ -59,6 +72,10 @@
     int xw_n;
     int xw_slot[MRZ_DEEP_XW];
     unsigned short rescan_list[MRZ_DEEP_LANES];
+    int64_t st_off[MRZ_DEEP_WAVES][MRZ_SMAX];
+    int st_slot[MRZ_DEEP_WAVES][MRZ_SMAX];
+    unsigned short st_raw[MRZ_DEEP_WAVES][MRZ_SMAX];
+    long long job[8];
     unsigned smap_key[MRZ_DEEP_MAP];
     int smap_lane[MRZ_DEEP_MAP];
     unsigned long long tmap_key[MRZ_DEEP_MAP];
@@ -124,9 +141,10 @@
     return fwd + rv >= MRZ_MIN_MATCH ? 1 : 0;
 }
 
-__device__ __forceinline__ unsigned mrz_deep_hs(unsigned x) { return (x * 2654435761u) >> (32 - 11); }
-static_assert(MRZ_DEEP_MAP == 2048, "mrz_deep_hs gives 11 bits");
-static_assert(MRZ_DEEP_LANES * 4 <= MRZ_DEEP_MAP * 3 / 4 || MRZ_DEEP_LANES <= 256, "the maps hold a batch's writes");
+__device__ __forceinline__ unsigned mrz_deep_hs(unsigned x) { return (x * 2654435761u) >> (32 - MRZ_DEEP_MAP_BITS); }
+static_assert(MRZ_DEEP_LANES * 3 <= MRZ_DEEP_MAP * 3 / 4, "the maps hold a batch's writes");
+static_assert(MRZ_DEEP_LANES <= MRZ_DEEP_THREADS, "one lane per thread of the committer");
+static_assert(MRZ_DEEP_LANES <= 1023, "the packed prefix sums of a round count lanes in 10-bit fields");
 
 __device__ static void mrz_deep_smap_put(mrz_deep_lds *S, int slot, int lane_no) {
     const unsigned key = (unsigned)slot + 1u;
@@ -193,7 +211,7 @@
 static_assert(MRZ_DEEP_CW_WORDS == 32, "mrz_deep_cw_slot searches 32 words in 5 steps");
 
 __device__ static void mrz_deep_scan(const mrz_cfg &C, mrz_deep_lds *S, int i, int64_t better, int64_t tag_mask,
-                                     int64_t clean_ptr, int xw_n, int lane, int from = 0) {
+                                     int64_t clean_ptr, int xw_n, int lane, int wave, bool again = false, int from = 0) {
     const mrz_slot *tab = C.tab;
     const uint8_t *__restrict__ buf = C.buf;
     const int smask = (int)C.slot_mask;
@@ -208,6 +226,11 @@
     int64_t occ_t = 0, occ_off = 0, old_t = 0;
     bool cont = false, insert_kept = false, fe2 = false;
     int nsame0 = 0;
+    int first0 = 0, room0 = 0;
+    if (again && !(mrz_uni((int)S->R.flags[i]) & MRZ_DF_CPLX)) {
+        first0 = mrz_uni((int)S->R.first[i]);
+        room0 = mrz_uni((int)S->R.nsame[i]);
+    }
     int alt_w = -1, alt_kind = MRZ_DK_NONE, alt_st = 0, alt_round = 0;
     int64_t alt_old_t = 0;
     if (from > 0) {
@@ -215,8 +238,13 @@
         const int ns0 = mrz_uni((int)S->R.nsame[i]);
         if (!(f0 & MRZ_DF_CPLX) && k0 != MRZ_DK_EVICT && k0 != MRZ_DK_DISPLACE && from <= ((mrz_uni(S->R.fe[i]) - h) & smask)) {
             cont = true;
-            const bool before = lane < ns0 && ((S->R.same_slot[i][lane < MRZ_SMAX ? lane : 0] - h) & smask) < from;
+            const bool before = lane < ns0 && ((S->R.pool_slot[first0 + (lane < ns0 ? lane : 0)] - h) & smask) < from;
             nsame0 = nsame = __popcll(__ballot(before));
+            if (lane < nsame0) {
+                S->st_slot[wave][lane] = S->R.pool_slot[first0 + lane];
+                S->st_off[wave][lane] = S->R.pool_off[first0 + lane];
+                S->st_raw[wave][lane] = S->R.pool_raw[first0 + lane];
+            }
             if (ins && (k0 == MRZ_DK_EMPTY || k0 == MRZ_DK_OVER) && ((mrz_uni(S->R.w[i]) - h) & smask) < from) {
                 insert_kept = true;
                 kind = k0;
@@ -312,8 +340,8 @@
                 if ((m_same >> lane) & 1) {
                     const int k = nsame + __popcll(m_same & mrz_low_mask(lane));
                     if (k < MRZ_SMAX) {
-                        S->R.same_slot[i][k] = (sb + lane) & smask;
-                        S->R.same_off[i][k] = e[g].off;
+                        S->st_slot[wave][k] = (sb + lane) & smask;
+                        S->st_off[wave][k] = e[g].off;
                     }
                 }
                 nsame += __popcll(m_same);
@@ -370,10 +398,27 @@
             }
         }
     }
-    const int ns = nsame < MRZ_SMAX ? nsame : MRZ_SMAX;
-    if (ns > nsame0) {
+    int ns = cplx ? 0 : (nsame < MRZ_SMAX ? nsame : MRZ_SMAX);
+    int first = first0;
+    if (ns > room0) {
+        int a = 0;
+        if (lane == 0) a = atomicAdd(&S->R.pool_n, ns);
+        a = mrz_lane_read(a, 0);
+        if (a + ns > MRZ_DEEP_POOL) {
+            cplx = true;
+            ns = 0;
+        } else
+            first = a;
+    }
+    if (ns > 0) {
         MRZ_WAVE_SYNC();
-        if (lane >= nsame0 && lane < ns) S->R.raw[i][lane] = (unsigned short)mrz_deep_probe_raw(buf, q, S->R.same_off[i][lane], C.end);
+        if (lane < ns) {
+            const int64_t op = S->st_off[wave][lane];
+            S->R.pool_slot[first + lane] = S->st_slot[wave][lane];
+            S->R.pool_off[first + lane] = op;
+            S->R.pool_raw[first + lane] = lane < nsame0 ? S->st_raw[wave][lane] : (unsigned short)mrz_deep_probe_raw(buf, q, op, C.end);
+        }
+        MRZ_WAVE_SYNC();
     }
     if (lane == 0) {
         S->R.h[i] = h;
@@ -391,6 +436,7 @@
         S->R.alt_kind[i] = (unsigned char)alt_kind;
         S->R.alt_old_t[i] = alt_old_t;
         S->R.nsame[i] = (unsigned char)ns;
+        S->R.first[i] = (unsigned short)first;
         S->R.flags[i] = (unsigned char)((ins ? MRZ_DF_INS : 0) | (cplx ? MRZ_DF_CPLX : 0) | (fe2 ? MRZ_DF_FE2 : 0));
         if (!cont) {
             S->R.cp_scan[i] = clean_ptr;
@@ -412,11 +458,11 @@
     unsigned long long n_ok;
     unsigned long long xcc_plus1;
     unsigned long long pad0[12];
-    long long nb, nscan, better, tag_mask, clean_ptr, xw_n;
-    long long pad1[10];
+    long long nb, nscan, better, tag_mask, clean_ptr, xw_n, stamp;
+    long long pad1[9];
     unsigned long long done;
     unsigned long long pad2[15];
-    mrz_deep_recs R;
+    mrz_deep_recs_dev R;
 };
 
 #ifdef __HIP_DEVICE_COMPILE__
@@ -429,7 +475,8 @@
 #define MRZ_DEEP_XCC_ID() 0
 #endif
 
-__device__ __forceinline__ void mrz_deep_rec_copy(mrz_deep_recs *dst, const mrz_deep_recs *src, int i) {
+template <int NA, int NB>
+__device__ __forceinline__ void mrz_deep_rec_copy(mrz_deep_recs_t<NA> *dst, const mrz_deep_recs_t<NB> *src, int i, bool take) {
     dst->occ_t[i] = src->occ_t[i];
     dst->occ_off[i] = src->occ_off[i];
     dst->old_t[i] = src->old_t[i];
@@ -446,13 +493,24 @@
     dst->xw_seen[i] = src->xw_seen[i];
     dst->kind[i] = src->kind[i];
     dst->kind2[i] = src->kind2[i];
-    dst->flags[i] = src->flags[i];
-    const int ns = src->nsame[i];
+    int ns = src->nsame[i], f = src->flags[i];
+    int first = i * MRZ_SMAX;
+    if (take && ns > 0) {
+        first = atomicAdd(&dst->pool_n, ns);
+        if (first + ns > NA) {
+            f |= MRZ_DF_CPLX;
+            ns = 0;
+            first = 0;
+        }
+    }
+    dst->flags[i] = (unsigned char)f;
     dst->nsame[i] = (unsigned char)ns;
+    dst->first[i] = (unsigned short)first;
+    const int sf = src->first[i];
     for (int k = 0; k < ns; k++) {
-        dst->same_slot[i][k] = src->same_slot[i][k];
-        dst->same_off[i][k] = src->same_off[i][k];
-        dst->raw[i][k] = src->raw[i][k];
+        dst->pool_slot[first + k] = src->pool_slot[sf + k];
+        dst->pool_off[first + k] = src->pool_off[sf + k];
+        dst->pool_raw[first + k] = src->pool_raw[sf + k];
     }
 }
 
@@ -481,24 +539,35 @@
             int v = 1;
             while (true) {
                 sq = __hip_atomic_load(&G->seq, __ATOMIC_RELAXED, __HIP_MEMORY_SCOPE_AGENT);
-                if (sq != seen) break;
+                if (sq != seen) {
+                    MRZ_DEEP_ACQUIRE();
+                    S->job[0] = __hip_atomic_load(&G->nb, __ATOMIC_RELAXED, __HIP_MEMORY_SCOPE_AGENT);
+                    S->job[1] = __hip_atomic_load(&G->nscan, __ATOMIC_RELAXED, __HIP_MEMORY_SCOPE_AGENT);
+                    S->job[2] = __hip_atomic_load(&G->better, __ATOMIC_RELAXED, __HIP_MEMORY_SCOPE_AGENT);
+                    S->job[3] = __hip_atomic_load(&G->tag_mask, __ATOMIC_RELAXED, __HIP_MEMORY_SCOPE_AGENT);
+                    S->job[4] = __hip_atomic_load(&G->clean_ptr, __ATOMIC_RELAXED, __HIP_MEMORY_SCOPE_AGENT);
+                    S->job[5] = __hip_atomic_load(&G->xw_n, __ATOMIC_RELAXED, __HIP_MEMORY_SCOPE_AGENT);
+                    asm volatile("" ::: "memory");
+                    const long long stamp = __hip_atomic_load(&G->stamp, __ATOMIC_RELAXED, __HIP_MEMORY_SCOPE_AGENT);
+                    if (stamp == (long long)sq) break;
+                }
                 if (__hip_atomic_load(&G->quit, __ATOMIC_RELAXED, __HIP_MEMORY_SCOPE_AGENT) || spins++ > MRZ_HELPER_SPIN_LIMIT) {
                     v = 0;
                     break;
                 }
                 __builtin_amdgcn_s_sleep(2);
             }
-            MRZ_DEEP_ACQUIRE();
             S->ctl[1] = v;
             S->lead.p = (int64_t)sq;
+            S->R.pool_n = 0;
         }
         __syncthreads();
         if (!mrz_uni(S->ctl[1])) return;
         seen = (unsigned long long)mrz_uni64(S->lead.p);
-        const int nb = (int)G->nb, nscan = (int)G->nscan, xw_n = (int)G->xw_n;
-        const int64_t better = G->better, tag_mask = G->tag_mask, clean_ptr = G->clean_ptr;
+        const int nb = (int)mrz_uni64(S->job[0]), nscan = (int)mrz_uni64(S->job[1]), xw_n = (int)mrz_uni64(S->job[5]);
+        const int64_t better = mrz_uni64(S->job[2]), tag_mask = mrz_uni64(S->job[3]), clean_ptr = mrz_uni64(S->job[4]);
         int mine_n = 0;
-        if (me < nscan) {
+        if (me < nscan && nb <= MRZ_DEEP_LANES) {
             for (int i = me + tid * nscan; i < nb; i += nscan * MRZ_DEEP_THREADS) {
                 S->R.q[i] = G->R.q[i];
                 S->R.t[i] = G->R.t[i];
@@ -506,16 +575,18 @@
             __syncthreads();
             int k = 0;
             for (int i = me; i < nb; i += nscan, k++)
-                if (k % MRZ_DEEP_WAVES == wave) mrz_deep_scan(C, S, i, better, tag_mask, clean_ptr, xw_n, lane);
+                if (k % MRZ_DEEP_WAVES == wave) mrz_deep_scan(C, S, i, better, tag_mask, clean_ptr, xw_n, lane, wave);
             mine_n = k;
             __syncthreads();
-            for (int i = me + tid * nscan; i < nb; i += nscan * MRZ_DEEP_THREADS) mrz_deep_rec_copy(&G->R, &S->R, i);
+            for (int i = me + tid * nscan; i < nb; i += nscan * MRZ_DEEP_THREADS) mrz_deep_rec_copy(&G->R, &S->R, i, false);
             MRZ_DEEP_WAIT();
         }
         __syncthreads();
         if (tid == 0 && mine_n) {
             MRZ_DEEP_RELEASE();
-            __hip_atomic_fetch_add(&G->done, (unsigned long long)mine_n, __ATOMIC_RELEASE, __HIP_MEMORY_SCOPE_AGENT);
+            const unsigned long long was =
+                __hip_atomic_fetch_add(&G->done, (unsigned long long)mine_n, __ATOMIC_RELEASE, __HIP_MEMORY_SCOPE_AGENT);
+            if ((was >> 32) != (seen & 0xffffffffull)) __hip_atomic_store(&C.st->error, 8, __ATOMIC_RELAXED, __HIP_MEMORY_SCOPE_AGENT);
         }
     }
 }
@@ -529,13 +600,13 @@
                                               int64_t *stat) {
     mrz_coop_lds *B = &S->coop;
     const int64_t q = mrz_uni64(S->R.q[i]), t = mrz_uni64(S->R.t[i]);
-    const int ns = mrz_uni((int)S->R.nsame[i]);
+    const int ns = mrz_uni((int)S->R.nsame[i]), pf = mrz_uni((int)S->R.first[i]);
     const int f = mrz_uni((int)S->R.flags[i]);
     int64_t mlen = 0, m_off = 0, m_rev = 0;
     L.p = q;
     if (ns) {
         if (lane < ns) {
-            const int64_t op = S->R.same_off[i][lane];
+            const int64_t op = S->R.pool_off[pf + lane];
             B->same_off[lane] = op;
             int64_t ml, rv;
             bool lng;
@@ -558,7 +629,7 @@
             L.count--;
         else if (kind == MRZ_DK_EVICT) {
             L.count--;
-            ws = mrz_uni(S->R.same_slot[i][(int)L.victim_round]);
+            ws = mrz_uni(S->R.pool_slot[pf + (int)L.victim_round]);
             L.victim_round = L.victim_round + 1 == C.max_chain ? 0 : L.victim_round + 1;
         } else if (kind == MRZ_DK_DISPLACE) {
             const int w2 = mrz_uni(S->R.w2[i]);
@@ -589,6 +660,12 @@
     }
     *xw_n = nx;
     return mrz_select_emit(C, L, mlen, m_off, m_rev, lane);
+}
+
+__device__ __forceinline__ int mrz_deep_cap(int64_t min_mask, int pinned, int narrow_bits) {
+    int cap = __popcll((unsigned long long)min_mask) >= narrow_bits ? MRZ_DEEP_LANES / 2 : MRZ_DEEP_LANES;
+    if (pinned > 0) cap = pinned < MRZ_DEEP_LANES ? pinned : MRZ_DEEP_LANES;
+    return cap;
 }
 
 __device__ __forceinline__ int mrz_deep_incl(int v, int *ws, int lane, int wave, int *total) {
@@ -689,6 +766,7 @@
     }
     if (tid == 0 && G) __hip_atomic_store(&G->xcc_plus1, (unsigned long long)MRZ_DEEP_XCC_ID() + 1ull, __ATOMIC_RELAXED, __HIP_MEMORY_SCOPE_AGENT);
     unsigned long long batch_seq = 0;
+    int max_nb = 0;
     const int64_t lim = (C.end < K.seg_end - 1) ? C.end : K.seg_end - 1;
     const int smask = (int)C.slot_mask;
     const int max_chain = (int)C.max_chain;
@@ -735,26 +813,39 @@
         PROF_T0R();
         const int64_t better = (L.min_mask << 1) | 1;
         const bool loose = L.tag_mask != better;
-        int64_t my_q = 0, my_t = 0;
-        bool live = false;
-        if (ci + tid < K.n) {
-            const mrz_cand c = K.cand[ci + tid];
-            my_q = c.off;
-            my_t = c.t;
-            live = c.off > L.p && c.off <= lim && (c.t & L.min_mask) == L.min_mask;
+        const int cap = mrz_deep_cap(L.min_mask, a.deep_batch, a.deep_narrow_bits);
+        mrz_cand my_c[2];
+        bool live[2];
+#pragma unroll
+        for (int k = 0; k < 2; k++) {
+            my_c[k].off = 0;
+            my_c[k].t = 0;
+            live[k] = false;
+            const int64_t e = ci + 2 * tid + k;
+            if (e < K.n) {
+                my_c[k] = K.cand[e];
+                live[k] = my_c[k].off > L.p && my_c[k].off <= lim && (my_c[k].t & L.min_mask) == L.min_mask;
+            }
         }
         int total;
-        const int incl = mrz_deep_incl(live ? 1 : 0, S->wsum, lane, wave, &total);
-        const int at = incl - 1;
-        if (live && at < MRZ_DEEP_LANES) {
-            S->R.q[at] = my_q;
-            S->R.t[at] = my_t;
-            S->idx[at] = (int)(ci + tid);
-        }
-        const int nb = total < MRZ_DEEP_LANES ? total : MRZ_DEEP_LANES;
-        int64_t n_examined = K.n - ci < MRZ_DEEP_THREADS ? K.n - ci : MRZ_DEEP_THREADS;
+        const int n_live = (live[0] ? 1 : 0) + (live[1] ? 1 : 0);
+        int at = mrz_deep_incl(n_live, S->wsum, lane, wave, &total) - n_live;
+#pragma unroll
+        for (int k = 0; k < 2; k++) {
+            if (live[k]) {
+                if (at < cap) {
+                    S->R.q[at] = my_c[k].off;
+                    S->R.t[at] = my_c[k].t;
+                    S->idx[at] = (int)(ci + 2 * tid + k);
+                }
+                at++;
+            }
+        }
+        if (tid == 0) S->R.pool_n = 0;
+        const int nb = total < cap ? total : cap;
+        int64_t n_examined = K.n - ci < 2 * MRZ_DEEP_THREADS ? K.n - ci : 2 * MRZ_DEEP_THREADS;
         __syncthreads();
-        if (total > MRZ_DEEP_LANES) n_examined = (int64_t)S->idx[MRZ_DEEP_LANES - 1] + 1 - ci;
+        if (total > cap) n_examined = (int64_t)S->idx[cap - 1] + 1 - ci;
         if (nb == 0) {
             ci += n_examined;
             __syncthreads();
@@ -762,6 +853,7 @@
         }
         ST_ADD(MRZ_ST_D_BATCHES, 1);
         ST_ADD(MRZ_ST_D_LANES, nb);
+        max_nb = nb > max_nb ? nb : max_nb;
         PROF_ADD(MRZ_ST_D_T_FORM);
         if (!loose) {
             int nscan = 1;
@@ -784,7 +876,8 @@
                     G->tag_mask = L.tag_mask;
                     G->clean_ptr = L.clean_ptr;
                     G->xw_n = 0;
-                    __hip_atomic_store(&G->done, 0ull, __ATOMIC_RELAXED, __HIP_MEMORY_SCOPE_AGENT);
+                    G->stamp = (long long)(batch_seq + 1);
+                    __hip_atomic_store(&G->done, (batch_seq + 1) << 32, __ATOMIC_RELAXED, __HIP_MEMORY_SCOPE_AGENT);
                 }
                 MRZ_DEEP_WAIT();
                 __syncthreads();
@@ -798,12 +891,13 @@
             {
                 int k = 0;
                 for (int i = 0; i < nb; i += nscan, k++)
-                    if (k % MRZ_DEEP_WAVES == wave) mrz_deep_scan(C, S, i, better, L.tag_mask, L.clean_ptr, 0, lane);
+                    if (k % MRZ_DEEP_WAVES == wave) mrz_deep_scan(C, S, i, better, L.tag_mask, L.clean_ptr, 0, lane, wave);
             }
             if (nscan > 1) {
                 if (tid == 0) {
                     long long spins = 0;
-                    while (__hip_atomic_load(&G->done, __ATOMIC_ACQUIRE, __HIP_MEMORY_SCOPE_AGENT) < (unsigned long long)helper_lanes &&
+                    while (__hip_atomic_load(&G->done, __ATOMIC_ACQUIRE, __HIP_MEMORY_SCOPE_AGENT) <
+                               (batch_seq << 32) + (unsigned long long)helper_lanes &&
                            spins++ < (1ll << 26))
                         __builtin_amdgcn_s_sleep(1);
                     S->ctl[6] = spins < (1ll << 26) ? 1 : 0;
@@ -814,7 +908,7 @@
                     if (tid == 0) C.st->error = 7;
                     ok = false;
                 } else if (tid < nb && tid % nscan != 0)
-                    mrz_deep_rec_copy(&S->R, &G->R, tid);
+                    mrz_deep_rec_copy(&S->R, &G->R, tid, true);
             }
         }
         __syncthreads();
@@ -952,10 +1046,10 @@
                         if ((res & 1) && mrz_deep_smap_get(S, w_e) < i) hard = true;
                         if ((res & 2) && mrz_deep_smap_get(S, fe_e) < i) hard = true;
                         if (hard || (f & MRZ_DF_STALE)) stop |= MRZ_DS_CONFLICT;
-                        const int ns = S->R.nsame[i];
+                        const int ns = S->R.nsame[i], pf = S->R.first[i];
                         const int64_t floor_p = L.last_match > 0 ? L.last_match : 0;
                         for (int k = 0; k < ns; k++)
-                            if (mrz_deep_pair_eval(S->R.raw[i][k], q, S->R.same_off[i][k], floor_p)) stop |= MRZ_DS_COOP;
+                            if (mrz_deep_pair_eval(S->R.pool_raw[pf + k], q, S->R.pool_off[pf + k], floor_p)) stop |= MRZ_DS_COOP;
                         if (wr_w && kind_e == MRZ_DK_OVER && w_e >= cw_base && w_e < cw_base + cw_len) stop |= MRZ_DS_COOP;
                         if (wr_w2 && kind2 == MRZ_DK_OVER && w2 >= cw_base && w2 < cw_base + cw_len) stop |= MRZ_DS_COOP;
                         for (int k = S->R.xw_seen[i]; k < xw_n; k++) {
@@ -1034,7 +1128,7 @@
                         if (a_ev) {
                             const int er = ((i1 >> 10) & 1023) - 1;
                             const int vr = (int)(((unsigned)L.victim_round + (unsigned)er) % (unsigned)max_chain);
-                            ws = S->R.same_slot[i][vr];
+                            ws = S->R.pool_slot[(int)S->R.first[i] + vr];
                         }
                         if (kind == MRZ_DK_DISPLACE) {
                             mrz_slot oc;
@@ -1173,7 +1267,7 @@
                         for (int k = wave; k < nr; k += MRZ_DEEP_WAVES) {
                             const int li = (int)S->rescan_list[k];
                             const int cf = mrz_uni(S->cpos[li]);
-                            mrz_deep_scan(C, S, li, better, L.tag_mask, L.clean_ptr, xw_n, lane, cf == 0x7fffffff ? 0 : cf);
+                            mrz_deep_scan(C, S, li, better, L.tag_mask, L.clean_ptr, xw_n, lane, wave, true, cf == 0x7fffffff ? 0 : cf);
                         }
                         __syncthreads();
                         PROF_ADD(MRZ_ST_D_T_RESCAN);
@@ -1273,6 +1367,7 @@
         st->hint_positions = L.p - hint_p0;
         st->hint_events = L.n_events - hint_ev0;
         st->hint_matched = L.mbytes;
+        if (max_nb > st->deep_max_batch) st->deep_max_batch = max_nb;
 #ifdef MRZ_SEQ_STATS
         for (int k = 0; k < MRZ_ST_N; k++) st->prof[k] += stat[k];
 #endif
@@ -1282,7 +1377,7 @@
 extern "C" hipError_t mrz_launch_sequencer_deep(hipStream_t stream, const uint8_t *buf, mrz_slot *tab, const mrz_cand *cand,
                                                 const int *tile_off, const mrz_u64 *bitmap, mrz_event *events,
                                                 mrz_seq_state *st, void *gmailbox, int n_helpers, int xcd, void *deep_shared,
-                                                int scanners) {
+                                                int scanners, int batch, int narrow_bits) {
     mrz_seq_args a;
     a.buf = buf;
     a.tab = tab;
@@ -1294,6 +1389,8 @@
     a.gmailbox = gmailbox;
     a.xcd = xcd & 7;
     a.deep_bits = 0;
+    a.deep_batch = batch > 0 ? batch : 0;
+    a.deep_narrow_bits = narrow_bits > 0 ? narrow_bits : MRZ_DEEP_NARROW_BITS;
 #if MRZ_HELPER_WGS == 0
     n_helpers = 0;
 #endif
```

After: 6.044 GiB/s. -5.1%, worse.
